# jimmyyhwu/spatial-intention-maps

Hardware: AMD Instinct MI355X
Metric: Q-map transitions/sec, 96x96: `value` = full train() step (M2: policy fwd + bwd, double-DQN next-state forwards, clip, SGD); `value_fwd_bwd_only` = policy fwd+bwd alone (M1, the literal reading of "fwd+bwd") (higher is better)
Workload: dtype f32

## Files before the change

### include/simq.h

```cpp
#ifndef SIMQ_H
#define SIMQ_H

#include <stdint.h>

#ifdef __cplusplus
extern "C" {
#endif

#define SIMQ_VERSION 500
#define SIMQ_STATE_WIDTH 96

#define SIMQ_MODE_EVAL 0
#define SIMQ_MODE_TRAIN 1
#define SIMQ_MODE_TRAIN_NOGRAD 2

#define SIMQ_KIND_CONV_W 0
#define SIMQ_KIND_CONV_B 1
#define SIMQ_KIND_BN_W 2
#define SIMQ_KIND_BN_B 3

#define SIMQ_PREC_FP32 0
#define SIMQ_PREC_BF16X3 1
#define SIMQ_PREC_BF16 2

typedef struct simq_plan simq_plan;

int simq_version(void);
#define SIMQ_BUILD_ABLATIONS 1
int simq_build_flags(void);
const char* simq_last_error(void);

int simq_plan_create(int num_input_channels, int num_output_channels, simq_plan** out);
int simq_plan_create_ex(int num_input_channels, int num_output_channels, int precision, simq_plan** out);
typedef struct simq_plan_options {
    int struct_bytes;
    int winograd;
    int winograd_min_cc;
    int winograd_f4_forward;
    int winograd_f4_min_tiles;
    int winograd_f4_grad;
    int winograd_f4_fwd_grad_min_cc;
    int winograd_wgrad;
    int winograd_wgrad_f4;
    int stem_bf16;
    int bf16_act_grads;
    int keep_fp32_activations;
    int fold_eval_bn_bf16;
    int fuse_bn_backward_sums;
    int fuse_stem_backward_sums;
    int fuse_bn1_apply;
    int deterministic;
    int bn1_mask_from_preact;
    int wgrad_ksplit;
    int fwd_overlap;
    int wgrad_overlap;
    int plane_xcd;
    int wgrad_xcd_group;
    int tail_split;
    int early_target_after_block;
    int gemm_split;
} simq_plan_options;
void simq_plan_options_default(simq_plan_options* options);
int simq_plan_create_opts(int num_input_channels, int num_output_channels, int precision, const simq_plan_options* options,
                          simq_plan** out);
int simq_plan_get_options(const simq_plan* plan, simq_plan_options* out);
int simq_plan_precision(const simq_plan* plan);
void simq_plan_destroy(simq_plan* plan);

int64_t simq_param_count(const simq_plan* plan);
int simq_param_num_tensors(const simq_plan* plan);
int simq_param_tensor_info(const simq_plan* plan, int index, char* name, int name_cap,
                           int64_t* offset, int64_t shape[4], int* kind);
int64_t simq_bnbuf_count(const simq_plan* plan);
int simq_bn_num_layers(const simq_plan* plan);
int simq_bn_layer_info(const simq_plan* plan, int index, char* name, int name_cap, int64_t* offset, int* channels);

int64_t simq_workspace_bytes(const simq_plan* plan, int batch);
int64_t simq_workspace_bytes_forward(const simq_plan* plan, int batch);

int64_t simq_wcache_bytes(const simq_plan* plan);
int simq_weights_prepare(const simq_plan* plan, const float* d_params, void* d_wcache, void* stream);

int simq_workspace_tensor(const simq_plan* plan, int batch, const char* name, int64_t* byte_offset, int64_t* elems,
                          int* channels);

int simq_workspace_tensor_ex(const simq_plan* plan, int batch, const char* name, int64_t* byte_offset, int64_t* elems, int* channels,
                             int* storage);

int simq_forward(const simq_plan* plan, int mode, int batch, const float* d_params, const void* d_wcache, float* d_bnbuf,
                 const float* d_x, float* d_q, void* d_workspace, void* stream);

int simq_backward(const simq_plan* plan, int batch, const float* d_params, const void* d_wcache, const float* d_dq,
                  float* d_grads, void* d_workspace, void* stream);

int64_t simq_backward_trace_bytes(const simq_plan* plan, int batch);
int simq_backward_trace_tensor(const simq_plan* plan, int batch, const char* name, int64_t* byte_offset, int64_t* elems, int* channels,
                               int* storage);
int simq_backward_traced(const simq_plan* plan, int batch, const float* d_params, const void* d_wcache, const float* d_dq,
                         float* d_grads, void* d_workspace, void* d_trace, void* stream);

int simq_backward_phase(const simq_plan* plan, int batch, const float* d_params, const void* d_wcache, const float* d_dq,
                        float* d_grads, void* d_workspace, int phase, void* stream);
int64_t simq_grad_bucket_split(const simq_plan* plan);
int simq_backward_onehot(const simq_plan* plan, int batch, const float* d_params, const void* d_wcache, const int64_t* d_action,
                         const float* d_q_sa, const float* d_y, float grad_scale, float* d_grads, void* d_workspace, int phase,
                         void* stream);

typedef int (*simq_reduce_fn)(void* user, double* d_buf, int64_t count, void* stream);
typedef struct simq_sync { simq_reduce_fn reduce; void* user; int global_batch; int world_size; } simq_sync;
int simq_forward_sync(const simq_plan* plan, int mode, int batch, const float* d_params, const void* d_wcache, float* d_bnbuf,
                      const float* d_x, float* d_q, void* d_workspace, void* stream, const simq_sync* sync);
int simq_backward_sync(const simq_plan* plan, int batch, const float* d_params, const void* d_wcache, const float* d_dq,
                       const int64_t* d_action, const float* d_q_sa, const float* d_y, float grad_scale, float* d_grads,
                       void* d_workspace, int phase, void* stream, const simq_sync* sync);
int simq_comm_reduce_f64(void* comm, double* d_buf, int64_t count, void* stream);
int simq_forward_sync_null(const simq_plan* plan, int layout_batch, float* d_bnbuf, void* d_workspace, void* stream, const simq_sync* sync);

int simq_q_argmax(const float* d_q, int rows, int n, int64_t* d_index, float* d_max, void* stream);
int simq_q_gather(const float* d_q, int rows, int n, const int64_t* d_index, float* d_out, void* stream);
int simq_scatter_next_values(const float* d_values, const int32_t* d_nonfinal_pos, int n_nonfinal,
                             float* d_next_state_values, int batch, void* stream);
int simq_td_huber(const float* d_q, int batch, int n, const int64_t* d_action, const float* d_reward,
                  const float* d_next_state_values, float gamma, float grad_scale,
                  float* d_q_sa, float* d_y, float* d_td_error, float* d_out4, float* d_dq, void* stream);

int simq_clip_sgd_step(float* d_params, float* d_grads, float* d_momentum, int64_t count,
                       float max_norm, float lr, float momentum, float weight_decay, int first_step,
                       void* d_scratch, float* d_total_norm, void* stream);

int simq_replay_gather(const float* d_ring, int64_t item_floats, const int64_t* d_index, int count,
                       float* d_out, void* stream);

typedef struct simq_train_args {
    const simq_plan* plan;
    int batch, num_nonfinal, global_batch, use_double_dqn, first_step;
    int sync_bn;
    float gamma, lr, momentum, weight_decay, max_norm, reserved2_;
    float* params; void* wcache; float* bnbuf; float* grads; float* momentum_buf; void* ws_train; void* ws_tmp;
    const float* t_params; const void* t_wcache; float* t_bnbuf; void* t_ws;
    const float* state; const float* next_state; const int64_t* action; const float* reward; const int32_t* nonfinal_pos;
    float* q; float* q_next; float* q_tgt; float* dq;
    float* nsv; float* vals; int64_t* best; float* q_sa; float* y; float* td; float* out4;
    void* opt_scratch; float* total_norm;
    void* stream; void* side_stream;
    int global_nonfinal;
    int struct_bytes;
    struct simq_comm* comm;
    float* loss_host;
    void* target_stream;
    void* third_stream;
} simq_train_args;
int simq_train_step(const simq_train_args* a);
int simq_train_loss_wait(const simq_plan* plan);
int simq_plan_adopt_side_stream(const simq_plan* plan, void* side_stream);

#define SIMQ_COMM_ID_BYTES 128
#define SIMQ_COMM_F32 0
#define SIMQ_COMM_F64 1
typedef struct simq_comm simq_comm;
int simq_comm_unique_id(void* id_out );
int simq_comm_init(const void* id, int world_size, int rank, simq_comm** out);
int simq_comm_adopt_stream(simq_comm* comm, void* stream);
int simq_comm_world_size(const simq_comm* comm);
int simq_comm_rank(const simq_comm* comm);
int simq_comm_allreduce(simq_comm* comm, void* d_buf, int64_t count, int dtype, void* producer_stream);
int simq_comm_broadcast(simq_comm* comm, void* d_buf, int64_t bytes, int root, void* producer_stream);
int simq_comm_wait(simq_comm* comm, void* consumer_stream);
int simq_comm_progress(simq_comm* comm, int64_t out[4]);
int simq_comm_time_waits(simq_comm* comm, int on);
int simq_comm_last_wait_ms(simq_comm* comm, float* ms);
int simq_comm_destroy(simq_comm* comm);

int simq_bce_with_logits(const float* d_logits, const float* d_target, int64_t n, float* d_dlogits, double* d_loss_sum, void* stream);
int simq_split_last_channel(const float* d_x, float* d_head, float* d_last, int64_t pixels, int channels, void* stream);
int simq_sigmoid_concat(const float* d_state, const float* d_logit, float* d_out, float* d_prob, int64_t pixels, int channels, void* stream);

int simq_nchw_to_nhwc(const float* d_in, float* d_out, int batch, int channels, int hw, void* stream);
int simq_nhwc_to_nchw(const float* d_in, float* d_out, int batch, int channels, int hw, void* stream);

typedef struct simq_launch_opts {
    int struct_bytes;
    int force_bm, force_bn;
    int tail_split;
    int plane_xcd;
    int wgrad_xcd_group;
    int wgrad_ksplit;
    int gemm_split;
} simq_launch_opts;
void simq_launch_opts_default(simq_launch_opts* opts);
int simq_conv2d_fwd(const float* d_x, const float* d_w_ohwi, const float* d_bias, float* d_y,
                    int batch, int hin, int win, int cin, int cout, int r, int s, int stride, int pad,
                    double* d_stats , void* stream, const simq_launch_opts* opts);
int simq_conv2d_fwd_winograd(const float* d_x, const float* d_w_ohwi, const float* d_bias, float* d_y,
                             int batch, int hin, int win, int cin, int cout,
                             double* d_stats , float* d_scratch, void* stream, const simq_launch_opts* opts);
int simq_conv2d_fwd_winograd4(const float* d_x, const float* d_w_ohwi, const float* d_bias, float* d_y,
                              int batch, int hin, int win, int cin, int cout,
                              double* d_stats , float* d_scratch, void* stream, const simq_launch_opts* opts);
int simq_bn_relu_apply(const void* d_y, const double* d_stats, const float* d_gamma, const float* d_beta, const void* d_res, int relu,
                       void* d_out, int64_t rows, int channels, int storage, float* d_saved, float* d_running, void* stream);
int simq_bn_relu_backward(const void* d_g, const void* d_mask, int mask_kind, const void* d_y, const float* d_saved, const float* d_gamma,
                          const double* d_red, void* d_dy, void* d_dz_out, float* d_dgamma, float* d_dbeta, int64_t rows, int channels,
                          int storage, void* stream);
int simq_conv2d_fwd_bnrelu_in(const float* d_y_pre, const float* d_in_scale, const float* d_in_shift, const float* d_w_ohwi,
                              const float* d_bias, float* d_y, int batch, int hin, int win, int cin, int cout, int r, int s, int stride,
                              int pad, int form, float* d_scratch, void* stream, const simq_launch_opts* opts);
int simq_conv2d_wgrad_bnrelu_in(const float* d_y_pre, const float* d_in_scale, const float* d_in_shift, const float* d_dy, float* d_dw,
                                int batch, int hin, int win, int cin, int cout, int r, int s, int stride, int pad, int form,
                                float* d_scratch, void* stream, const simq_launch_opts* opts);
int simq_conv2d_fwd_stem_f32(const float* d_x, const float* d_w_ohwi, float* d_y, int batch, int hin, int win, int cin, double* d_stats,
                             void* stream);
int simq_conv2d_fwd_stem_bf16(const float* d_x, const float* d_w_ohwi, uint16_t* d_y, int batch, int hin, int win, int cin,
                              double* d_stats, void* d_scratch, void* stream);
int simq_conv2d_wgrad_stem_bf16(const float* d_x, const uint16_t* d_dy, float* d_dw, int batch, int hin, int win, int cin,
                                float* d_scratch, void* stream);
int simq_conv2d_wgrad_winograd(const float* d_x, const float* d_dy, float* d_dw_ohwi,
                               int batch, int hin, int win, int cin, int cout, float* d_scratch, void* stream, const simq_launch_opts* opts);
int simq_gemm_f32_batched(const float* d_x, const float* d_w, float* d_y, int m, int n, int k, int batch, void* stream,
                          const simq_launch_opts* opts);
int simq_conv2d_dgrad(const float* d_dy, const float* d_w_ohwi, float* d_wt_scratch, float* d_dx,
                      int batch, int hin, int win, int cin, int cout, int r, int s, int pad, void* stream, const simq_launch_opts* opts);
int simq_conv2d_wgrad(const float* d_x, const float* d_dy, float* d_dw_ohwi ,
                      int batch, int hin, int win, int cin, int cout, int r, int s, int stride, int pad,
                      void* stream, const simq_launch_opts* opts);
int simq_conv2d_fwd_bf16(const float* d_x, const float* d_w_ohwi, const float* d_bias, float* d_y, int batch, int hin, int win,
                         int cin, int cout, int r, int s, int stride, int pad, int nplanes, void* d_scratch, double* d_stats,
                         void* stream, const simq_launch_opts* opts);
int simq_conv2d_wgrad_bf16(const float* d_x, const float* d_dy, float* d_dw_ohwi, int batch, int hin, int win, int cin, int cout,
                           int r, int s, int stride, int pad, int nplanes, void* d_scratch, void* stream, const simq_launch_opts* opts);
int64_t simq_conv2d_wgrad_bf16_slab_bytes(void);
int simq_conv2d_wgrad_bf16_slab(const float* d_x, const float* d_dy, float* d_dw_ohwi, int batch, int hin, int win, int cin, int cout,
                                int r, int s, int stride, int pad, int nplanes, void* d_scratch, void* d_slab, void* stream, const simq_launch_opts* opts);
int simq_upsample2x_fwd(const float* d_in, float* d_out, int batch, int h, int w, int c, void* stream);
int simq_upsample2x_bwd(const float* d_dout, float* d_din, int batch, int h, int w, int c, void* stream);

typedef struct simq_grid_problem {
    int64_t grid_offset;
    int64_t out_offset;
    int32_t rows, cols;
    int32_t src_i, src_j;
} simq_grid_problem;
#define SIMQ_GRID_MAX_CELLS (1 << 22)
int simq_grid_distance_images(const uint8_t* d_grids, int64_t grids_bytes, const simq_grid_problem* problems, int n,
                              simq_grid_problem* d_problems, float* d_out, int64_t out_floats, float pixels_per_meter,
                              int unreachable_to_max, float scale, int32_t* d_status, void* stream);

typedef struct simq_grid_path_problem {
    int64_t grid_offset;
    int64_t thin_offset;
    int64_t closest_offset;
    int64_t path_offset;
    int64_t parents_offset;
    int64_t dist_offset;
    int32_t path_capacity;
    int32_t rows, cols;
    int32_t src_i, src_j, tgt_i, tgt_j;
    int32_t box_i0, box_j0, box_rows, box_cols;
    int32_t reserved_;
} simq_grid_path_problem;
#define SIMQ_GRID_PATH_MAX_BOX_CELLS 20000
int simq_grid_paths(const uint8_t* d_grids, int64_t grids_bytes, const int32_t* d_closest, int64_t closest_ints,
                    const simq_grid_path_problem* problems, int n, simq_grid_path_problem* d_problems, int32_t* d_paths,
                    int64_t path_pairs, int32_t* d_lengths, int32_t* d_endpoints, int32_t* d_parents, int64_t parents_ints, float* d_dist,
                    int64_t dist_floats, int32_t* d_status, void* stream);

typedef struct simq_grid_query_problem {
    int64_t grid_offset;
    int64_t closest_offset;
    int64_t work_offset;
    int64_t target_offset;
    int32_t n_targets;
    int32_t rows, cols;
    int32_t src_i, src_j;
    int32_t reserved_;
} simq_grid_query_problem;
int simq_grid_distance_queries(const uint8_t* d_grids, int64_t grids_bytes, const int32_t* d_closest, int64_t closest_ints,
                               const simq_grid_query_problem* problems, int n, const int32_t* targets, int64_t n_targets_total,
                               void* d_descriptors, float* d_work, int64_t work_floats, int images, float* d_out, int64_t out_floats,
                               int32_t* d_status, void* stream);

#define SIMQ_LOCAL_MAP 0
#define SIMQ_LOCAL_DISTANCE 1
#define SIMQ_LOCAL_ROBOTS 2
#define SIMQ_LOCAL_OVERHEAD 3
#define SIMQ_LOCAL_CONSTANT 4
#define SIMQ_LOCAL_CROP 136
#define SIMQ_LOCAL_MAX_CHANNELS 64
typedef struct simq_local_rotation {
    double r[4];
    double offset[2];
    int32_t shape[2];
} simq_local_rotation;
typedef struct simq_local_map {
    const float* d_data;
    int32_t rows, cols;
} simq_local_map;
typedef struct simq_local_robot {
    simq_local_rotation rot;
    int32_t pixel_i, pixel_j;
    int32_t mask;
    float seg_value;
    float map_value;
    int32_t seg_mask;
} simq_local_robot;
typedef struct simq_local_problem {
    simq_local_rotation rot;
    int32_t pixel_i, pixel_j;
    int32_t rows, cols;
    int32_t robot_begin, robot_count;
} simq_local_problem;
typedef struct simq_local_channel {
    int32_t kind;
    int32_t map;
    float value;
    int32_t reserved_;
} simq_local_channel;
int64_t simq_local_state_desc_bytes(int n_maps, int n_robots, int n, int n_channels);
int simq_local_state_images(const simq_local_map* maps, int n_maps, const float* d_masks, int n_masks, const simq_local_robot* robots,
                            int n_robots, const simq_local_problem* problems, int n, const simq_local_channel* channels, int n_channels,
                            void* d_desc, int64_t desc_bytes, float* d_out, int64_t out_floats, void* stream);

#define SIMQ_INTENTION_STORE 0
#define SIMQ_INTENTION_RAMP 1
#define SIMQ_INTENTION_MAX_RADIUS 8
typedef struct simq_intention_segment {
    double start, stop, step;
    int32_t r0, c0, r1, c1;
    int32_t mode;
    int32_t drop_last;
    float value;
    int32_t reserved_;
} simq_intention_segment;
typedef struct simq_intention_problem {
    int32_t seg_begin, seg_count;
} simq_intention_problem;
int64_t simq_intention_desc_bytes(int n_segments, int n);
int simq_intention_maps(const simq_intention_segment* segments, int n_segments, const simq_intention_problem* problems, int n, int rows,
                        int cols, int radius, void* d_desc, int64_t desc_bytes, float* d_out, int64_t out_floats, void* stream);

#define SIMQ_OCCUPANCY_MAX_DIM 256
#define SIMQ_OCCUPANCY_MAX_RADIUS 16
typedef struct simq_occupancy_problem {
    int64_t occupancy_offset;
    int64_t mask_offset;
    int64_t out_offset;
    int32_t rows, cols;
    int32_t radius, thin_radius;
} simq_occupancy_problem;
int simq_occupancy_maps(const uint8_t* d_maps, int64_t maps_bytes, const simq_occupancy_problem* problems, int n,
                        simq_occupancy_problem* d_problems, uint8_t* d_cspace, uint8_t* d_thin, int64_t cspace_bytes, int32_t* d_closest,
                        int64_t closest_ints, int32_t* d_status, void* stream);

#define SIMQ_OBSERVATION_MAX_POINTS (1 << 22)
typedef struct simq_observation_problem {
    int64_t depth_offset;
    int64_t ids_offset;
    int64_t px_offset;
    int64_t py_offset;
    int64_t overhead_offset;
    int64_t occupancy_offset;
    float cam[3], principal[3], right[3], up[3];
    float far_near, far, far_minus_near;
    int32_t min_obstacle, max_obstacle;
    int32_t receptacle, has_receptacle;
    int32_t min_cube, max_cube;
    int32_t height, width;
    int32_t rows, cols;
    int32_t reserved_;
} simq_observation_problem;
int simq_observation_update(const void* d_frames, int64_t frame_words, const simq_observation_problem* problems, int n,
                            simq_observation_problem* d_problems, float* d_overhead, int64_t overhead_floats, uint8_t* d_occupancy,
                            int64_t occupancy_bytes, int32_t* d_status, void* stream);

#define SIMQ_VISUALIZATION_MAX_OUTPUTS 4
typedef struct simq_visualization_problem {
    const float* d_state;
    const float* d_output;
    int64_t out_offset;
    int32_t n, channels;
} simq_visualization_problem;
int simq_state_output_visualizations(const simq_visualization_problem* problems, int n_problems, simq_visualization_problem* d_problems,
                                     const float* d_jet, double alpha, int chw, float* d_out, int64_t out_floats, void* stream);

int simq_profile_start(void);
int simq_profile_stop(double* out, int max_kinds);
int simq_launch_counts_reset(void);
int64_t simq_launch_count(const char* family);
int simq_launch_counts(char* buf, int cap);

#ifdef __cplusplus
}
#endif
#endif
```

### spatial-intention-maps_amd/csrc/backward.hip

```cpp
#include "plan.h"

using namespace simq;

namespace {

int bn_bwd(const Ctx& c, const BnL& bn, const float* g, const float* mask, const float* y, const Act& dy, float* dz_out, int64_t rows,
           bool reduced = false, const uint16_t* mask16 = nullptr, int y_bf16 = -1, int g_bf16 = 0, bool mask_from_y = false) {
    if (y_bf16 < 0) y_bf16 = c.ybf();
    SIMQ_REQUIRE(!mask_from_y || (reduced && !mask && !mask16), "bn_bwd: the recomputed mask needs the fused reduction and no mask tensor");
    if (!reduced) {
        if (bn.C <= 128) {
            double* rep = reinterpret_cast<double*>(c.ws + c.L.colsum);
            SIMQ_CHECK_HIP(hipMemsetAsync(rep, 0, sizeof(double) * kStatReplicas * 2 * bn.C, c.stream));
            RC(launch_bn_bwd_reduce(g, mask, y, c.aux(bn, 2), c.aux(bn, 3), rep, rows, bn.C, c.stream, y_bf16, g_bf16, kStatReplicas));
            RC(launch_stats_fold(rep, c.red(bn), 2 * bn.C, kStatReplicas, c.stream));
        } else {
            RC(launch_bn_bwd_reduce(g, mask, y, c.aux(bn, 2), c.aux(bn, 3), c.red(bn), rows, bn.C, c.stream, y_bf16, g_bf16));
        }
    }
    RC(c.sync_reduce(c.red(bn), 2 * (int64_t)bn.C));
    return launch_bn_bwd_apply(g, mask, y, c.aux(bn, 2), c.aux(bn, 3), c.params + bn.g_off, c.red(bn), dy.fv ? dy.f : nullptr, dz_out,
                               c.grads + bn.g_off, c.grads + bn.b_off, rows, bn.C, c.stream, dy.pl, mask16, y_bf16,
                               c.sync ? c.bn_rows(rows) : 0.0, c.sync ? 1.f / (float)c.sync->world_size : 1.f, g_bf16,
                               mask_from_y ? c.aux(bn, 0) : nullptr, mask_from_y ? c.aux(bn, 1) : nullptr);
}

int conv_wgrad(const Ctx& c, const ConvL& cv, const Act& x, const Act& dy, int hin, const InBn& in = InBn()) {
    ConvGeom g = geom(c.p, cv, c.B, hin);
    if (c.mc() && cv.wp_off >= 0) {
        SIMQ_REQUIRE(!in.on(), "conv_wgrad: BatchNorm-on-load exists for fp32 plans only");
        const uint16_t* xs[2] = {x.pl.hi, x.pl.lo ? x.pl.lo : x.pl.hi};
        const uint16_t* ds[2] = {dy.pl.hi, dy.pl.lo ? dy.pl.lo : dy.pl.hi};
        return launch_conv_wgrad_bf16(xs, ds, c.p->np(), c.grads + cv.w_off, g, c.stream, c.L.wslab >= 0 ? c.f(c.L.wslab) : nullptr, c.dslab());
    }
    if (cv.wu_off >= 0 && c.L.wino >= 0 && winograd_wgrad_eligible(g) && c.p->opt.winograd_wgrad &&
        winograd_wgrad_pays(g, c.p->opt.winograd_wgrad_f4 != 0))
        return launch_conv_wgrad_winograd(x.f, dy.f, c.grads + cv.w_off, g, c.f(c.L.wino), c.stream, c.p->opt.winograd_wgrad_f4 != 0, in);
    return launch_conv_wgrad(x.f, dy.f, c.grads + cv.w_off, g, c.stream, in, c.dslab());
}

int conv_dgrad(const Ctx& c, const ConvL& cv, const Act& dy, float* dx, const float* addend, int hin,
               const ConvEpilogue& fuse = ConvEpilogue(), int g_bf16 = 0) {
    ConvGeom g;
    g.tune = c.p->tune();
    g.B = c.B; g.Hin = hin; g.Win = hin; g.Cin = cv.cout; g.Cout = cv.cin; g.Hout = hin; g.Wout = hin;
    g.R = cv.k; g.S = cv.k; g.stride = 1; g.pad = cv.k - 1 - cv.pad;
    ConvEpilogue e = fuse;
    e.addend = addend;
    e.y_bf16 = g_bf16; e.addend_bf16 = g_bf16;
    if (c.mc() && cv.wp_off >= 0) {
        const uint16_t* ds[2] = {dy.pl.hi, dy.pl.lo ? dy.pl.lo : dy.pl.hi};
        const uint16_t* wsp[2];
        c.wplanes(cv, true, wsp);
        return launch_conv_igemm_bf16(ds, wsp, c.p->np(), dx, g, e, c.stream);
    }
    if (cv.wut4_off >= 0 && c.L.wino >= 0 && winograd_f4_forward(g, c.p->opt.winograd_f4_min_tiles))
        return launch_conv_winograd4(dy.f, reinterpret_cast<const float*>(c.wc + c.W.wu) + cv.wut4_off, dx, g, e, c.f(c.L.wino), c.stream);
    if (cv.wut_off >= 0 && c.L.wino >= 0 && winograd_eligible(g))
        return launch_conv_winograd(dy.f, reinterpret_cast<const float*>(c.wc + c.W.wu) + cv.wut_off, dx, g, e, c.f(c.L.wino), c.stream);
    return launch_conv_igemm(dy.f, reinterpret_cast<const float*>(c.wc + c.W.wt) + cv.wt_off, dx, g, e, c.stream);
}

}

namespace simq {

int backward_impl(const Ctx& c, const float* d_dq, int phase, const OneHotGrad* oh) {
    const simq_plan* p = c.p;
    const Layout& L = c.L;
    const int B = c.B;
    const int wov = p->opt.wgrad_overlap;
    const bool mc_piped = c.mc() && wov == 4 && c.planes_only() && L.DP[2] >= 0 && L.S2[0] >= 0;
    const bool ov = c.wstream != nullptr && (wov == 2 || mc_piped || ((wov == 1 || wov == 3 || wov == 4) && !c.mc()));
    const bool wide_mc = ov && mc_piped;
    const bool wide = (ov && !c.mc() && wov != 3) || wide_mc;
    const bool piped = wide && wov == 4 && L.S2[0] >= 0 && c.ev_wdone[0] && c.ev_wdone[1];
    Ctx cw = c;
    if (ov) { cw.stream = c.wstream; if (L.wino2 >= 0) cw.L.wino = L.wino2; }
    const TraceLayout TL = c.trace ? make_trace_layout(p, B) : TraceLayout();
    auto trace = [&](int64_t off, const void* src, int64_t bytes) -> int {
        if (c.trace && src) SIMQ_CHECK_HIP(hipMemcpyAsync(c.trace + off, src, (size_t)bytes, hipMemcpyDeviceToDevice, c.stream));
        return 0;
    };
    auto fork = [&]() -> int {
        if (ov) { SIMQ_CHECK_HIP(hipEventRecord(c.ev_wfork, c.stream)); SIMQ_CHECK_HIP(hipStreamWaitEvent(c.wstream, c.ev_wfork, 0)); }
        return 0;
    };
    auto join = [&]() -> int {
        if (ov) { SIMQ_CHECK_HIP(hipEventRecord(c.ev_wjoin, c.wstream)); SIMQ_CHECK_HIP(hipStreamWaitEvent(c.stream, c.ev_wjoin, 0)); }
        return 0;
    };
    if (phase != 2) {
        SIMQ_CHECK_HIP(hipMemsetAsync(c.grads, 0, p->nparams * sizeof(float), c.stream));
        SIMQ_CHECK_HIP(hipMemsetAsync(c.ws + L.red, 0, p->red_total * sizeof(double), c.stream));
    }
    float* S[4] = {c.f(L.S[0]), c.f(L.S[1]), c.f(L.S[2]), c.f(L.S[3])};
    const int64_t smax = (int64_t)B * 294912;
    auto dyact = [&](float* buf, int which) { Act a; a.f = buf; a.pl = c.planes(L.DP[which], smax); return a; };
    double* cs = reinterpret_cast<double*>(c.ws + L.colsum);
    double* cs_side = cs + kStatReplicas * 2 * 128;
    const int64_t rows = (int64_t)B * 576;
    const bool no_fuse_head = !p->opt.fuse_bn_backward_sums;
    const bool head_side = piped && phase != 2;
    Act dyh = dyact(S[0], 0);
    Act t2 = dyact(S[1], 1);
    if (phase != 2) {
    if (oh) {
        RC(launch_head_onehot_bwd(c.f(L.ah2), c.params + p->h3.w_off, oh->action, oh->q_sa, oh->y, oh->grad_scale, S[1],
                                  c.grads + p->h3.w_off, c.grads + p->h3.b_off, B, p->cout, c.stream,
                                  c.f(L.yh2), 0, c.aux(p->hb2, 2), c.aux(p->hb2, 3), no_fuse_head ? nullptr : c.red(p->hb2), p->opt.deterministic));
    } else {
        RC(launch_upsample2x_fwd(c.f(L.ah2), c.f(L.up2), B, 48, 48, 32, c.stream));
        RC(launch_head_conv3_bwd(c.f(L.up2), c.params + p->h3.w_off, d_dq, S[0], c.grads + p->h3.w_off, c.grads + p->h3.b_off, B, 9216, 32, p->cout, c.stream,
                                 c.dslab()));
        RC(launch_upsample2x_bwd(S[0], S[1], B, 48, 48, 32, c.stream));
        RC(trace(TL.head.da2, S[1], (int64_t)B * 2304 * 32 * 4));
    }
    if (head_side) {
        dyh.f = c.f(L.S2[0]); dyh.pl = c.planes(L.DP2[0], smax);
        t2.f = c.f(L.S2[1]); t2.pl = c.planes(L.DP2[1], smax);
    }
    const Ctx& ch = head_side ? cw : c;
    static const int bias_side_on = SIMQ_TUNE_INT("SIMQ_HEAD_BIAS_SIDE", 1);
    const bool bias_side = head_side && c.mc() && bias_side_on;
    bool hb1_fused = false;
    {
        Act dy2; dy2.f = S[0];
        RC(bn_bwd(c, p->hb2, S[1], c.f(L.ah2), c.f(L.yh2), dy2, nullptr, (int64_t)B * 2304, oh != nullptr && !no_fuse_head, nullptr, 0));
        RC(trace(TL.head.dy2, S[0], (int64_t)B * 2304 * 32 * 4));
        RC(launch_upsample2x_bwd(S[0], t2.f, B, 24, 24, 32, c.stream, t2.pl));
        RC(trace(TL.head.dz2, t2.f, rows * 32 * 4));
        Act a1; a1.f = c.f(L.ah1); a1.pl = c.planes(L.p_up1, rows * 128);
        if (head_side) RC(fork());
        RC(launch_colsum_rep(t2.f, bias_side ? cs_side : cs, c.grads + p->h2.b_off, rows, 32, kStatReplicas, bias_side ? ch.stream : c.stream));
        if (c.lazy1()) {
            Act yh1; yh1.f = c.f(L.yh1);
            RC(conv_wgrad(ch, p->h2, yh1, t2, 24, c.inbn_saved(p->hb1)));
        } else {
            RC(conv_wgrad(ch, p->h2, a1, t2, 24));
        }
        ConvEpilogue fh;
        const bool fuse_hb1 = !no_fuse_head && !c.mc();
        if (fuse_hb1) {
            if (c.lazy1()) { fh.bnr_mscale = c.aux(p->hb1, 0); fh.bnr_mshift = c.aux(p->hb1, 1); }
            else fh.bnr_mask = c.f(L.ah1);
            fh.bnr_y1 = c.f(L.yh1); fh.bnr_y_bf16 = c.ybf();
            fh.bnr_mean1 = c.aux(p->hb1, 2); fh.bnr_invstd1 = c.aux(p->hb1, 3); fh.bnr_red1 = c.red(p->hb1);
        }
        RC(conv_dgrad(c, p->h2, t2, S[2], nullptr, 24, fh));
        RC(trace(TL.head.da1, S[2], rows * 128 * 4));
        hb1_fused = fuse_hb1;
    }
    RC(bn_bwd(c, p->hb1, S[2], c.lazy1() ? nullptr : c.f(L.ah1), c.f(L.yh1), dyh, nullptr, rows, hb1_fused, nullptr, -1, 0, c.lazy1()));
    RC(trace(TL.head.dy1, dyh.f, rows * 128 * 4));
    if (head_side) RC(fork());
    RC(launch_colsum_rep(dyh.f, bias_side ? cs_side : cs, c.grads + p->h1.b_off, rows, 128, kStatReplicas, bias_side ? ch.stream : c.stream));
    RC(conv_wgrad(ch, p->h1, c.act(L.blk[7].out, L.blk[7].p_out, rows * 512), dyh, 24));
    if (head_side) SIMQ_CHECK_HIP(hipEventRecord(c.ev_wdone[1], c.wstream));
    }
    const bool no_fuse = !p->opt.fuse_bn_backward_sums;
    auto fuse_block_out = [&](int bi) {
        ConvEpilogue e;
        if (no_fuse) return e;
        const BlockL& bb = p->blocks[bi];
        if (c.planes_only()) e.bnr_mask16 = c.planes(L.blk[bi].p_out, rows * bb.planes).hi;
        else e.bnr_mask = c.f(L.blk[bi].out);
        e.bnr_y_bf16 = c.ybf();
        e.bnr_y1 = c.f(L.blk[bi].y2); e.bnr_mean1 = c.aux(bb.b2, 2); e.bnr_invstd1 = c.aux(bb.b2, 3); e.bnr_red1 = c.red(bb.b2);
        if (bb.has_ds) {
            e.bnr_y2 = c.f(L.blk[bi].yd); e.bnr_mean2 = c.aux(bb.bds, 2); e.bnr_invstd2 = c.aux(bb.bds, 3); e.bnr_red2 = c.red(bb.bds);
        }
        return e;
    };
    const int gb = c.gbf();
    if (phase != 2) RC(conv_dgrad(c, p->h1, dyh, S[1], nullptr, 24, fuse_block_out(7), gb));
    const int gi = 1;
    const int i_hi = phase == 2 ? kPhaseSplitBlock - 1 : 7, i_lo = phase == 1 ? kPhaseSplitBlock : 0;
    for (int i = i_hi; i >= i_lo; --i) {
        if (c.ev_late && i == c.late_block) SIMQ_CHECK_HIP(hipEventRecord(c.ev_late, c.stream));
        const BlockL& b = p->blocks[i];
        const Layout::Blk& o = L.blk[i];
        const Act xin = i == 0 ? c.act(L.pooled, L.p_pooled, rows * 64)
                               : c.act(L.blk[i - 1].out, L.blk[i - 1].p_out, rows * p->blocks[i - 1].planes);
        const Act a1 = c.act(o.a1, o.p_a1, rows * b.planes);
        float* G = S[gi];
        Act T0 = dyact(S[(gi + 1) & 3], 0);
        Act T1 = dyact(S[(gi + 2) & 3], 1);
        float* T2 = S[(gi + 3) & 3];
        const int set = (i_hi - i) & 1;
        if (piped) {
            if (set) {
                T0 = Act(); T0.f = c.f(L.S2[0]); T0.pl = c.planes(L.DP2[0], smax);
                T1 = Act(); T1.f = c.f(L.S2[1]); T1.pl = c.planes(L.DP2[1], smax);
                T2 = c.f(L.S2[2]);
            }
            if (i_hi - i >= 2 || (head_side && i_hi - i == 1))
                SIMQ_CHECK_HIP(hipStreamWaitEvent(c.stream, c.ev_wdone[set], 0));
        }
        const bool po = c.planes_only();
        T0.fv = T1.fv = !po;
        const float* m_out = po ? nullptr : c.f(o.out);
        const bool mfy = c.mask1_from_y() && !no_fuse;
        const float* m_a1 = (po || mfy) ? nullptr : c.f(o.a1);
        const uint16_t* m16_out = po ? c.planes(o.p_out, rows * b.planes).hi : nullptr;
        const uint16_t* m16_a1 = (po && !mfy) ? c.planes(o.p_a1, rows * b.planes).hi : nullptr;
        const int64_t nel = rows * b.planes, gsz = gb ? 2 : 4, dsz = po ? 2 : 4;
        auto dptr = [&](const Act& a) -> const void* { return po ? (const void*)a.pl.hi : (const void*)a.f; };
        RC(trace(TL.blk[i].g_out, G, nel * gsz));
        RC(bn_bwd(c, b.b2, G, m_out, c.f(o.y2), T0, b.has_ds ? nullptr : T1.f, rows, !no_fuse, m16_out, -1, gb));
        if (b.has_ds) RC(bn_bwd(c, b.bds, G, m_out, c.f(o.yd), T1, nullptr, rows, !no_fuse, m16_out, -1, gb));
        RC(trace(TL.blk[i].dy2, dptr(T0), nel * dsz));
        if (b.has_ds) RC(trace(TL.blk[i].t1, dptr(T1), nel * dsz));
        else RC(trace(TL.blk[i].t1, T1.f, nel * gsz));
        RC(fork());
        if (c.lazy1()) {
            Act y1; y1.f = c.f(o.y1);
            RC(conv_wgrad(cw, b.c2, y1, T0, 24, c.inbn_saved(b.b1)));
        } else {
            RC(conv_wgrad(cw, b.c2, a1, T0, 24));
        }
        ConvEpilogue f1;
        if (!no_fuse) {
        f1.bnr_y_bf16 = c.ybf();
        if (mfy) { f1.bnr_mscale = c.aux(b.b1, 0); f1.bnr_mshift = c.aux(b.b1, 1); }
        f1.bnr_mask = m_a1; f1.bnr_mask16 = m16_a1; f1.bnr_y1 = c.f(o.y1); f1.bnr_mean1 = c.aux(b.b1, 2); f1.bnr_invstd1 = c.aux(b.b1, 3); f1.bnr_red1 = c.red(b.b1);
        }
        RC(conv_dgrad(c, b.c2, T0, T2, nullptr, 24, f1, gb));
        RC(trace(TL.blk[i].da1, T2, nel * gsz));
        Act D1 = T0;
        if (wide) { D1 = Act(); D1.f = T2; D1.fv = !po; if (wide_mc) D1.pl = c.planes((piped && set) ? L.DP2[2] : L.DP[2], smax); }
        else RC(join());
        RC(bn_bwd(c, b.b1, T2, m_a1, c.f(o.y1), D1, nullptr, rows, !no_fuse, m16_a1, -1, gb, mfy));
        RC(trace(TL.blk[i].dy1, dptr(D1), nel * dsz));
        RC(fork());
        RC(conv_wgrad(cw, b.c1, xin, D1, 24));
        const ConvEpilogue fin = i > 0 ? fuse_block_out(i - 1) : ConvEpilogue();
        if (b.has_ds) {
            RC(conv_wgrad(cw, b.ds, xin, T1, 24));
            RC(conv_dgrad(c, b.ds, T1, G, nullptr, 24, ConvEpilogue(), gb));
            RC(trace(TL.blk[i].g_ds, G, rows * b.cin * gsz));
            RC(conv_dgrad(c, b.c1, D1, G, G, 24, fin, gb));
        } else {
            RC(conv_dgrad(c, b.c1, D1, G, T1.f, 24, fin, gb));
        }
        RC(trace(TL.blk[i].g_in, G, rows * b.cin * gsz));
        if (piped) SIMQ_CHECK_HIP(hipEventRecord(c.ev_wdone[set], c.wstream));
        else RC(join());
    }
    const bool late_join = piped && phase != 1 && i_hi > i_lo && ((i_hi - i_lo) & 1) == 1 && !p->opt.deterministic;
    if (piped) {
        if (late_join) SIMQ_CHECK_HIP(hipStreamWaitEvent(c.stream, c.ev_wdone[0], 0));
        else RC(join());
    }
    if (phase == 1) return 0;
    float* G = S[gi];
    float* T0 = S[(gi + 1) & 3];
    Act T1; T1.f = S[(gi + 2) & 3];
    const bool stem16 = c.W.stem16 >= 0;
    if (stem16) { T1 = dyact(S[(gi + 2) & 3], 1); T1.fv = false; }
    Act x0; x0.f = c.x_ext ? const_cast<float*>(c.x_ext) : c.f(L.x);
    const int y0_bf16 = c.W.stem16 >= 0 ? 1 : 0;
    const bool no_stem_fuse = !p->opt.fuse_stem_backward_sums || !p->opt.fuse_bn_backward_sums;
    double* srep = reinterpret_cast<double*>(c.ws + L.red) + p->stem_rep_off;
    RC(launch_stem_pool_bwd(G, c.f(L.pooled), reinterpret_cast<const uint8_t*>(c.ws + L.idx), T0, B, 48, 48, 64, c.stream, c.gbf(),
                            c.f(L.y0), c.aux(p->stem_bn, 2), c.aux(p->stem_bn, 3), no_stem_fuse ? nullptr : srep, y0_bf16, kStatReplicas));
    if (!no_stem_fuse) RC(launch_stats_fold(srep, c.red(p->stem_bn), 2 * p->stem_bn.C, kStatReplicas, c.stream));
    RC(trace(TL.stem.dz, T0, (int64_t)B * 2304 * 64 * 4));
    RC(bn_bwd(c, p->stem_bn, T0, nullptr, c.f(L.y0), T1, nullptr, (int64_t)B * 2304, !no_stem_fuse, nullptr, y0_bf16));
    RC(trace(TL.stem.dy0, stem16 ? (const void*)T1.pl.hi : (const void*)T1.f, (int64_t)B * 2304 * 64 * (stem16 ? 2 : 4)));
    if (stem16)
        RC(launch_stem_wgrad_bf16(x0.f, T1.pl.hi, c.grads + p->stem.w_off, T0, B, 96, 96, p->cin, c.stream));
    else
        RC(conv_wgrad(c, p->stem, x0, T1, 96));
    if (late_join) RC(join());
    return 0;
}

}

static int attach_backward_side(Ctx& c) {
    const int wov = c.p->opt.wgrad_overlap;
    if (c.wstream || wov == 0 || (c.mc() && wov != 2 && wov != 4)) return 0;
    PlanStreams* ps = nullptr;
    int dev = 0;
    RC(plan_streams(c.p, &ps, &dev));
    if (!ps) return 0;
    if (c.stream) {
        hipDevice_t sdev = 0;
        SIMQ_CHECK_HIP(hipStreamGetDevice(c.stream, &sdev));
        if ((int)sdev != dev) return 0;
    }
    if (!ps->bwd_ev[0]) {
        std::lock_guard<std::mutex> lk(c.p->mu);
        for (int i = 0; i < 4; ++i) SIMQ_CHECK_HIP(hipEventCreateWithFlags(&ps->bwd_ev[i], hipEventDisableTiming));
    }
    if (!ps->bwd_side_ext && !ps->bwd_side) {
        std::lock_guard<std::mutex> lk(c.p->mu);
        SIMQ_CHECK_HIP(hipStreamCreateWithFlags(&ps->bwd_side, hipStreamNonBlocking));
    }
    c.wstream = ps->bwd_side_ext ? ps->bwd_side_ext : ps->bwd_side; c.ev_wfork = ps->bwd_ev[0]; c.ev_wjoin = ps->bwd_ev[1]; c.ev_wdone[0] = ps->bwd_ev[2]; c.ev_wdone[1] = ps->bwd_ev[3];
    return 0;
}

namespace simq {
TraceLayout make_trace_layout(const simq_plan* p, int B) {
    TraceLayout T;
    int64_t off = 0;
    auto take = [&](int64_t bytes) { int64_t o = off; off = align_up(off + bytes, 256); return o; };
    const bool mc = p->precision != SIMQ_PREC_FP32;
    const bool po = mc && !p->opt.keep_fp32_activations && p->opt.fuse_bn_backward_sums;
    const int64_t gsz = (p->precision == SIMQ_PREC_BF16 && p->opt.bf16_act_grads) ? 2 : 4, dsz = po ? 2 : 4;
    for (int i = 7; i >= 0; --i) {
        const int64_t n = (int64_t)B * 576 * p->blocks[i].planes;
        T.blk[i].g_out = take(n * gsz); T.blk[i].dy2 = take(n * dsz);
        T.blk[i].t1 = take(n * (p->blocks[i].has_ds ? dsz : gsz));
        T.blk[i].da1 = take(n * gsz); T.blk[i].dy1 = take(n * dsz);
        T.blk[i].g_ds = p->blocks[i].has_ds ? take((int64_t)B * 576 * p->blocks[i].cin * gsz) : -1;
        T.blk[i].g_in = take((int64_t)B * 576 * p->blocks[i].cin * gsz);
    }
    T.head.da2 = take((int64_t)B * 2304 * 32 * 4); T.head.dy2 = take((int64_t)B * 2304 * 32 * 4); T.head.dz2 = take((int64_t)B * 576 * 32 * 4);
    T.head.da1 = take((int64_t)B * 576 * 128 * 4); T.head.dy1 = take((int64_t)B * 576 * 128 * 4);
    T.stem.dz = take((int64_t)B * 2304 * 64 * 4); T.stem.dy0 = take((int64_t)B * 2304 * 64 * 4);
    T.total = off;
    return T;
}

int backward_sync_side(const simq_plan* plan, int batch, const float* d_params, const void* d_wcache, const float* d_dq,
                              const int64_t* d_action, const float* d_q_sa, const float* d_y, float grad_scale, float* d_grads,
                              void* d_workspace, int phase, void* stream, const simq_sync* sync, hipStream_t wstream, hipEvent_t ev_wfork,
                              hipEvent_t ev_wjoin, hipEvent_t ev_wdone0, hipEvent_t ev_wdone1, const float* x_ext, hipEvent_t ev_late, int late_block) {
    Ctx c{plan, batch, d_params, d_grads, nullptr, static_cast<char*>(d_workspace), make_layout(plan, batch), static_cast<hipStream_t>(stream)};
    c.wc = static_cast<char*>(const_cast<void*>(d_wcache)); c.W = make_wlayout(plan);
    c.sync = sync;
    c.x_ext = x_ext;
    c.ev_late = ev_late; c.late_block = late_block;
    if (wstream && ev_wfork && ev_wjoin) { c.wstream = wstream; c.ev_wfork = ev_wfork; c.ev_wjoin = ev_wjoin; c.ev_wdone[0] = ev_wdone0; c.ev_wdone[1] = ev_wdone1; }
    else RC(attach_backward_side(c));
    if (d_dq) return backward_impl(c, d_dq, phase);
    const OneHotGrad oh{d_action, d_q_sa, d_y, grad_scale};
    return backward_impl(c, nullptr, phase, &oh);
}
}

extern "C" {

int simq_backward_sync(const simq_plan* plan, int batch, const float* d_params, const void* d_wcache, const float* d_dq,
                       const int64_t* d_action, const float* d_q_sa, const float* d_y, float grad_scale, float* d_grads,
                       void* d_workspace, int phase, void* stream, const simq_sync* sync) {
    SIMQ_REQUIRE(plan && d_params && d_wcache && d_grads && d_workspace && (d_dq || (d_action && d_q_sa && d_y)), "backward_sync: NULL argument");
    SIMQ_REQUIRE(phase >= 0 && phase <= 2, "backward: bad phase %d", phase);
    SIMQ_REQUIRE(batch >= 1 && batch <= 4096, "backward: batch=%d out of range", batch);
    RC(check_sync(sync, batch));
    return backward_sync_side(plan, batch, d_params, d_wcache, d_dq, d_action, d_q_sa, d_y, grad_scale, d_grads, d_workspace, phase, stream, sync,
                              nullptr, nullptr, nullptr);
}

int simq_backward_phase(const simq_plan* plan, int batch, const float* d_params, const void* d_wcache, const float* d_dq,
                        float* d_grads, void* d_workspace, int phase, void* stream) {
    SIMQ_REQUIRE(plan && d_params && d_wcache && d_dq && d_grads && d_workspace, "backward: NULL argument");
    SIMQ_REQUIRE(phase >= 0 && phase <= 2, "backward: bad phase %d", phase);
    SIMQ_REQUIRE(batch >= 1 && batch <= 4096, "backward: batch=%d out of range", batch);
    Ctx c{plan, batch, d_params, d_grads, nullptr, static_cast<char*>(d_workspace), make_layout(plan, batch), static_cast<hipStream_t>(stream)};
    c.wc = static_cast<char*>(const_cast<void*>(d_wcache)); c.W = make_wlayout(plan);
    RC(attach_backward_side(c));
    return backward_impl(c, d_dq, phase);
}

int simq_backward_onehot(const simq_plan* plan, int batch, const float* d_params, const void* d_wcache, const int64_t* d_action,
                         const float* d_q_sa, const float* d_y, float grad_scale, float* d_grads, void* d_workspace, int phase,
                         void* stream) {
    SIMQ_REQUIRE(plan && d_params && d_wcache && d_action && d_q_sa && d_y && d_grads && d_workspace, "backward_onehot: NULL argument");
    SIMQ_REQUIRE(phase >= 0 && phase <= 2, "backward: bad phase %d", phase);
    SIMQ_REQUIRE(batch >= 1 && batch <= 4096, "backward: batch=%d out of range", batch);
    Ctx c{plan, batch, d_params, d_grads, nullptr, static_cast<char*>(d_workspace), make_layout(plan, batch), static_cast<hipStream_t>(stream)};
    c.wc = static_cast<char*>(const_cast<void*>(d_wcache)); c.W = make_wlayout(plan);
    const OneHotGrad oh{d_action, d_q_sa, d_y, grad_scale};
    RC(attach_backward_side(c));
    return backward_impl(c, nullptr, phase, &oh);
}

int simq_plan_adopt_side_stream(const simq_plan* plan, void* side_stream) {
    SIMQ_REQUIRE(plan, "plan_adopt_side_stream: NULL plan");
    PlanStreams* ps = nullptr;
    int dev = 0;
    RC(plan_streams(plan, &ps, &dev));
    SIMQ_REQUIRE(ps, "plan_adopt_side_stream: device index %d out of range", dev);
    if (side_stream) {
        hipDevice_t sdev = 0;
        SIMQ_CHECK_HIP(hipStreamGetDevice(static_cast<hipStream_t>(side_stream), &sdev));
        SIMQ_REQUIRE((int)sdev == dev, "plan_adopt_side_stream: the stream belongs to device %d, the calling thread's current device is %d", (int)sdev, dev);
    }
    ps->bwd_side_ext = static_cast<hipStream_t>(side_stream);
    return 0;
}

int64_t simq_backward_trace_bytes(const simq_plan* plan, int batch) {
    if (!plan || batch < 1) return -1;
    return make_trace_layout(plan, batch).total;
}

int simq_backward_trace_tensor(const simq_plan* plan, int batch, const char* name, int64_t* byte_offset, int64_t* elems, int* channels, int* storage) {
    SIMQ_REQUIRE(plan && name && batch >= 1, "backward_trace_tensor: bad argument");
    const TraceLayout T = make_trace_layout(plan, batch);
    const bool mc = plan->precision != SIMQ_PREC_FP32;
    const bool po = mc && !plan->opt.keep_fp32_activations && plan->opt.fuse_bn_backward_sums;
    const int gst = (plan->precision == SIMQ_PREC_BF16 && plan->opt.bf16_act_grads) ? 1 : 0, dst = po ? 1 : 0;
    int li = 0, bi = 0;
    char what[32] = "";
    int64_t off = -1;
    int ch = 0, st = 0;
    if (sscanf(name, "layer%d.%d.%31s", &li, &bi, what) == 3 && li >= 1 && li <= 4 && bi >= 0 && bi <= 1) {
        const int i = (li - 1) * 2 + bi;
        const BlockL& b = plan->blocks[i];
        const std::string w(what);
        ch = b.planes;
        if (w == "g_out") { off = T.blk[i].g_out; st = gst; }
        else if (w == "dy2") { off = T.blk[i].dy2; st = dst; }
        else if (w == "dz" && !b.has_ds) { off = T.blk[i].t1; st = gst; }
        else if (w == "dyd" && b.has_ds) { off = T.blk[i].t1; st = dst; }
        else if (w == "da1") { off = T.blk[i].da1; st = gst; }
        else if (w == "dy1") { off = T.blk[i].dy1; st = dst; }
        else if (w == "g_in") { off = T.blk[i].g_in; st = gst; ch = b.cin; }
        else if (w == "g_ds" && b.has_ds) { off = T.blk[i].g_ds; st = gst; ch = b.cin; }
    }
    int64_t pixels = 576;
    if (off < 0) {
        const std::string n(name);
        const bool stem16 = make_wlayout(plan).stem16 >= 0;
        if (n == "head.da2") { off = T.head.da2; ch = 32; pixels = 2304; }
        else if (n == "head.dy2") { off = T.head.dy2; ch = 32; pixels = 2304; }
        else if (n == "head.dz2") { off = T.head.dz2; ch = 32; }
        else if (n == "head.da1") { off = T.head.da1; ch = 128; }
        else if (n == "head.dy1") { off = T.head.dy1; ch = 128; }
        else if (n == "stem.dz") { off = T.stem.dz; ch = 64; pixels = 2304; }
        else if (n == "stem.dy0") { off = T.stem.dy0; ch = 64; pixels = 2304; st = stem16 ? 1 : 0; }
    }
    SIMQ_REQUIRE(off >= 0, "backward_trace_tensor: '%s' is not a tensor of the traced walk (layer<1-4>.<0-1>.<g_out|dy2|dz|dyd|da1|dy1|g_ds|g_in>, "
                 "head.<da2|dy2|dz2|da1|dy1>, stem.<dz|dy0>)", name);
    if (byte_offset) *byte_offset = off;
    if (elems) *elems = (int64_t)batch * pixels * ch;
    if (channels) *channels = ch;
    if (storage) *storage = st;
    return 0;
}

int simq_backward_traced(const simq_plan* plan, int batch, const float* d_params, const void* d_wcache, const float* d_dq,
                         float* d_grads, void* d_workspace, void* d_trace, void* stream) {
    SIMQ_REQUIRE(plan && d_params && d_wcache && d_dq && d_grads && d_workspace && d_trace, "backward_traced: NULL argument");
    SIMQ_REQUIRE(batch >= 1 && batch <= 4096, "backward: batch=%d out of range", batch);
    Ctx c{plan, batch, d_params, d_grads, nullptr, static_cast<char*>(d_workspace), make_layout(plan, batch), static_cast<hipStream_t>(stream)};
    c.wc = static_cast<char*>(const_cast<void*>(d_wcache)); c.W = make_wlayout(plan);
    c.trace = static_cast<char*>(d_trace);
    RC(attach_backward_side(c));
    return backward_impl(c, d_dq, 0);
}

int simq_backward(const simq_plan* plan, int batch, const float* d_params, const void* d_wcache, const float* d_dq,
                  float* d_grads, void* d_workspace, void* stream) {
    return simq_backward_phase(plan, batch, d_params, d_wcache, d_dq, d_grads, d_workspace, 0, stream);
}

}
```

### spatial-intention-maps_amd/csrc/common.h

```cpp
#pragma once
#include <hip/hip_runtime.h>
#include <stdint.h>

struct simq_comm;

namespace simq {

typedef float floatx16 __attribute__((ext_vector_type(16)));
typedef float floatx4 __attribute__((ext_vector_type(4)));

void set_error(const char* fmt, ...);

#ifdef SIMQ_ABLATIONS
int tune_env_int(const char* name, int dflt);
#define SIMQ_TUNE_INT(name, dflt) (simq::tune_env_int(name, dflt))
#else
#define SIMQ_TUNE_INT(name, dflt) (dflt)
#endif

#define SIMQ_CHECK_HIP(expr)                                                        \
    do {                                                                            \
        hipError_t _e = (expr);                                                     \
        if (_e != hipSuccess) {                                                     \
            simq::set_error("%s:%d: %s -> %s", __FILE__, __LINE__, #expr, hipGetErrorString(_e)); \
            return -2;                                                              \
        }                                                                           \
    } while (0)

#define SIMQ_CHECK_LAUNCH() SIMQ_CHECK_HIP(hipGetLastError())

#define SIMQ_REQUIRE(cond, ...)             \
    do {                                    \
        if (!(cond)) {                      \
            simq::set_error(__VA_ARGS__);   \
            return -1;                      \
        }                                   \
    } while (0)

struct LaunchTune {
    int force_bm = 0, force_bn = 0;
    int tail_split = 0;
    int plane_xcd = 1;
    int wgrad_xcd_group = 1;
    int wgrad_ksplit = 0;
    int gemm_split = 0;
};

struct ConvGeom {
    int B, Hin, Win, Cin, Hout, Wout, Cout, R, S, stride, pad;
    LaunchTune tune;
    int M() const { return B * Hout * Wout; }
    int K() const { return R * S * Cin; }
};

struct ConvEpilogue {
    const float* bias = nullptr;
    double* stats = nullptr;
    const float* scale = nullptr;
    const float* shift = nullptr;
    const float* addend = nullptr;
    int relu = 0;
    int y_bf16 = 0, bnr_y_bf16 = 0;
    int addend_bf16 = 0;
    const float* bnr_mask = nullptr;
    const uint16_t* bnr_mask16 = nullptr;
    const float* bnr_mscale = nullptr; const float* bnr_mshift = nullptr;
    const float* bnr_y1 = nullptr; const float* bnr_mean1 = nullptr; const float* bnr_invstd1 = nullptr; double* bnr_red1 = nullptr;
    const float* bnr_y2 = nullptr; const float* bnr_mean2 = nullptr; const float* bnr_invstd2 = nullptr; double* bnr_red2 = nullptr;
};

struct BnRef {
    const double* stats = nullptr;
    const float* gamma = nullptr;
    const float* beta = nullptr;
    float* rmean = nullptr;
    float* rvar = nullptr;
    float* save_mean = nullptr;
    float* save_invstd = nullptr;
    float* save_scale = nullptr;
    float* save_shift = nullptr;
    double rows = 0.0, inv_rows = 0.0;
    int C = 0;
    double* defer = nullptr;
};
struct InBn {
    const float* scale = nullptr; const float* shift = nullptr;
    BnRef bn;
    int live = 0;
    bool on() const { return live != 0 || scale != nullptr; }
};

void prof_launch_begin(int kind, double flops, double bytes, hipStream_t stream);
void prof_launch_end(hipStream_t stream);
void note_launch(const char* family);

int launch_conv_igemm(const float* x, const float* w, float* y, const ConvGeom& g, const ConvEpilogue& e,
                      hipStream_t stream, const InBn& in = InBn());
int try_gemm_batched_pp(const float* x, const float* w, float* y, int M, int N, int K, int batch, hipStream_t stream);
int launch_gemm_batched(const float* x, const float* w, float* y, int M, int N, int K, int batch, hipStream_t stream, const LaunchTune& tune = LaunchTune());
bool gemm_split3_eligible(int M, int N, int K, int batch);
int launch_gemm_batched_split3(const float* x, const float* w, float* y, int M, int N, int K, int batch, hipStream_t stream, const LaunchTune& tune);
bool winograd_eligible(const ConvGeom& g);
bool winograd_pays(int cin, int cout, long min_cc);
int64_t winograd_scratch_floats(const ConvGeom& g);
int launch_wino_weight(const float* w_ohwi, float* U, int cout, int cin, hipStream_t stream);
struct WinoWeightDesc { int64_t src_off, u_off; int cout, cin, from_wt, pad_; };
constexpr int kWinoWeightTableCap = 72;
struct WinoWeightTable { WinoWeightDesc d[kWinoWeightTableCap]; int n; };
int launch_wino_weight_all(const float* params, const float* wt, float* ubase, const WinoWeightTable& t, hipStream_t stream);
int launch_conv_winograd(const float* x, const float* U, float* y, const ConvGeom& g, const ConvEpilogue& e, float* scratch,
                         hipStream_t stream, const InBn& in = InBn());
bool winograd_f4_forward(const ConvGeom& g, int min_tiles);
int launch_conv_winograd4(const float* x, const float* U4, float* y, const ConvGeom& g, const ConvEpilogue& e, float* scratch,
                          hipStream_t stream, const InBn& in = InBn());
constexpr int64_t kWgradDetSlabFloats = 16 << 20;
int launch_conv_wgrad(const float* x, const float* dy, float* dw, const ConvGeom& g, hipStream_t stream, const InBn& in = InBn(), float* det_slab = nullptr);
int launch_wgrad_slab_sum(const float* slab, float* dw, int64_t n, int splits, hipStream_t stream);
int launch_wgrad_batched(const float* x, const float* dy, float* dw, int M, int N, int K, int batch, hipStream_t stream, const LaunchTune& tune = LaunchTune());
bool winograd_wgrad_eligible(const ConvGeom& g);
bool winograd_wgrad_pays(const ConvGeom& g, bool allow_f4);
int launch_conv_wgrad_winograd(const float* x, const float* dy, float* dw, const ConvGeom& g, float* scratch, hipStream_t stream, bool allow_f4 = true,
                               const InBn& in = InBn());
int tune_forced_tile(const LaunchTune& t, int* bm, int* bn);
int launch_conv_igemm_bf16(const uint16_t* const x[2], const uint16_t* const w[2], int nplanes, float* y, const ConvGeom& g,
                           const ConvEpilogue& e, hipStream_t stream);
int launch_conv_wgrad_bf16(const uint16_t* const x[2], const uint16_t* const dy[2], int nplanes, float* dw, const ConvGeom& g,
                           hipStream_t stream, float* slab = nullptr, float* det_slab = nullptr);
int try_conv_wgrad_bf16_pp(const uint16_t* x, const uint16_t* dy, float* dw, const ConvGeom& g, unsigned x_bytes, unsigned dy_bytes,
                           hipStream_t stream);
int try_conv_wgrad_bf16_img(const uint16_t* x, const uint16_t* dy, float* dw, const ConvGeom& g, unsigned x_bytes, unsigned dy_bytes,
                           hipStream_t stream, float* slab = nullptr);
int64_t conv_wgrad_bf16_slab_bytes();
struct WeightPrepDesc { int64_t w_off, wt_off, wp_off; int cout, taps, cin, pad_; };
struct WeightPrepTable { WeightPrepDesc d[24]; int n; };
int launch_weight_prep_all(const float* params, const WeightPrepTable& t, float* wt_f32, uint16_t* wpl, uint16_t* wtpl, int np,
                           int64_t wp_total, hipStream_t stream);
int launch_split_planes(const float* src, uint16_t* hi, uint16_t* lo, int64_t n, hipStream_t stream);
int launch_weight_planes(const float* w, uint16_t* w_hi, uint16_t* w_lo, uint16_t* wt_hi, uint16_t* wt_lo, int cout, int taps,
                         int cin, hipStream_t stream);
int launch_weight_transpose(const float* w, float* wt, int cout, int taps, int cin, hipStream_t stream);

struct Planes { uint16_t* hi = nullptr; uint16_t* lo = nullptr; };

struct BnEvalDesc { int64_t g_off, b_off, buf_off, aux_off; int C, pad_; };
struct BnEvalTable { BnEvalDesc d[24]; int n; };
int launch_bn_eval_coeff(const BnEvalTable& t, const float* params, const float* bnbuf, float* aux, hipStream_t stream);
int launch_bn_running_update(const double* stats, float* rmean, float* rvar, double rows, int C, hipStream_t stream);
int launch_bn_apply(const float* y, const BnRef& bn, const float* res, const BnRef* rbn, int relu, float* out, int64_t rows,
                    int C, hipStream_t stream, Planes pl = Planes(), Planes res_pl = Planes(), int y_bf16 = 0);
int launch_head_bn_relu_conv3(const float* y, const BnRef& bn, const float* w3, float* a, float* z, int B, int HW, int Cout, hipStream_t stream);
int launch_stem_pool_fwd(const float* y, const BnRef& bn, float* pooled, uint8_t* idx, int B, int H, int W, int C,
                         hipStream_t stream, Planes pl = Planes(), int y_bf16 = 0);
int stem_conv_bf16_wbytes();
int try_conv_img_f32(const float* x, const float* w, float* y, const ConvGeom& g, const ConvEpilogue& e, hipStream_t stream, const InBn& in = InBn());
bool stem_conv_f32_eligible(int H, int W, int C, int cout, int k, int stride, int pad);
int launch_stem_conv_f32(const float* x, const float* w_ohwi, float* y, double* stats, int B, int H, int W, int C, hipStream_t stream);
bool stem_conv_bf16_eligible(int H, int W, int C, int cout, int k, int stride, int pad);
int launch_stem_weight_prep(const float* w, uint16_t* w16, int C, hipStream_t stream);
int launch_stem_conv_bf16(const float* x, const uint16_t* w16, uint16_t* y, double* stats, int B, int H, int W, int C, hipStream_t stream);
int stem_wgrad_bf16_slabs(int B, int H, int W);
int launch_stem_wgrad_bf16(const float* x, const uint16_t* dy, float* dw, float* partial, int B, int H, int W, int C, hipStream_t stream);
int launch_stem_pool_bwd(const float* g, const float* pooled, const uint8_t* idx, float* dz, int B, int H, int W,
                         int C, hipStream_t stream, int g_bf16 = 0, const float* y = nullptr, const float* mean = nullptr,
                         const float* invstd = nullptr, double* red = nullptr, int y_bf16 = 0, int replicas = 1);
int launch_bn_bwd_reduce(const float* g, const float* mask, const float* y, const float* mean,
                         const float* invstd, double* red, int64_t rows, int C, hipStream_t stream, int y_bf16 = 0, int g_bf16 = 0, int replicas = 1);
int launch_bn_bwd_apply(const float* g, const float* mask, const float* y, const float* mean,
                        const float* invstd, const float* gamma, const double* red, float* dy, float* dz_out,
                        float* dgamma, float* dbeta, int64_t rows, int C, hipStream_t stream, Planes pl = Planes(),
                        const uint16_t* mask16 = nullptr, int y_bf16 = 0, double global_rows = 0.0, float dparam_scale = 1.f,
                        int g_bf16 = 0,
                        const float* mscale = nullptr, const float* mshift = nullptr);
int launch_colsum(const float* x, double* red_scratch, float* out, int64_t rows, int C, hipStream_t stream);
int launch_colsum_rep(const float* x, double* red_scratch, float* out, int64_t rows, int C, int replicas, hipStream_t stream);
int launch_colsum_finish(const double* red, float* out, int C, hipStream_t stream);
int launch_upsample2x_fwd(const float* in, float* out, int B, int H, int W, int C, hipStream_t stream, Planes pl = Planes(),
                          double* stats = nullptr, int relu = 0, int replicas = 1);
int launch_bn_running_deferred(float* bnbuf, const double* defer, int64_t n, hipStream_t stream);
int launch_stats_fold(const double* rep, double* out, int n, int replicas, hipStream_t stream);
int launch_upsample2x_bwd(const float* dout, float* din, int B, int H, int W, int C, hipStream_t stream, Planes pl = Planes());
int launch_add_inplace(float* dst, const float* src, int64_t n, hipStream_t stream);
int launch_nchw_to_nhwc(const float* in, float* out, int B, int C, int HW, hipStream_t stream);
int launch_nhwc_to_nchw(const float* in, float* out, int B, int C, int HW, hipStream_t stream);

int launch_head_conv3_fwd(const float* x, const float* w, const float* bias, float* q, int B, int HW, int Cin,
                          int Cout, hipStream_t stream);
int launch_head_up_relu_conv3(const float* z2, const float* w, float* z, int B, int Cout, hipStream_t stream);
int launch_head_upsample_q(const float* z, const float* bias, float* q, int B, int Cout, hipStream_t stream);
int launch_head_onehot_bwd(const float* ah2, const float* w3, const int64_t* action, const float* q_sa, const float* y,
                           float grad_scale, float* ds1, float* dw3, float* db3, int B, int Cout, hipStream_t stream,
                           const float* ypre = nullptr, int ypre_bf16 = 0, const float* mean = nullptr, const float* invstd = nullptr,
                           double* red = nullptr,
                           int serial = 0);
int launch_head_conv3_bwd(const float* x, const float* w, const float* dq, float* dx, float* dw, float* dbias,
                          int B, int HW, int Cin, int Cout, hipStream_t stream, float* det_slab = nullptr);

int launch_q_argmax(const float* q, int rows, int n, int64_t* index, float* maxv, hipStream_t stream);
int launch_q_gather(const float* q, int rows, int n, const int64_t* index, float* out, hipStream_t stream);
int launch_scatter_next_values(const float* values, const int32_t* pos, int n, float* nsv, int batch,
                               hipStream_t stream);
int launch_td_huber(const float* q, int batch, int n, const int64_t* action, const float* reward,
                    const float* nsv, float gamma, float grad_scale, float* q_sa, float* y, float* td,
                    float* out4, float* dq, hipStream_t stream);
int launch_clip_sgd(float* p, float* g, float* m, int64_t count, float max_norm, float lr, float momentum,
                    float wd, int first_step, void* scratch, float* total_norm, hipStream_t stream);
int launch_bce_logits(const float* x, const float* t, int64_t n, float* dx, double* loss_sum, hipStream_t stream);
int launch_split_last_channel(const float* x, float* head, float* last, int64_t pixels, int C, hipStream_t stream);
int launch_sigmoid_concat(const float* state, const float* logit, float* out, float* prob, int64_t pixels, int Cs, hipStream_t stream);
int launch_replay_gather(const float* ring, int64_t item_floats, const int64_t* index, int count, float* out,
                         hipStream_t stream);

int comm_allreduce(simq_comm* c, void* buf, int64_t count, int dtype, hipStream_t producer);
int comm_reduce_f64(void* comm, double* buf, int64_t count, void* stream);
int comm_wait(simq_comm* c, hipStream_t consumer);
hipStream_t comm_stream(simq_comm* c);

}
```

### spatial-intention-maps_amd/csrc/conv_wgrad.hip

```cpp
#include <cstdlib>
#include <type_traits>

#include "common.h"

namespace simq {

namespace {

constexpr int BR = 16;

struct WgradArgs {
    const float* x;
    const float* dy;
    float* dw;
    int Hin, Win, Cin, Hout, Wout, Cout, R, S, stride, pad;
    int M, K;
    int tilesI, tilesJ, rows_per_split;
    int splits, xcd_group;
    unsigned x_bytes, dy_bytes;
    long gx, gdy, gdw;
    float* slab;
    const float* xscale; const float* xshift;
};

template <int TI, int TJ, int WI, int WJ, bool VEC, bool XBN = false>
__global__ void __launch_bounds__(256) wgrad_kernel(const WgradArgs p) {
    static_assert(WI * WJ == 4, "4 waves per block");
    static_assert(VEC || !XBN, "the BatchNorm-on-load form exists for the vector loader only");
    constexpr int NI = TI / WI / 32, NJ = TJ / WJ / 32;
    static_assert(NI >= 1 && NJ >= 1, "wave tile must be a multiple of 32x32");
    constexpr int STAGE = BR * (TI + TJ);
    __shared__ __attribute__((aligned(16))) float smem[2 * STAGE];

    const int tid = threadIdx.x, lane = tid & 63, wave = tid >> 6;
    const int wi = wave / WJ, wj = wave % WJ;
    int id = blockIdx.x, split;
    {
        const int tiles = p.tilesI * p.tilesJ;
        if (p.xcd_group) {
            const int k = id & 7, j = id >> 3;
            split = (j / tiles) * 8 + k;
            id = (j + k) % tiles;
            if (split >= p.splits) return;
        } else {
            split = id / tiles;
            id -= split * tiles;
        }
    }
    const int tj = id % p.tilesJ;
    const int ti = id / p.tilesJ;
    const int i0 = ti * TI;
    const int rbeg = split * p.rows_per_split;
    const int rend = min(p.M, rbeg + p.rows_per_split);
    const int hw = p.Hout * p.Wout;

    int tap = 0, cj0 = 0, ky = 0, kx = 0;
    int sk = 0, sci = 0, sky = 0, skx = 0;
    bool skok = false;
    if constexpr (VEC) {
        const int cj_tiles = p.Cin / TJ;
        tap = tj / cj_tiles;
        cj0 = (tj - tap * cj_tiles) * TJ;
        ky = tap / p.S;
        kx = tap - ky * p.S;
    } else {
        sk = tj * TJ + (tid % TJ);
        skok = sk < p.K;
        int t = sk / p.Cin;
        sci = sk - t * p.Cin;
        sky = t / p.S;
        skx = t - sky * p.S;
    }

    floatx16 acc[NI][NJ];
#pragma unroll
    for (int a = 0; a < NI; ++a)
#pragma unroll
        for (int b = 0; b < NJ; ++b)
#pragma unroll
            for (int r = 0; r < 16; ++r) acc[a][b][r] = 0.f;

    constexpr int Y_F4 = BR * TI / 4, X_F4 = BR * TJ / 4;
    constexpr int Y_PASSES = (Y_F4 + 255) / 256, X_PASSES_V = (X_F4 + 255) / 256;
    constexpr int X_PASSES_S = BR * TJ / 256;
    float4 vy[2][Y_PASSES], vx[2][VEC ? X_PASSES_V : 1];
    float sx[2][VEC ? 1 : X_PASSES_S];
    unsigned xok[2] = {0u, 0u};
    float4 xsc = make_float4(1.f, 1.f, 1.f, 1.f), xsh = make_float4(0.f, 0.f, 0.f, 0.f);
    if constexpr (XBN) {
        const int ch = cj0 + (tid % (TJ / 4)) * 4;
        xsc = make_float4(p.xscale[ch], p.xscale[ch + 1], p.xscale[ch + 2], p.xscale[ch + 3]);
        xsh = make_float4(p.xshift[ch], p.xshift[ch + 1], p.xshift[ch + 2], p.xshift[ch + 3]);
    }
    __amdgpu_buffer_rsrc_t xr = __builtin_amdgcn_make_buffer_rsrc(const_cast<float*>(p.x + blockIdx.y * p.gx), 0, p.x_bytes, 0x00020000);
    __amdgpu_buffer_rsrc_t yr = __builtin_amdgcn_make_buffer_rsrc(const_cast<float*>(p.dy + blockIdx.y * p.gdy), 0, p.dy_bytes, 0x00020000);

    int xb[VEC ? X_PASSES_V : 1], xoy[VEC ? X_PASSES_V : 1], xox[VEC ? X_PASSES_V : 1];
    if constexpr (VEC) {
#pragma unroll
        for (int ps = 0; ps < X_PASSES_V; ++ps) {
            const int r = rbeg + (tid + 256 * ps) / (TJ / 4);
            xb[ps] = r / hw;
            const int rem = r - xb[ps] * hw;
            xoy[ps] = rem / p.Wout;
            xox[ps] = rem - xoy[ps] * p.Wout;
        }
    }
    auto load_tile = [&](auto set_c, int r0) {
        constexpr int SET = decltype(set_c)::value;
#pragma unroll
        for (int ps = 0; ps < Y_PASSES; ++ps) {
            const int idx = tid + 256 * ps;
            const int row = idx / (TI / 4), c4 = idx - row * (TI / 4);
            const int r = r0 + row;
            const bool ok = (Y_F4 % 256 == 0 || idx < Y_F4) && r < rend;
            const unsigned voff = ok ? (unsigned)(r * p.Cout + i0 + c4 * 4) * 4u : 0xFFFFFFFFu;
            vy[SET][ps] = __builtin_bit_cast(float4, __builtin_amdgcn_raw_buffer_load_b128(yr, voff, 0, 0));
        }
        if constexpr (VEC) {
            if constexpr (XBN) xok[SET] = 0u;
#pragma unroll
            for (int ps = 0; ps < X_PASSES_V; ++ps) {
                const int idx = tid + 256 * ps;
                const int row = idx / (TJ / 4), c4 = idx - row * (TJ / 4);
                const int r = r0 + row;
                const int iy = xoy[ps] * p.stride - p.pad + ky, ix = xox[ps] * p.stride - p.pad + kx;
                const bool ok = (X_F4 % 256 == 0 || idx < X_F4) && r < rend && (unsigned)iy < (unsigned)p.Hin &&
                                (unsigned)ix < (unsigned)p.Win;
                const unsigned voff = ok ? (unsigned)(((xb[ps] * p.Hin + iy) * p.Win + ix) * p.Cin + cj0 + c4 * 4) * 4u : 0xFFFFFFFFu;
                vx[SET][ps] = __builtin_bit_cast(float4, __builtin_amdgcn_raw_buffer_load_b128(xr, voff, 0, 0));
                if constexpr (XBN) xok[SET] |= ok ? (1u << ps) : 0u;
                xox[ps] += BR;
                while (xox[ps] >= p.Wout) { xox[ps] -= p.Wout; ++xoy[ps]; }
                if (xoy[ps] >= p.Hout) { xoy[ps] -= p.Hout; ++xb[ps]; }
            }
        } else {
#pragma unroll
            for (int ps = 0; ps < X_PASSES_S; ++ps) {
                const int row = tid / TJ + (256 / TJ) * ps;
                const int r = r0 + row;
                const int b = r / hw, rem = r - b * hw;
                const int oy = rem / p.Wout, ox = rem - oy * p.Wout;
                const int iy = oy * p.stride - p.pad + sky, ix = ox * p.stride - p.pad + skx;
                const bool ok = skok && r < rend && (unsigned)iy < (unsigned)p.Hin && (unsigned)ix < (unsigned)p.Win;
                const unsigned voff = ok ? (unsigned)(((b * p.Hin + iy) * p.Win + ix) * p.Cin + sci) * 4u : 0xFFFFFFFFu;
                sx[SET][ps] = __builtin_bit_cast(float, __builtin_amdgcn_raw_buffer_load_b32(xr, voff, 0, 0));
            }
        }
    };
    auto store_tile = [&](auto set_c, int buf) {
        constexpr int SET = decltype(set_c)::value;
        float* Ys = smem + buf * STAGE;
        float* Xs = Ys + BR * TI;
#pragma unroll
        for (int ps = 0; ps < Y_PASSES; ++ps) {
            int idx = tid + 256 * ps;
            if (Y_F4 % 256 == 0 || idx < Y_F4) *reinterpret_cast<float4*>(Ys + idx * 4) = vy[SET][ps];
        }
        if constexpr (VEC) {
#pragma unroll
            for (int ps = 0; ps < X_PASSES_V; ++ps) {
                int idx = tid + 256 * ps;
                float4 v = vx[SET][ps];
                if constexpr (XBN) {
                    const bool ok = (xok[SET] >> ps) & 1u;
                    v.x = ok ? fmaxf(__builtin_fmaf(v.x, xsc.x, xsh.x), 0.f) : 0.f; v.y = ok ? fmaxf(__builtin_fmaf(v.y, xsc.y, xsh.y), 0.f) : 0.f;
                    v.z = ok ? fmaxf(__builtin_fmaf(v.z, xsc.z, xsh.z), 0.f) : 0.f; v.w = ok ? fmaxf(__builtin_fmaf(v.w, xsc.w, xsh.w), 0.f) : 0.f;
                }
                if (X_F4 % 256 == 0 || idx < X_F4) *reinterpret_cast<float4*>(Xs + idx * 4) = v;
            }
        } else {
#pragma unroll
            for (int ps = 0; ps < X_PASSES_S; ++ps) Xs[(tid / TJ + (256 / TJ) * ps) * TJ + (tid % TJ)] = sx[SET][ps];
        }
    };

    const int fi = lane & 31, fh = lane >> 5;
    auto compute = [&](int buf) {
        const float* Ys = smem + buf * STAGE;
        const float* Xs = Ys + BR * TI;
#pragma unroll
        for (int kk = 0; kk < BR / 2; ++kk) {
            float af[NI], bf[NJ];
#pragma unroll
            for (int a = 0; a < NI; ++a) af[a] = Ys[(kk * 2 + fh) * TI + wi * (TI / WI) + a * 32 + fi];
#pragma unroll
            for (int b = 0; b < NJ; ++b) bf[b] = Xs[(kk * 2 + fh) * TJ + wj * (TJ / WJ) + b * 32 + fi];
#pragma unroll
            for (int a = 0; a < NI; ++a)
#pragma unroll
                for (int b = 0; b < NJ; ++b)
                    acc[a][b] = __builtin_amdgcn_mfma_f32_32x32x2f32(af[a], bf[b], acc[a][b], 0, 0, 0);
        }
    };
    using S0 = std::integral_constant<int, 0>;
    using S1 = std::integral_constant<int, 1>;

    if (rbeg >= rend) return;
    const int nk = (rend - rbeg + BR - 1) / BR;
    load_tile(S0{}, rbeg);
    store_tile(S0{}, 0);
    load_tile(S1{}, rbeg + BR);
    __syncthreads();
    int kt = 0;
    for (; kt + 1 < nk; kt += 2) {
        load_tile(S0{}, rbeg + (kt + 2) * BR);
        compute(0);
        store_tile(S1{}, 1);
        __syncthreads();
        load_tile(S1{}, rbeg + (kt + 3) * BR);
        compute(1);
        store_tile(S0{}, 0);
        __syncthreads();
    }
    if (kt < nk) compute(0);

#pragma unroll
    for (int b = 0; b < NJ; ++b) {
        const int j = wj * (TJ / WJ) + b * 32 + fi;
        size_t col;
        bool cok = true;
        if constexpr (VEC) {
            col = (size_t)tap * p.Cin + cj0 + j;
        } else {
            col = (size_t)tj * TJ + j;
            cok = col < (size_t)p.K;
        }
        if (!cok) continue;
#pragma unroll
        for (int a = 0; a < NI; ++a) {
#pragma unroll
            for (int r = 0; r < 16; ++r) {
                const int i = i0 + wi * (TI / WI) + a * 32 + (r & 3) + 8 * (r >> 2) + 4 * fh;
                if (p.slab) p.slab[((size_t)split * p.Cout + i) * p.K + col] = acc[a][b][r];
                else unsafeAtomicAdd(p.dw + blockIdx.y * p.gdw + (size_t)i * p.K + col, acc[a][b][r]);
            }
        }
    }
}

template <int TI, int TJ, int WI, int WJ, bool VEC>
int run(const WgradArgs& a, hipStream_t stream, const LaunchTune& tune, int batch = 1) {
    static_assert(256 % (TJ / 4) == 0, "a lane keeps its channel quad across the passes of the x loader");
    WgradArgs p = a;
    p.tilesI = p.Cout / TI;
    p.tilesJ = VEC ? p.R * p.S * (p.Cin / TJ) : (p.K + TJ - 1) / TJ;
    const int tiles = p.tilesI * p.tilesJ;
    const int ltiles = tiles * batch;
    const int rsteps = (p.M + BR - 1) / BR;
    int max_splits = rsteps / 8;
    if (max_splits > 96) max_splits = 96;
    if (max_splits < 1) max_splits = 1;
    int splits = 1;
    double best = 1e300;
    for (int s = 1; s <= max_splits; ++s) {
        const long rounds = ((long)ltiles * s + 255) / 256;
        const double util = rounds == 1 ? 0.6 : rounds == 2 ? 0.85 : 1.0;
        const double cost = (double)rounds * ((rsteps + s - 1) / s + 6) / util;
        if (cost < best * 0.999) { best = cost; splits = s; }
    }
    if (p.slab) {
        const int64_t fit = kWgradDetSlabFloats / ((int64_t)p.Cout * p.K);
        SIMQ_REQUIRE(batch == 1 && fit >= 1, "wgrad: the deterministic slab holds %ld floats, one tile set needs %ld", (long)kWgradDetSlabFloats, (long)p.Cout * p.K);
        if (splits > fit) splits = (int)fit;
    }
    if (const int forced_s = batch > 1 ? SIMQ_TUNE_INT("SIMQ_WGRAD_BATCHED_SPLITS", 0) : SIMQ_TUNE_INT("SIMQ_WGRAD_SPLITS", 0)) splits = forced_s;
    int rps = (p.M + splits - 1) / splits;
    rps = ((rps + BR - 1) / BR) * BR;
    splits = (p.M + rps - 1) / rps;
    p.rows_per_split = rps;
    p.splits = splits;
    p.xcd_group = (tune.wgrad_xcd_group == 2 && batch == 1 && splits >= 8 && tiles > 1) ? 1 : 0;
    const int launch_splits = p.xcd_group ? ((splits + 7) / 8) * 8 : splits;
    note_launch(batch > 1 ? "wgrad_f32_batched" : "wgrad_f32");
    prof_launch_begin(1, 2.0 * p.M * p.Cout * p.K * batch,
                      4.0 * batch * ((double)p.M / (p.Hout * p.Wout) * p.Hin * p.Win * p.Cin + (double)p.Cout * p.K + (double)p.M * p.Cout),
                      stream);
    if constexpr (VEC) {
        if (p.xscale) hipLaunchKernelGGL((wgrad_kernel<TI, TJ, WI, WJ, VEC, true>), dim3((unsigned)(tiles * launch_splits), (unsigned)batch), dim3(256), 0, stream, p);
        else hipLaunchKernelGGL((wgrad_kernel<TI, TJ, WI, WJ, VEC>), dim3((unsigned)(tiles * launch_splits), (unsigned)batch), dim3(256), 0, stream, p);
    } else {
        hipLaunchKernelGGL((wgrad_kernel<TI, TJ, WI, WJ, VEC>), dim3((unsigned)(tiles * launch_splits), (unsigned)batch), dim3(256), 0, stream, p);
    }
    prof_launch_end(stream);
    SIMQ_CHECK_LAUNCH();
    if (p.slab) return launch_wgrad_slab_sum(p.slab, p.dw, (int64_t)p.Cout * p.K, splits, stream);
    return 0;
}

__global__ void __launch_bounds__(256) wgrad_slab_sum_kernel(const float* __restrict__ slab, float* __restrict__ dw, size_t n, int splits) {
    for (size_t e = blockIdx.x * (size_t)256 + threadIdx.x; e < n; e += (size_t)gridDim.x * 256) {
        float a = slab[e];
        for (int s2 = 1; s2 < splits; ++s2) a += slab[(size_t)s2 * n + e];
        dw[e] = a;
    }
}

}

int launch_wgrad_slab_sum(const float* slab, float* dw, int64_t n, int splits, hipStream_t stream) {
    int blocks = (int)((n + 255) / 256);
    if (blocks > 2048) blocks = 2048;
    hipLaunchKernelGGL(wgrad_slab_sum_kernel, dim3(blocks), dim3(256), 0, stream, slab, dw, (size_t)n, splits);
    SIMQ_CHECK_LAUNCH();
    return 0;
}

int launch_conv_wgrad(const float* x, const float* dy, float* dw, const ConvGeom& g, hipStream_t stream, const InBn& in, float* det_slab) {
    WgradArgs a;
    a.x = x; a.dy = dy; a.dw = dw; a.slab = det_slab;
    a.xscale = in.scale; a.xshift = in.shift;
    SIMQ_REQUIRE(!in.live, "conv_wgrad: BatchNorm-on-load takes the scale / shift the forward pass saved (not a live layer)");
    SIMQ_REQUIRE(!in.scale || g.Cin % 64 == 0, "conv_wgrad: BatchNorm-on-load needs Cin %% 64 == 0 (Cin=%d)", g.Cin);
    a.Hin = g.Hin; a.Win = g.Win; a.Cin = g.Cin; a.Hout = g.Hout; a.Wout = g.Wout; a.Cout = g.Cout;
    a.R = g.R; a.S = g.S; a.stride = g.stride; a.pad = g.pad;
    a.M = g.M(); a.K = g.K();
    a.tilesI = a.tilesJ = a.rows_per_split = 0;
    a.gx = a.gdy = a.gdw = 0;
    SIMQ_REQUIRE(a.M > 0, "wgrad: empty problem");
    SIMQ_REQUIRE(g.Cout % 32 == 0, "conv_wgrad: Cout=%d must be a multiple of 32", g.Cout);
    const double xb = 4.0 * g.B * g.Hin * g.Win * g.Cin, yb = 4.0 * a.M * g.Cout;
    SIMQ_REQUIRE(xb < 4294967000.0 && yb < 4294967000.0, "conv_wgrad: tensor exceeds the 4 GiB buffer-addressing limit");
    a.x_bytes = (unsigned)xb; a.dy_bytes = (unsigned)yb;
    const bool vec = (g.Cin % 64) == 0;
    if (vec) {
        if (g.Cout % 128 == 0) {
            if (g.Cin % 128 == 0) return (g.Cout / 128) * (g.R * g.S * g.Cin / 128) >= 16 ? run<128, 128, 2, 2, true>(a, stream, g.tune)
                                                                                            : run<64, 64, 2, 2, true>(a, stream, g.tune);
            return run<128, 64, 2, 2, true>(a, stream, g.tune);
        }
        if (g.Cout % 64 == 0) return run<64, 64, 2, 2, true>(a, stream, g.tune);
        if (g.Cin % 128 == 0) return run<32, 128, 1, 4, true>(a, stream, g.tune);
        SIMQ_REQUIRE(false, "conv_wgrad: unsupported Cout=%d Cin=%d", g.Cout, g.Cin);
    }
    SIMQ_REQUIRE(g.Cout % 64 == 0, "conv_wgrad (generic gather): Cout=%d must be a multiple of 64", g.Cout);
    return run<64, 64, 2, 2, false>(a, stream, g.tune);
}

int launch_wgrad_batched(const float* x, const float* dy, float* dw, int M, int N, int K, int batch, hipStream_t stream, const LaunchTune& tune) {
    SIMQ_REQUIRE(M > 0 && N % 128 == 0 && K % 128 == 0 && batch >= 1, "wgrad_batched: M=%d N=%d K=%d batch=%d not supported", M, N, K, batch);
    WgradArgs a;
    a.x = x; a.dy = dy; a.dw = dw;
    a.Hin = M; a.Win = 1; a.Cin = K; a.Hout = M; a.Wout = 1; a.Cout = N; a.R = 1; a.S = 1; a.stride = 1; a.pad = 0;
    a.M = M; a.K = K;
    a.tilesI = a.tilesJ = a.rows_per_split = 0;
    a.gx = (long)M * K; a.gdy = (long)M * N; a.gdw = (long)N * K;
    a.xscale = a.xshift = nullptr; a.slab = nullptr;
    const double xb = 4.0 * M * K, yb = 4.0 * M * N;
    SIMQ_REQUIRE(xb < 4294967000.0 && yb < 4294967000.0, "wgrad_batched: operand exceeds the 4 GiB buffer-addressing limit");
    a.x_bytes = (unsigned)xb; a.dy_bytes = (unsigned)yb;
    return run<128, 128, 2, 2, true>(a, stream, tune, batch);
}

}
```

### spatial-intention-maps_amd/csrc/head.hip

```cpp
#include "common.h"

namespace simq {

namespace {

constexpr int MAX_COUT = 4;

template <int CIN>
__global__ void __launch_bounds__(256) head_conv3_fwd_kernel(const float* __restrict__ x, const float* __restrict__ w,
                                                             const float* __restrict__ bias, float* __restrict__ q,
                                                             int B, int HW, int Cout) {
    constexpr int L = CIN / 4;
    const int sub = threadIdx.x % L;
    float4 wv[MAX_COUT];
    for (int co = 0; co < MAX_COUT; ++co)
        wv[co] = co < Cout ? *reinterpret_cast<const float4*>(w + co * CIN + sub * 4) : make_float4(0, 0, 0, 0);
    const size_t total = (size_t)B * HW;
    const size_t ppb = blockDim.x / L;
    for (size_t pix = blockIdx.x * ppb + threadIdx.x / L; pix < total; pix += (size_t)gridDim.x * ppb) {
        float4 v = *reinterpret_cast<const float4*>(x + pix * CIN + sub * 4);
        const unsigned b = (unsigned)pix / (unsigned)HW, p = (unsigned)pix - b * (unsigned)HW;
        for (int co = 0; co < Cout; ++co) {
            float s = v.x * wv[co].x + v.y * wv[co].y + v.z * wv[co].z + v.w * wv[co].w;
#pragma unroll
            for (int o = L / 2; o >= 1; o >>= 1) s += __shfl_xor(s, o);
            if (sub == 0) q[((size_t)b * Cout + co) * HW + p] = s + (bias ? bias[co] : 0.f);
        }
    }
}

template <int CIN>
__global__ void __launch_bounds__(256) head_conv3_bwd_kernel(const float* __restrict__ x, const float* __restrict__ w,
                                                             const float* __restrict__ dq, float* __restrict__ dx,
                                                             float* dw, float* dbias, int B, int HW, int Cout, float* slab_w, float* slab_b) {
    constexpr int L = CIN / 4;
    __shared__ float red[256 * 4];
    const int sub = threadIdx.x % L;
    float4 wv[MAX_COUT], gw[MAX_COUT];
    float gb[MAX_COUT];
    for (int co = 0; co < MAX_COUT; ++co) {
        wv[co] = co < Cout ? *reinterpret_cast<const float4*>(w + co * CIN + sub * 4) : make_float4(0, 0, 0, 0);
        gw[co] = make_float4(0, 0, 0, 0);
        gb[co] = 0.f;
    }
    const size_t total = (size_t)B * HW;
    const size_t ppb = blockDim.x / L;
    for (size_t pix = blockIdx.x * ppb + threadIdx.x / L; pix < total; pix += (size_t)gridDim.x * ppb) {
        const unsigned b = (unsigned)pix / (unsigned)HW, p = (unsigned)pix - b * (unsigned)HW;
        float4 v = *reinterpret_cast<const float4*>(x + pix * CIN + sub * 4);
        float4 o = make_float4(0, 0, 0, 0);
#pragma unroll
        for (int co = 0; co < MAX_COUT; ++co) {
            if (co < Cout) {
                float g = dq[((size_t)b * Cout + co) * HW + p];
                o.x += g * wv[co].x; o.y += g * wv[co].y; o.z += g * wv[co].z; o.w += g * wv[co].w;
                gw[co].x += g * v.x; gw[co].y += g * v.y; gw[co].z += g * v.z; gw[co].w += g * v.w;
                gb[co] += g;
            }
        }
        *reinterpret_cast<float4*>(dx + pix * CIN + sub * 4) = o;
    }
    for (int co = 0; co < Cout; ++co) {
        __syncthreads();
        red[threadIdx.x * 4 + 0] = gw[co].x; red[threadIdx.x * 4 + 1] = gw[co].y;
        red[threadIdx.x * 4 + 2] = gw[co].z; red[threadIdx.x * 4 + 3] = gw[co].w;
        __syncthreads();
        if (threadIdx.x < CIN) {
            int s = threadIdx.x / 4, e = threadIdx.x % 4;
            float a = 0.f;
            for (int t = s; t < 256; t += L) a += red[t * 4 + e];
            if (slab_w) slab_w[(size_t)blockIdx.x * Cout * CIN + co * CIN + threadIdx.x] = a;
            else unsafeAtomicAdd(dw + co * CIN + threadIdx.x, a);
        }
        __syncthreads();
        red[threadIdx.x] = (sub == 0) ? gb[co] : 0.f;
        __syncthreads();
        if (threadIdx.x == 0) {
            float a = 0.f;
            for (int t = 0; t < 256; ++t) a += red[t];
            if (slab_b) slab_b[(size_t)blockIdx.x * Cout + co] = a;
            else unsafeAtomicAdd(dbias + co, a);
        }
    }
}

__device__ __forceinline__ void lerp2x(int o, int in_size, float scale, int& i0, int& i1, float& l0, float& l1) {
    const float real = scale * (float)o;
    i0 = (int)real;
    if (i0 > in_size - 1) i0 = in_size - 1;
    i1 = i0 + ((i0 < in_size - 1) ? 1 : 0);
    l1 = fminf(fmaxf(real - (float)i0, 0.f), 1.f);
    l0 = 1.f - l1;
}

__global__ void __launch_bounds__(256) head_up_relu_conv3_kernel(const float* __restrict__ z2, const float* __restrict__ w, float* __restrict__ z,
                                                                  int B, int Cout) {
    constexpr int CIN = 32, L = CIN / 4, W1 = 24, W2 = 48;
    const int sub = threadIdx.x % L;
    float4 wv[MAX_COUT];
    for (int co = 0; co < MAX_COUT; ++co)
        wv[co] = co < Cout ? *reinterpret_cast<const float4*>(w + co * CIN + sub * 4) : make_float4(0, 0, 0, 0);
    const float sc = (float)(W1 - 1) / (float)(W2 - 1);
    const unsigned total = (unsigned)B * W2 * W2, ppb = 256 / L;
    for (unsigned pix = blockIdx.x * ppb + threadIdx.x / L; pix < total; pix += gridDim.x * ppb) {
        const unsigned b = pix / (W2 * W2), p = pix - b * (W2 * W2);
        const int oy = (int)(p / W2), ox = (int)(p - (unsigned)oy * W2);
        int y0, y1, x0, x1;
        float ly0, ly1, lx0, lx1;
        lerp2x(oy, W1, sc, y0, y1, ly0, ly1);
        lerp2x(ox, W1, sc, x0, x1, lx0, lx1);
        const float* base = z2 + (size_t)b * W1 * W1 * CIN + sub * 4;
        const float4 v00 = *reinterpret_cast<const float4*>(base + (y0 * W1 + x0) * CIN), v01 = *reinterpret_cast<const float4*>(base + (y0 * W1 + x1) * CIN);
        const float4 v10 = *reinterpret_cast<const float4*>(base + (y1 * W1 + x0) * CIN), v11 = *reinterpret_cast<const float4*>(base + (y1 * W1 + x1) * CIN);
        float4 v;
        v.x = fmaxf(ly0 * (lx0 * v00.x + lx1 * v01.x) + ly1 * (lx0 * v10.x + lx1 * v11.x), 0.f);
        v.y = fmaxf(ly0 * (lx0 * v00.y + lx1 * v01.y) + ly1 * (lx0 * v10.y + lx1 * v11.y), 0.f);
        v.z = fmaxf(ly0 * (lx0 * v00.z + lx1 * v01.z) + ly1 * (lx0 * v10.z + lx1 * v11.z), 0.f);
        v.w = fmaxf(ly0 * (lx0 * v00.w + lx1 * v01.w) + ly1 * (lx0 * v10.w + lx1 * v11.w), 0.f);
        for (int co = 0; co < Cout; ++co) {
            float s = v.x * wv[co].x + v.y * wv[co].y + v.z * wv[co].z + v.w * wv[co].w;
#pragma unroll
            for (int o = L / 2; o >= 1; o >>= 1) s += __shfl_xor(s, o);
            if (sub == 0) z[((size_t)b * Cout + co) * (W2 * W2) + p] = s;
        }
    }
}

__global__ void __launch_bounds__(32) head_onehot_bwd_kernel(const float* __restrict__ ah2, const float* __restrict__ w3,
                                                             const int64_t* __restrict__ action, const float* __restrict__ q_sa,
                                                             const float* __restrict__ y, float grad_scale, float* ds1, float* dw3,
                                                             float* db3, int Cout, const float* __restrict__ ypre, int ypre_bf16,
                                                             const float* __restrict__ mean, const float* __restrict__ invstd, double* red, int B) {
    constexpr int W2 = 96, W1 = 48, CIN = 32;
    for (int b = blockIdx.x; b < B; b += gridDim.x) {
    const int ci = threadIdx.x;
    const int64_t a = action[b];
    const int co = (int)(a / (W2 * W2)), p = (int)(a - (int64_t)co * W2 * W2);
    if (co >= Cout) continue;
    const int oy = p / W2, ox = p - oy * W2;
    const float d = q_sa[b] - y[b];
    const float g = fminf(fmaxf(d, -1.f), 1.f) * grad_scale;
    const float s = (float)(W1 - 1) / (float)(W2 - 1);
    int y0, y1, x0, x1;
    float ly0, ly1, lx0, lx1;
    lerp2x(oy, W1, s, y0, y1, ly0, ly1);
    lerp2x(ox, W1, s, x0, x1, lx0, lx1);
    const float* src = ah2 + (size_t)b * W1 * W1 * CIN + ci;
    const float up = ly0 * (lx0 * src[(y0 * W1 + x0) * CIN] + lx1 * src[(y0 * W1 + x1) * CIN]) +
                     ly1 * (lx0 * src[(y1 * W1 + x0) * CIN] + lx1 * src[(y1 * W1 + x1) * CIN]);
    unsafeAtomicAdd(dw3 + co * CIN + ci, g * up);
    if (ci == 0) unsafeAtomicAdd(db3 + co, g);
    const float dx = g * w3[co * CIN + ci];
    float* base = ds1 + (size_t)b * W1 * W1 * CIN + ci;
    base[(y0 * W1 + x0) * CIN] += ly0 * lx0 * dx;
    base[(y0 * W1 + x1) * CIN] += ly0 * lx1 * dx;
    base[(y1 * W1 + x0) * CIN] += ly1 * lx0 * dx;
    base[(y1 * W1 + x1) * CIN] += ly1 * lx1 * dx;
    if (!red) continue;
    const float mu = mean[ci], is = invstd[ci];
    float s0 = 0.f, s1 = 0.f;
#pragma unroll
    for (int a = 0; a < 2; ++a) {
        if (a == 1 && y1 == y0) continue;
#pragma unroll
        for (int e = 0; e < 2; ++e) {
            if (e == 1 && x1 == x0) continue;
            const size_t o = ((size_t)b * W1 * W1 + (a ? y1 : y0) * W1 + (e ? x1 : x0)) * CIN + ci;
            const float dz = ah2[o] > 0.f ? ds1[o] : 0.f;
            const float yv = ypre_bf16 ? __uint_as_float((uint32_t)reinterpret_cast<const uint16_t*>(ypre)[o] << 16) : ypre[o];
            s0 += dz;
            s1 += dz * ((yv - mu) * is);
        }
    }
    unsafeAtomicAdd(red + ci, (double)s0);
    unsafeAtomicAdd(red + CIN + ci, (double)s1);
    }
}

__global__ void __launch_bounds__(256) head_upsample_q_kernel(const float* __restrict__ z, const float* __restrict__ bias,
                                                              float* __restrict__ q, int planes, int Cout, int vec) {
    constexpr int W2 = 96, W1 = 48;
    const float s = (float)(W1 - 1) / (float)(W2 - 1);
    const unsigned total = (unsigned)planes * W2 * (W2 / 4);
    for (unsigned i = blockIdx.x * blockDim.x + threadIdx.x; i < total; i += gridDim.x * blockDim.x) {
        const unsigned x4 = i % (W2 / 4), r = i / (W2 / 4);
        const unsigned oy = r % W2, pl = r / W2;
        const float bv = bias[pl % (unsigned)Cout];
        int y0, y1; float ly0, ly1;
        lerp2x((int)oy, W1, s, y0, y1, ly0, ly1);
        const float* r0 = z + (size_t)pl * W1 * W1 + y0 * W1;
        const float* r1 = z + (size_t)pl * W1 * W1 + y1 * W1;
        float o[4];
#pragma unroll
        for (int e = 0; e < 4; ++e) {
            int x0, x1; float lx0, lx1;
            lerp2x((int)x4 * 4 + e, W1, s, x0, x1, lx0, lx1);
            o[e] = ly0 * (lx0 * r0[x0] + lx1 * r0[x1]) + ly1 * (lx0 * r1[x0] + lx1 * r1[x1]) + bv;
        }
        float* dst = q + ((size_t)pl * W2 + oy) * W2 + x4 * 4;
        if (vec) *reinterpret_cast<float4*>(dst) = make_float4(o[0], o[1], o[2], o[3]);
        else { dst[0] = o[0]; dst[1] = o[1]; dst[2] = o[2]; dst[3] = o[3]; }
    }
}

}

int launch_head_upsample_q(const float* z, const float* bias, float* q, int B, int Cout, hipStream_t stream) {
    SIMQ_REQUIRE(Cout >= 1 && Cout <= MAX_COUT, "head_upsample_q: Cout=%d unsupported", Cout);
    SIMQ_REQUIRE((size_t)B * Cout * 9216 < 2147483648ull, "head_upsample_q: too many pixels for 32-bit indexing");
    const unsigned total = (unsigned)B * Cout * 96 * 24;
    unsigned blocks = (total + 255) / 256;
    if (blocks > 4096) blocks = 4096;
    hipLaunchKernelGGL(head_upsample_q_kernel, dim3(blocks), dim3(256), 0, stream, z, bias, q, B * Cout, Cout,
                       (reinterpret_cast<uintptr_t>(q) & 15) == 0 ? 1 : 0);
    SIMQ_CHECK_LAUNCH();
    return 0;
}

int launch_head_onehot_bwd(const float* ah2, const float* w3, const int64_t* action, const float* q_sa, const float* y,
                           float grad_scale, float* ds1, float* dw3, float* db3, int B, int Cout, hipStream_t stream,
                           const float* ypre, int ypre_bf16, const float* mean, const float* invstd, double* red, int serial) {
    SIMQ_REQUIRE(Cout >= 1 && Cout <= MAX_COUT, "head_onehot_bwd: Cout=%d unsupported", Cout);
    SIMQ_CHECK_HIP(hipMemsetAsync(ds1, 0, sizeof(float) * (size_t)B * 48 * 48 * 32, stream));
    hipLaunchKernelGGL(head_onehot_bwd_kernel, dim3(serial ? 1 : B), dim3(32), 0, stream, ah2, w3, action, q_sa, y, grad_scale, ds1, dw3, db3, Cout,
                       ypre, ypre_bf16, mean, invstd, red, B);
    SIMQ_CHECK_LAUNCH();
    return 0;
}

int launch_head_up_relu_conv3(const float* z2, const float* w, float* z, int B, int Cout, hipStream_t stream) {
    SIMQ_REQUIRE(Cout >= 1 && Cout <= MAX_COUT, "head_up_relu_conv3: Cout=%d unsupported", Cout);
    SIMQ_REQUIRE((size_t)B * 2304 < 2147483648ull / 32, "head_up_relu_conv3: too many pixels for 32-bit indexing");
    size_t blocks = ((size_t)B * 2304 + 31) / 32;
    if (blocks > 4096) blocks = 4096;
    hipLaunchKernelGGL(head_up_relu_conv3_kernel, dim3((unsigned)blocks), dim3(256), 0, stream, z2, w, z, B, Cout);
    SIMQ_CHECK_LAUNCH();
    return 0;
}

int launch_head_conv3_fwd(const float* x, const float* w, const float* bias, float* q, int B, int HW, int Cin, int Cout,
                          hipStream_t stream) {
    SIMQ_REQUIRE(Cin == 32 && Cout >= 1 && Cout <= MAX_COUT, "head_conv3: Cin=%d Cout=%d unsupported", Cin, Cout);
    SIMQ_REQUIRE((size_t)B * HW < 2147483648ull, "head_conv3: too many pixels for 32-bit indexing");
    size_t blocks = ((size_t)B * HW + 31) / 32;
    if (blocks > 4096) blocks = 4096;
    hipLaunchKernelGGL(head_conv3_fwd_kernel<32>, dim3((unsigned)blocks), dim3(256), 0, stream, x, w, bias, q, B, HW, Cout);
    SIMQ_CHECK_LAUNCH();
    return 0;
}

int launch_head_conv3_bwd(const float* x, const float* w, const float* dq, float* dx, float* dw, float* dbias, int B,
                          int HW, int Cin, int Cout, hipStream_t stream, float* det_slab) {
    SIMQ_REQUIRE(Cin == 32 && Cout >= 1 && Cout <= MAX_COUT, "head_conv3: Cin=%d Cout=%d unsupported", Cin, Cout);
    SIMQ_REQUIRE((size_t)B * HW < 2147483648ull, "head_conv3: too many pixels for 32-bit indexing");
    size_t blocks = ((size_t)B * HW + 31) / 32;
    if (blocks > 1024) blocks = 1024;
    float* slab_w = det_slab;
    float* slab_b = det_slab ? det_slab + 1024 * MAX_COUT * 32 : nullptr;
    hipLaunchKernelGGL(head_conv3_bwd_kernel<32>, dim3((unsigned)blocks), dim3(256), 0, stream, x, w, dq, dx, dw, dbias, B,
                       HW, Cout, slab_w, slab_b);
    SIMQ_CHECK_LAUNCH();
    if (det_slab) {
        if (int rc = launch_wgrad_slab_sum(slab_w, dw, (int64_t)Cout * 32, (int)blocks, stream)) return rc;
        return launch_wgrad_slab_sum(slab_b, dbias, Cout, (int)blocks, stream);
    }
    return 0;
}

}
```

### spatial-intention-maps_amd/csrc/layout.hip

```cpp
#include <algorithm>
#include <cstdarg>
#include <cstdio>
#include <cstdlib>
#include <cstring>

#include "plan.h"

namespace simq {

static thread_local char g_error[512] = "";

#ifdef SIMQ_ABLATIONS
int tune_env_int(const char* name, int dflt) {
    const char* e = getenv(name);
    return e ? atoi(e) : dflt;
}
#endif

void set_error(const char* fmt, ...) {
    va_list ap;
    va_start(ap, fmt);
    vsnprintf(g_error, sizeof(g_error), fmt, ap);
    va_end(ap);
}

Layout make_layout(const simq_plan* p, int B) {
    Layout L;
    int64_t off = 0;
    auto take = [&](int64_t bytes) { int64_t o = off; off = align_up(off + bytes, 256); return o; };
    const int64_t f = sizeof(float);
    L.x = take((int64_t)B * 96 * 96 * p->cin * f);
    L.y0 = take((int64_t)B * 48 * 48 * 64 * f);
    L.pooled = take((int64_t)B * 576 * 64 * f);
    L.idx = take((int64_t)B * 576 * 64);
    for (int i = 0; i < 8; ++i) {
        const int64_t n = (int64_t)B * 576 * p->blocks[i].planes * f;
        L.blk[i].y1 = take(n); L.blk[i].a1 = take(n); L.blk[i].y2 = take(n);
        L.blk[i].yd = p->blocks[i].has_ds ? take(n) : -1;
        L.blk[i].out = take(n);
    }
    L.yh1 = take((int64_t)B * 576 * 128 * f); L.ah1 = take((int64_t)B * 576 * 128 * f);
    L.up1 = take((int64_t)B * 576 * 32 * f);
    L.yh2 = take((int64_t)B * 2304 * 32 * f); L.ah2 = take((int64_t)B * 2304 * 32 * f);
    L.up2 = take((int64_t)B * 9216 * 32 * f);
    L.aux = take(p->aux_total * f);
    L.red = take(p->red_total * (int64_t)sizeof(double));
    L.colsum = take(2 * kStatReplicas * 2 * 128 * sizeof(double));
    L.defer = take(p->nbnbuf * (int64_t)sizeof(double));
    const int64_t smax = (int64_t)B * 294912 * f;
    for (int i = 0; i < 4; ++i) L.S[i] = take(smax);
    L.p_pooled = L.p_up1 = L.DP[0] = L.DP[1] = L.DP[2] = L.DP2[0] = L.DP2[1] = L.DP2[2] = -1;
    for (int i = 0; i < 8; ++i) L.blk[i].p_a1 = L.blk[i].p_out = -1;
    if (p->precision != SIMQ_PREC_FP32) {
        const int64_t h = (int64_t)sizeof(uint16_t) * p->np();
        L.p_pooled = take((int64_t)B * 576 * 64 * h);
        for (int i = 0; i < 8; ++i) {
            const int64_t n = (int64_t)B * 576 * p->blocks[i].planes * h;
            L.blk[i].p_a1 = take(n);
            L.blk[i].p_out = take(n);
        }
        L.p_up1 = take((int64_t)B * 576 * 128 * h);
        L.DP[0] = take((int64_t)B * 294912 * h);
        L.DP[1] = take((int64_t)B * 294912 * h);
    }
    L.wino = p->wino_scratch_per_sample > 0 ? take(((int64_t)B * p->wino_scratch_per_sample + p->wino_du_floats) * f) : -1;
    L.fwd_total = off;
    L.wino2 = L.wino >= 0 ? take(((int64_t)B * p->wino_scratch_per_sample + p->wino_du_floats) * f) : -1;
    const bool piped_mc = p->precision != SIMQ_PREC_FP32;
    for (int i = 0; i < 3; ++i) L.S2[i] = take(smax);
    if (piped_mc) {
        const int64_t h = (int64_t)sizeof(uint16_t) * p->np();
        L.DP[2] = take((int64_t)B * 294912 * h);
        for (int i = 0; i < 3; ++i) L.DP2[i] = take((int64_t)B * 294912 * h);
    }
    L.wslab = p->precision == SIMQ_PREC_BF16 ? take(conv_wgrad_bf16_slab_bytes()) : -1;
    L.dslab = p->opt.deterministic ? take(kWgradDetSlabFloats * f) : -1;
    L.total = off;
    return L;
}

WLayout make_wlayout(const simq_plan* p) {
    WLayout W;
    W.wt = W.wpl = W.wtpl = W.wu = W.stem16 = -1;
    int64_t off = 0;
    auto take = [&](int64_t bytes) { int64_t o = off; off = align_up(off + bytes, 256); return o; };
    if (p->precision == SIMQ_PREC_FP32) {
        W.wt = take(p->wt_total * (int64_t)sizeof(float));
        if (p->wu_total > 0) W.wu = take(p->wu_total * (int64_t)sizeof(float));
    } else {
        const int64_t h = (int64_t)sizeof(uint16_t) * p->np();
        W.wpl = take(p->wp_total * h);
        W.wtpl = take(p->wp_total * h);
        if (p->precision == SIMQ_PREC_BF16 && p->opt.stem_bf16 &&
            stem_conv_bf16_eligible(96, 96, p->stem.cin, p->stem.cout, p->stem.k, p->stem.stride, p->stem.pad))
            W.stem16 = take(stem_conv_bf16_wbytes());
    }
    W.total = off;
    return W;
}

WeightPrepTable weight_table(const simq_plan* p) {
    WeightPrepTable t;
    t.n = 0;
    (void)for_each_mc_conv(p, [&](const ConvL& cv) {
        WeightPrepDesc& d = t.d[t.n++];
        d.w_off = cv.w_off; d.wt_off = cv.wt_off; d.wp_off = cv.wp_off; d.cout = cv.cout; d.taps = cv.k * cv.k; d.cin = cv.cin; d.pad_ = 0;
        return 0;
    });
    return t;
}

int plan_streams(const simq_plan* plan, PlanStreams** out, int* device) {
    int dev = 0;
    SIMQ_CHECK_HIP(hipGetDevice(&dev));
    if (device) *device = dev;
    *out = (dev >= 0 && dev < kMaxDevices) ? &plan->streams[dev] : nullptr;
    return 0;
}

}

using namespace simq;

namespace {

struct Builder {
    simq_plan* p;
    void conv(ConvL& c, const std::string& name, int cin, int cout, int k, int stride, int pad, bool bias, bool dgrad) {
        c.name = name; c.cin = cin; c.cout = cout; c.k = k; c.stride = stride; c.pad = pad;
        c.w_off = p->nparams;
        p->tensors.push_back({name + ".weight", c.w_off, {cout, k, k, cin}, SIMQ_KIND_CONV_W});
        p->nparams += c.wcount();
        if (bias) {
            c.b_off = p->nparams;
            p->tensors.push_back({name + ".bias", c.b_off, {cout, 1, 1, 1}, SIMQ_KIND_CONV_B});
            p->nparams += cout;
        }
        if (dgrad) { c.wt_off = p->wt_total; p->wt_total += c.wcount(); c.wp_off = p->wp_total; p->wp_total += c.wcount(); }
        if (p->precision == SIMQ_PREC_FP32 && dgrad && k == 3 && stride == 1 && pad == 1 && p->opt.winograd && winograd_pays(cin, cout, p->opt.winograd_min_cc)) {
            ConvGeom g;
            g.B = 1; g.Hin = g.Win = g.Hout = g.Wout = 24; g.Cin = cin; g.Cout = cout; g.R = g.S = 3; g.stride = 1; g.pad = 1;
            ConvGeom gt = g;
            gt.Cin = cout; gt.Cout = cin;
            if (winograd_eligible(g)) {
                p->wino_du_floats = std::max(p->wino_du_floats, 36 * c.wcount() / 9);
                c.wu_off = p->wu_total; p->wu_total += 16 * c.wcount() / 9;
                c.wu4_off = p->wu_total; p->wu_total += 36 * c.wcount() / 9;
                p->wino_scratch_per_sample = std::max(p->wino_scratch_per_sample, winograd_scratch_floats(g));
            }
            if (winograd_eligible(gt)) {
                c.wut_off = p->wu_total; p->wu_total += 16 * c.wcount() / 9;
                if (p->opt.winograd_f4_grad) { c.wut4_off = p->wu_total; p->wu_total += 36 * c.wcount() / 9; }
                p->wino_scratch_per_sample = std::max(p->wino_scratch_per_sample, winograd_scratch_floats(gt));
            }
        }
    }
    void bn(BnL& b, const std::string& name, int C) {
        b.name = name; b.C = C;
        b.g_off = p->nparams; p->tensors.push_back({name + ".weight", b.g_off, {C, 1, 1, 1}, SIMQ_KIND_BN_W}); p->nparams += C;
        b.b_off = p->nparams; p->tensors.push_back({name + ".bias", b.b_off, {C, 1, 1, 1}, SIMQ_KIND_BN_B}); p->nparams += C;
        b.buf_off = p->nbnbuf; p->nbnbuf += 2 * C;
        b.aux_off = p->aux_total; p->aux_total += 4 * C;
        b.red_off = p->red_total; p->red_total += 2 * C;
        p->bns.push_back(&b);
    }
};

int copy_name(const std::string& s, char* dst, int cap) {
    if (!dst || cap <= 0) return 0;
    snprintf(dst, (size_t)cap, "%s", s.c_str());
    return 0;
}

}

extern "C" {

int simq_version(void) { return SIMQ_VERSION; }

int simq_build_flags(void) {
#ifdef SIMQ_ABLATIONS
    return SIMQ_BUILD_ABLATIONS;
#else
    return 0;
#endif
}
const char* simq_last_error(void) { return simq::g_error; }

void simq_plan_options_default(simq_plan_options* o) {
    if (!o) return;
    o->struct_bytes = (int)sizeof(simq_plan_options);
    o->winograd = 1; o->winograd_min_cc = 128 * 128; o->winograd_f4_forward = 1; o->winograd_f4_min_tiles = 256;
    o->winograd_f4_grad = 2; o->winograd_f4_fwd_grad_min_cc = 512 * 512; o->winograd_wgrad = 1; o->winograd_wgrad_f4 = 1;
    o->stem_bf16 = 1; o->bf16_act_grads = 1; o->keep_fp32_activations = 0; o->fold_eval_bn_bf16 = 1;
    o->fuse_bn_backward_sums = 1; o->fuse_stem_backward_sums = 1;
    o->fuse_bn1_apply = 1; o->bn1_mask_from_preact = 1; o->deterministic = 0;
    o->wgrad_ksplit = 0; o->fwd_overlap = 2; o->wgrad_overlap = 4; o->plane_xcd = 1; o->wgrad_xcd_group = 1; o->tail_split = 0;
    o->early_target_after_block = 4;
    o->gemm_split = 1;
}

void simq_launch_opts_default(simq_launch_opts* o) {
    if (!o) return;
    const LaunchTune t;
    o->struct_bytes = (int)sizeof(simq_launch_opts);
    o->force_bm = t.force_bm; o->force_bn = t.force_bn; o->tail_split = t.tail_split; o->plane_xcd = t.plane_xcd;
    o->wgrad_xcd_group = t.wgrad_xcd_group; o->wgrad_ksplit = t.wgrad_ksplit; o->gemm_split = t.gemm_split;
}

int simq_plan_get_options(const simq_plan* plan, simq_plan_options* out) {
    SIMQ_REQUIRE(plan && out, "plan_get_options: NULL argument");
    *out = plan->opt;
    return 0;
}

int simq_plan_create_ex(int cin, int cout, int precision, simq_plan** out) { return simq_plan_create_opts(cin, cout, precision, nullptr, out); }

int simq_plan_create_opts(int cin, int cout, int precision, const simq_plan_options* opts, simq_plan** out) {
    SIMQ_REQUIRE(out != nullptr, "plan_create: out is NULL");
    simq_plan_options opt;
    simq_plan_options_default(&opt);
    if (opts) {
        SIMQ_REQUIRE(opts->struct_bytes == (int)sizeof(simq_plan_options), "plan_create: simq_plan_options.struct_bytes = %d, this library's struct has %d "
                     "(fill it with simq_plan_options_default first)", opts->struct_bytes, (int)sizeof(simq_plan_options));
        opt = *opts;
        SIMQ_REQUIRE(opt.winograd_f4_grad >= 0 && opt.winograd_f4_grad <= 2, "plan_create: winograd_f4_grad = %d (0, 1 or 2)", opt.winograd_f4_grad);
        SIMQ_REQUIRE(opt.winograd_min_cc >= 64 * 64, "plan_create: winograd_min_cc = %d below 64*64 (layer1 does not fit the transform table)", opt.winograd_min_cc);
        SIMQ_REQUIRE(opt.winograd_f4_min_tiles >= 1, "plan_create: winograd_f4_min_tiles = %d", opt.winograd_f4_min_tiles);
        SIMQ_REQUIRE(opt.wgrad_ksplit == 0 || opt.wgrad_ksplit == 1 || opt.wgrad_ksplit == 2 || opt.wgrad_ksplit == 4, "plan_create: wgrad_ksplit = %d (0, 1, 2 or 4)", opt.wgrad_ksplit);
        SIMQ_REQUIRE(opt.fwd_overlap >= 0 && opt.fwd_overlap <= 2, "plan_create: fwd_overlap = %d (0, 1 or 2)", opt.fwd_overlap);
        SIMQ_REQUIRE(opt.wgrad_overlap >= 0 && opt.wgrad_overlap <= 4, "plan_create: wgrad_overlap = %d (0 .. 4)", opt.wgrad_overlap);
        SIMQ_REQUIRE(opt.wgrad_xcd_group >= 0 && opt.wgrad_xcd_group <= 2, "plan_create: wgrad_xcd_group = %d (0, 1 or 2)", opt.wgrad_xcd_group);
        SIMQ_REQUIRE(opt.early_target_after_block >= -1 && opt.early_target_after_block <= 7, "plan_create: early_target_after_block = %d (-1 .. 7)",
                     opt.early_target_after_block);
        SIMQ_REQUIRE(opt.gemm_split == 0 || opt.gemm_split == 1, "plan_create: gemm_split = %d (0 or 1)", opt.gemm_split);
    }
    SIMQ_REQUIRE(cin >= 1 && cin <= 64, "plan_create: num_input_channels=%d out of range", cin);
    SIMQ_REQUIRE(cout >= 1 && cout <= 4, "plan_create: num_output_channels=%d out of range [1,4]", cout);
    SIMQ_REQUIRE(precision >= SIMQ_PREC_FP32 && precision <= SIMQ_PREC_BF16, "plan_create: bad precision %d", precision);
    simq_plan* p = new simq_plan();
    p->cin = cin; p->cout = cout; p->precision = precision; p->opt = opt;
    Builder bd{p};
    bd.conv(p->stem, "resnet18.conv1", cin, 64, 7, 2, 3, false, false);
    bd.bn(p->stem_bn, "resnet18.bn1", 64);
    int inplanes = 64, bi = 0;
    const int planes_of[4] = {64, 128, 256, 512};
    for (int li = 0; li < 4; ++li) {
        for (int k = 0; k < 2; ++k, ++bi) {
            BlockL& b = p->blocks[bi];
            const int planes = planes_of[li];
            const int bcin = k == 0 ? inplanes : planes;
            char nm[64];
            snprintf(nm, sizeof(nm), "resnet18.layer%d.%d.", li + 1, k);
            b.cin = bcin; b.planes = planes; b.has_ds = (k == 0 && bcin != planes);
            bd.conv(b.c1, std::string(nm) + "conv1", bcin, planes, 3, 1, 1, false, true);
            bd.bn(b.b1, std::string(nm) + "bn1", planes);
            bd.conv(b.c2, std::string(nm) + "conv2", planes, planes, 3, 1, 1, false, true);
            bd.bn(b.b2, std::string(nm) + "bn2", planes);
            if (b.has_ds) {
                bd.conv(b.ds, std::string(nm) + "downsample.0", bcin, planes, 1, 1, 0, false, true);
                bd.bn(b.bds, std::string(nm) + "downsample.1", planes);
            }
        }
        inplanes = planes_of[li];
    }
    bd.conv(p->h1, "conv1", 512, 128, 1, 1, 0, true, true);
    bd.bn(p->hb1, "bn1", 128);
    bd.conv(p->h2, "conv2", 128, 32, 1, 1, 0, true, true);
    bd.bn(p->hb2, "bn2", 32);
    p->hb2_rep_off = p->red_total; p->red_total += kStatReplicas * 2 * 32;
    p->stem_rep_off = p->red_total; p->red_total += kStatReplicas * 2 * 64;
    bd.conv(p->h3, "conv3", 32, cout, 1, 1, 0, true, false);
    for (const TensorInfo& t : p->tensors)
        if (t.kind == SIMQ_KIND_CONV_W && (t.off % 4) != 0) {
            set_error("plan_create: tensor %s not 16-byte aligned in the flat buffer", t.name.c_str());
            delete p;
            return -1;
        }
    *out = p;
    return 0;
}

int simq_plan_create(int cin, int cout, simq_plan** out) { return simq_plan_create_ex(cin, cout, SIMQ_PREC_FP32, out); }

void simq_plan_destroy(simq_plan* plan) {
    if (!plan) return;
    for (int d = 0; d < kMaxDevices; ++d) {
        PlanStreams& s = plan->streams[d];
        hipStream_t* streams[3] = {&s.bwd_side, &s.third, &s.copy};
        for (hipStream_t* st : streams)
            if (*st) { (void)hipStreamDestroy(*st); *st = nullptr; }
        hipEvent_t* events[] = {&s.bwd_ev[0], &s.bwd_ev[1], &s.bwd_ev[2], &s.bwd_ev[3], &s.third_ev, &s.step_ev[0], &s.step_ev[1], &s.step_ev[2],
                                &s.step_ev[3], &s.step_ev[4], &s.step_ev[5], &s.step_ev[6], &s.copy_ready, &s.copy_done};
        for (hipEvent_t* ev : events)
            if (*ev) { (void)hipEventDestroy(*ev); *ev = nullptr; }
    }
    (void)hipGetLastError();
    delete plan;
}

int simq_plan_precision(const simq_plan* plan) { return plan ? plan->precision : -1; }

int64_t simq_param_count(const simq_plan* plan) { return plan ? plan->nparams : -1; }
int simq_param_num_tensors(const simq_plan* plan) { return plan ? (int)plan->tensors.size() : -1; }

int simq_param_tensor_info(const simq_plan* plan, int index, char* name, int name_cap, int64_t* offset, int64_t shape[4], int* kind) {
    SIMQ_REQUIRE(plan && index >= 0 && index < (int)plan->tensors.size(), "param_tensor_info: bad index %d", index);
    const TensorInfo& t = plan->tensors[index];
    copy_name(t.name, name, name_cap);
    if (offset) *offset = t.off;
    if (shape) for (int i = 0; i < 4; ++i) shape[i] = t.shape[i];
    if (kind) *kind = t.kind;
    return 0;
}

int64_t simq_bnbuf_count(const simq_plan* plan) { return plan ? plan->nbnbuf : -1; }
int simq_bn_num_layers(const simq_plan* plan) { return plan ? (int)plan->bns.size() : -1; }

int simq_bn_layer_info(const simq_plan* plan, int index, char* name, int name_cap, int64_t* offset, int* channels) {
    SIMQ_REQUIRE(plan && index >= 0 && index < (int)plan->bns.size(), "bn_layer_info: bad index %d", index);
    const BnL* b = plan->bns[index];
    copy_name(b->name, name, name_cap);
    if (offset) *offset = b->buf_off;
    if (channels) *channels = b->C;
    return 0;
}

int64_t simq_workspace_bytes(const simq_plan* plan, int batch) {
    if (!plan || batch < 1) return -1;
    return make_layout(plan, batch).total;
}

int64_t simq_workspace_bytes_forward(const simq_plan* plan, int batch) {
    if (!plan || batch < 1) return -1;
    return make_layout(plan, batch).fwd_total;
}

int simq_workspace_tensor(const simq_plan* plan, int batch, const char* name, int64_t* byte_offset, int64_t* elems, int* channels) {
    SIMQ_REQUIRE(plan && name && batch >= 1, "workspace_tensor: bad argument");
    const Layout L = make_layout(plan, batch);
    const std::string n(name);
    int64_t off = -1, cnt = 0;
    int ch = 0;
    if (n == "stem.conv") { off = L.y0; ch = 64; cnt = (int64_t)batch * 2304 * 64; }
    else if (n == "stem.pool") { off = L.pooled; ch = 64; cnt = (int64_t)batch * 576 * 64; }
    else if (n == "head.a1") {
        SIMQ_REQUIRE(plan->precision != SIMQ_PREC_FP32 || !plan->opt.fuse_bn1_apply || !plan->opt.fuse_bn_backward_sums,
                     "workspace_tensor: head.a1 is not stored by this plan (simq_plan_options.fuse_bn1_apply: the head's BatchNorm 1 + ReLU is "
                     "applied inside conv2's operand staging); create the plan with fuse_bn1_apply = 0 to inspect it");
        off = L.ah1; ch = 128; cnt = (int64_t)batch * 576 * 128;
    }
    else if (n == "head.a2") { off = L.ah2; ch = 32; cnt = (int64_t)batch * 2304 * 32; }
    else {
        int li = 0, bi = 0;
        if (sscanf(name, "layer%d.%d", &li, &bi) == 2 && li >= 1 && li <= 4 && bi >= 0 && bi <= 1) {
            const int i = (li - 1) * 2 + bi;
            off = L.blk[i].out; ch = plan->blocks[i].planes; cnt = (int64_t)batch * 576 * ch;
        }
    }
    SIMQ_REQUIRE(off >= 0, "workspace_tensor: unknown tensor '%s'", name);
    if (byte_offset) *byte_offset = off;
    if (elems) *elems = cnt;
    if (channels) *channels = ch;
    return 0;
}

int simq_workspace_tensor_ex(const simq_plan* plan, int batch, const char* name, int64_t* byte_offset, int64_t* elems, int* channels, int* storage) {
    SIMQ_REQUIRE(plan && name && batch >= 1, "workspace_tensor_ex: bad argument");
    const Layout L = make_layout(plan, batch);
    const bool mc = plan->precision != SIMQ_PREC_FP32, ybf = plan->precision == SIMQ_PREC_BF16;
    const bool planes_only = mc && !plan->opt.keep_fp32_activations && plan->opt.fuse_bn_backward_sums;
    int li = 0, bi = 0;
    char what[32] = "";
    int64_t off = -1, cnt = 0;
    int ch = 0, st = 0;
    if (sscanf(name, "layer%d.%d.%31s", &li, &bi, what) == 3 && li >= 1 && li <= 4 && bi >= 0 && bi <= 1) {
        const int i = (li - 1) * 2 + bi;
        const BlockL& b = plan->blocks[i];
        const Layout::Blk& o = L.blk[i];
        const std::string w(what);
        ch = b.planes; cnt = (int64_t)batch * 576 * ch;
        auto bnaux = [&](const BnL& bn) { off = L.aux + bn.aux_off * (int64_t)sizeof(float); cnt = 4 * (int64_t)bn.C; ch = bn.C; st = 0; };
        if (w == "y1") { off = o.y1; st = ybf; }
        else if (w == "y2") { off = o.y2; st = ybf; }
        else if (w == "yd" && b.has_ds) { off = o.yd; st = ybf; }
        else if (w == "a1") { off = planes_only ? o.p_a1 : o.a1; st = planes_only ? 1 : 0; }
        else if (w == "out") { off = planes_only ? o.p_out : o.out; st = planes_only ? 1 : 0; }
        else if (w == "bn1") bnaux(b.b1);
        else if (w == "bn2") bnaux(b.b2);
        else if (w == "bnd" && b.has_ds) bnaux(b.bds);
        auto bnred = [&](const BnL& bn) { off = L.red + bn.red_off * (int64_t)sizeof(double); cnt = 2 * (int64_t)bn.C; ch = bn.C; st = 2; };
        if (w == "red1") bnred(b.b1);
        else if (w == "red2") bnred(b.b2);
        else if (w == "redd" && b.has_ds) bnred(b.bds);
        if ((w == "a1") && plan->precision == SIMQ_PREC_FP32 && plan->opt.fuse_bn1_apply && plan->opt.fuse_bn_backward_sums) off = -1;
    } else if (std::string(name) == "stem.pool.plane" && mc) {
        off = L.p_pooled; ch = 64; cnt = (int64_t)batch * 576 * 64; st = 1;
    } else {
        const std::string n(name);
        const bool stem16 = make_wlayout(plan).stem16 >= 0;
        auto bnaux = [&](const BnL& bn) { off = L.aux + bn.aux_off * (int64_t)sizeof(float); cnt = 4 * (int64_t)bn.C; ch = bn.C; st = 0; };
        if (n == "stem.y0") { off = L.y0; ch = 64; cnt = (int64_t)batch * 2304 * 64; st = stem16 ? 1 : 0; }
        else if (n == "stem.bn") bnaux(plan->stem_bn);
        else if (n == "stem.idx") { off = L.idx; ch = 64; cnt = (int64_t)batch * 576 * 64; st = 3; }
        else if (n == "head.y1") { off = L.yh1; ch = 128; cnt = (int64_t)batch * 576 * 128; st = (ybf && plan->h1.wp_off >= 0) ? 1 : 0; }
        else if (n == "head.bn1") bnaux(plan->hb1);
        else if (n == "head.a1.plane" && mc) { off = L.p_up1; ch = 128; cnt = (int64_t)batch * 576 * 128; st = 1; }
        else if (n == "head.z2") { off = L.up1; ch = 32; cnt = (int64_t)batch * 576 * 32; }
        else if (n == "head.y2") { off = L.yh2; ch = 32; cnt = (int64_t)batch * 2304 * 32; }
        else if (n == "head.bn2") bnaux(plan->hb2);
        else if (n == "head.z3") { off = L.up2; ch = plan->cout; cnt = (int64_t)batch * 2304 * plan->cout; }
        auto bnred = [&](const BnL& bn) { off = L.red + bn.red_off * (int64_t)sizeof(double); cnt = 2 * (int64_t)bn.C; ch = bn.C; st = 2; };
        if (n == "stem.red") bnred(plan->stem_bn);
        else if (n == "head.red1") bnred(plan->hb1);
        else if (n == "head.red2") bnred(plan->hb2);
    }
    SIMQ_REQUIRE(off >= 0, "workspace_tensor_ex: '%s' is not a tensor this plan stores", name);
    if (byte_offset) *byte_offset = off;
    if (elems) *elems = cnt;
    if (channels) *channels = ch;
    if (storage) *storage = st;
    return 0;
}

int64_t simq_wcache_bytes(const simq_plan* plan) { return plan ? make_wlayout(plan).total : -1; }

int simq_weights_prepare(const simq_plan* plan, const float* d_params, void* d_wcache, void* stream) {
    SIMQ_REQUIRE(plan && d_params && d_wcache, "weights_prepare: NULL argument");
    const WLayout W = make_wlayout(plan);
    char* wc = static_cast<char*>(d_wcache);
    if (plan->precision == SIMQ_PREC_FP32) {
        RC(launch_weight_prep_all(d_params, weight_table(plan), reinterpret_cast<float*>(wc + W.wt), nullptr, nullptr, 1, 0,
                                  static_cast<hipStream_t>(stream)));
        if (W.wu < 0) return 0;
        WinoWeightTable t;
        t.n = 0;
        RC(for_each_mc_conv(plan, [&](const ConvL& cv) {
            SIMQ_REQUIRE(t.n + 4 <= kWinoWeightTableCap, "weights_prepare: more Winograd layers than the transform table holds");
            if (cv.wu_off >= 0) t.d[t.n++] = WinoWeightDesc{cv.w_off, cv.wu_off, cv.cout, cv.cin, 0, 0};
            if (cv.wu4_off >= 0) t.d[t.n++] = WinoWeightDesc{cv.w_off, cv.wu4_off, cv.cout, cv.cin, 0, 1};
            if (cv.wut_off >= 0) t.d[t.n++] = WinoWeightDesc{cv.wt_off, cv.wut_off, cv.cin, cv.cout, 1, 0};
            if (cv.wut4_off >= 0) t.d[t.n++] = WinoWeightDesc{cv.wt_off, cv.wut4_off, cv.cin, cv.cout, 1, 1};
            return 0;
        }));
        return launch_wino_weight_all(d_params, reinterpret_cast<const float*>(wc + W.wt), reinterpret_cast<float*>(wc + W.wu), t,
                                      static_cast<hipStream_t>(stream));
    }
    RC(launch_weight_prep_all(d_params, weight_table(plan), nullptr, reinterpret_cast<uint16_t*>(wc + W.wpl),
                              reinterpret_cast<uint16_t*>(wc + W.wtpl), plan->np(), plan->wp_total, static_cast<hipStream_t>(stream)));
    if (W.stem16 >= 0)
        RC(launch_stem_weight_prep(d_params + plan->stem.w_off, reinterpret_cast<uint16_t*>(wc + W.stem16), plan->stem.cin,
                                   static_cast<hipStream_t>(stream)));
    return 0;
}

}
```

### spatial-intention-maps_amd/csrc/ops_abi.hip

```cpp
#include "plan.h"

using namespace simq;

namespace {
int tune_of(const simq_launch_opts* o, LaunchTune* t) {
    *t = LaunchTune();
    if (!o) return 0;
    SIMQ_REQUIRE(o->struct_bytes == (int)sizeof(simq_launch_opts), "simq_launch_opts.struct_bytes = %d, this library's struct has %d (fill it with "
                 "simq_launch_opts_default first)", o->struct_bytes, (int)sizeof(simq_launch_opts));
    t->force_bm = o->force_bm > 0 ? o->force_bm : 0; t->force_bn = o->force_bm > 0 ? o->force_bn : 0;
    t->tail_split = o->tail_split; t->plane_xcd = o->plane_xcd; t->wgrad_xcd_group = o->wgrad_xcd_group; t->wgrad_ksplit = o->wgrad_ksplit;
    t->gemm_split = o->gemm_split;
    return 0;
}
}

extern "C" {

int simq_q_argmax(const float* d_q, int rows, int n, int64_t* d_index, float* d_max, void* stream) {
    SIMQ_REQUIRE(rows >= 0 && n >= 1, "q_argmax: bad shape");
    return launch_q_argmax(d_q, rows, n, d_index, d_max, static_cast<hipStream_t>(stream));
}

int simq_q_gather(const float* d_q, int rows, int n, const int64_t* d_index, float* d_out, void* stream) {
    SIMQ_REQUIRE(rows >= 0 && n >= 1, "q_gather: bad shape");
    return launch_q_gather(d_q, rows, n, d_index, d_out, static_cast<hipStream_t>(stream));
}

int simq_scatter_next_values(const float* d_values, const int32_t* d_nonfinal_pos, int n_nonfinal, float* d_nsv, int batch, void* stream) {
    return launch_scatter_next_values(d_values, d_nonfinal_pos, n_nonfinal, d_nsv, batch, static_cast<hipStream_t>(stream));
}

int simq_td_huber(const float* d_q, int batch, int n, const int64_t* d_action, const float* d_reward, const float* d_nsv,
                  float gamma, float grad_scale, float* d_q_sa, float* d_y, float* d_td_error, float* d_out4, float* d_dq, void* stream) {
    SIMQ_REQUIRE(batch >= 1 && n >= 1, "td_huber: bad shape");
    return launch_td_huber(d_q, batch, n, d_action, d_reward, d_nsv, gamma, grad_scale, d_q_sa, d_y, d_td_error, d_out4, d_dq,
                           static_cast<hipStream_t>(stream));
}

int simq_clip_sgd_step(float* d_params, float* d_grads, float* d_momentum, int64_t count, float max_norm, float lr,
                       float momentum, float weight_decay, int first_step, void* d_scratch, float* d_total_norm, void* stream) {
    SIMQ_REQUIRE(d_params && d_grads && d_momentum && d_scratch && count > 0, "clip_sgd_step: bad argument");
    return launch_clip_sgd(d_params, d_grads, d_momentum, count, max_norm, lr, momentum, weight_decay, first_step, d_scratch,
                           d_total_norm, static_cast<hipStream_t>(stream));
}

int simq_bce_with_logits(const float* d_logits, const float* d_target, int64_t n, float* d_dlogits, double* d_loss_sum, void* stream) {
    SIMQ_REQUIRE(d_logits && d_target && d_loss_sum && n > 0, "bce_with_logits: bad argument");
    return launch_bce_logits(d_logits, d_target, n, d_dlogits, d_loss_sum, static_cast<hipStream_t>(stream));
}

int simq_split_last_channel(const float* d_x, float* d_head, float* d_last, int64_t pixels, int channels, void* stream) {
    SIMQ_REQUIRE(d_x && d_head && d_last && pixels > 0 && channels >= 2, "split_last_channel: bad argument");
    return launch_split_last_channel(d_x, d_head, d_last, pixels, channels, static_cast<hipStream_t>(stream));
}

int simq_sigmoid_concat(const float* d_state, const float* d_logit, float* d_out, float* d_prob, int64_t pixels, int channels, void* stream) {
    SIMQ_REQUIRE(d_state && d_logit && d_out && pixels > 0 && channels >= 1, "sigmoid_concat: bad argument");
    return launch_sigmoid_concat(d_state, d_logit, d_out, d_prob, pixels, channels, static_cast<hipStream_t>(stream));
}

int simq_replay_gather(const float* d_ring, int64_t item_floats, const int64_t* d_index, int count, float* d_out, void* stream) {
    return launch_replay_gather(d_ring, item_floats, d_index, count, d_out, static_cast<hipStream_t>(stream));
}

int simq_nchw_to_nhwc(const float* d_in, float* d_out, int batch, int channels, int hw, void* stream) {
    return launch_nchw_to_nhwc(d_in, d_out, batch, channels, hw, static_cast<hipStream_t>(stream));
}

int simq_nhwc_to_nchw(const float* d_in, float* d_out, int batch, int channels, int hw, void* stream) {
    return launch_nhwc_to_nchw(d_in, d_out, batch, channels, hw, static_cast<hipStream_t>(stream));
}

int simq_conv2d_fwd(const float* d_x, const float* d_w, const float* d_bias, float* d_y, int batch, int hin, int win,
                    int cin, int cout, int r, int s, int stride, int pad, double* d_stats, void* stream, const simq_launch_opts* opts) {
    ConvGeom g;
    RC(tune_of(opts, &g.tune));
    g.B = batch; g.Hin = hin; g.Win = win; g.Cin = cin; g.Cout = cout; g.R = r; g.S = s; g.stride = stride; g.pad = pad;
    g.Hout = (hin + 2 * pad - r) / stride + 1; g.Wout = (win + 2 * pad - s) / stride + 1;
    ConvEpilogue e;
    e.bias = d_bias; e.stats = d_stats;
    return launch_conv_igemm(d_x, d_w, d_y, g, e, static_cast<hipStream_t>(stream));
}

int simq_conv2d_fwd_winograd(const float* d_x, const float* d_w, const float* d_bias, float* d_y, int batch, int hin, int win,
                             int cin, int cout, double* d_stats, float* d_scratch, void* stream, const simq_launch_opts* opts) {
    SIMQ_REQUIRE(d_x && d_w && d_y && d_scratch && batch >= 1, "conv2d_fwd_winograd: bad argument");
    ConvGeom g;
    RC(tune_of(opts, &g.tune));
    g.B = batch; g.Hin = hin; g.Win = win; g.Cin = cin; g.Cout = cout; g.R = 3; g.S = 3; g.stride = 1; g.pad = 1; g.Hout = hin; g.Wout = win;
    SIMQ_REQUIRE(winograd_eligible(g), "conv2d_fwd_winograd: geometry not supported (even map, cin %% 16, cout %% 64)");
    ConvEpilogue e;
    e.bias = d_bias; e.stats = d_stats;
    hipStream_t st = static_cast<hipStream_t>(stream);
    RC(launch_wino_weight(d_w, d_scratch, cout, cin, st));
    return launch_conv_winograd(d_x, d_scratch, d_y, g, e, d_scratch + (size_t)16 * cout * cin, st);
}

int simq_bn_relu_apply(const void* d_y, const double* d_stats, const float* d_gamma, const float* d_beta, const void* d_res, int relu, void* d_out,
                       int64_t rows, int channels, int storage, float* d_saved, float* d_running, void* stream) {
    SIMQ_REQUIRE(d_y && d_stats && d_gamma && d_beta && d_out && d_saved && d_running && rows >= 1 && channels >= 4, "bn_relu_apply: bad argument");
    SIMQ_REQUIRE(storage == 0 || storage == 1, "bn_relu_apply: storage %d (0 fp32, 1 bf16)", storage);
    BnRef r;
    r.stats = d_stats; r.gamma = d_gamma; r.beta = d_beta;
    r.rmean = d_running; r.rvar = d_running + channels;
    r.save_scale = d_saved; r.save_shift = d_saved + channels; r.save_mean = d_saved + 2 * channels; r.save_invstd = d_saved + 3 * channels;
    r.rows = (double)rows; r.inv_rows = 1.0 / r.rows; r.C = channels;
    hipStream_t st = static_cast<hipStream_t>(stream);
    if (storage == 0)
        return launch_bn_apply(static_cast<const float*>(d_y), r, static_cast<const float*>(d_res), nullptr, relu, static_cast<float*>(d_out), rows, channels, st);
    Planes out, res;
    out.hi = static_cast<uint16_t*>(d_out);
    res.hi = static_cast<uint16_t*>(const_cast<void*>(d_res));
    return launch_bn_apply(static_cast<const float*>(d_y), r, nullptr, nullptr, relu, nullptr, rows, channels, st, out, res, 1);
}

int simq_bn_relu_backward(const void* d_g, const void* d_mask, int mask_kind, const void* d_y, const float* d_saved, const float* d_gamma,
                          const double* d_red, void* d_dy, void* d_dz_out, float* d_dgamma, float* d_dbeta, int64_t rows, int channels,
                          int storage, void* stream) {
    SIMQ_REQUIRE(d_g && d_y && d_saved && d_gamma && d_red && d_dy && d_dgamma && d_dbeta && rows >= 1 && channels >= 4, "bn_relu_backward: bad argument");
    SIMQ_REQUIRE((storage == 0 || storage == 1) && mask_kind >= 0 && mask_kind <= 2 && (mask_kind != 1 || d_mask), "bn_relu_backward: storage %d / mask_kind %d", storage, mask_kind);
    const float* mean = d_saved + 2 * channels;
    const float* invstd = d_saved + 3 * channels;
    const float* msc = mask_kind == 2 ? d_saved : nullptr;
    const float* msh = mask_kind == 2 ? d_saved + channels : nullptr;
    hipStream_t st = static_cast<hipStream_t>(stream);
    if (storage == 0)
        return launch_bn_bwd_apply(static_cast<const float*>(d_g), mask_kind == 1 ? static_cast<const float*>(d_mask) : nullptr, static_cast<const float*>(d_y),
                                   mean, invstd, d_gamma, d_red, static_cast<float*>(d_dy), static_cast<float*>(d_dz_out), d_dgamma, d_dbeta, rows, channels,
                                   st, Planes(), nullptr, 0, 0.0, 1.f, 0, msc, msh);
    Planes dy;
    dy.hi = static_cast<uint16_t*>(d_dy);
    return launch_bn_bwd_apply(static_cast<const float*>(d_g), nullptr, static_cast<const float*>(d_y), mean, invstd, d_gamma, d_red, nullptr,
                               static_cast<float*>(d_dz_out), d_dgamma, d_dbeta, rows, channels, st, dy,
                               mask_kind == 1 ? static_cast<const uint16_t*>(d_mask) : nullptr, 1, 0.0, 1.f, 1, msc, msh);
}

int simq_conv2d_fwd_bnrelu_in(const float* d_y_pre, const float* d_in_scale, const float* d_in_shift, const float* d_w, const float* d_bias,
                              float* d_y, int batch, int hin, int win, int cin, int cout, int r, int s, int stride, int pad, int form,
                              float* d_scratch, void* stream, const simq_launch_opts* opts) {
    SIMQ_REQUIRE(d_y_pre && d_in_scale && d_in_shift && d_w && d_y && batch >= 1, "conv2d_fwd_bnrelu_in: bad argument");
    SIMQ_REQUIRE(form >= 0 && form <= 2 && (form == 0 || d_scratch), "conv2d_fwd_bnrelu_in: form %d (0 direct, 1 F(2x2,3x3), 2 F(4x4,3x3) with scratch)", form);
    ConvGeom g;
    RC(tune_of(opts, &g.tune));
    g.B = batch; g.Hin = hin; g.Win = win; g.Cin = cin; g.Cout = cout; g.R = r; g.S = s; g.stride = stride; g.pad = pad;
    g.Hout = (hin + 2 * pad - r) / stride + 1; g.Wout = (win + 2 * pad - s) / stride + 1;
    ConvEpilogue e;
    e.bias = d_bias;
    InBn in; in.scale = d_in_scale; in.shift = d_in_shift;
    hipStream_t st = static_cast<hipStream_t>(stream);
    if (form == 0) {
        SIMQ_REQUIRE(cin % 16 == 0, "conv2d_fwd_bnrelu_in: cin %% 16 == 0 (cin=%d)", cin);
        return launch_conv_igemm(d_y_pre, d_w, d_y, g, e, st, in);
    }
    SIMQ_REQUIRE(winograd_eligible(g) && (form == 1 || (hin % 4 == 0 && win % 4 == 0)), "conv2d_fwd_bnrelu_in: geometry not supported by the Winograd forms");
    WinoWeightTable t;
    t.n = 1;
    t.d[0] = WinoWeightDesc{0, 0, cout, cin, 0, form == 2 ? 1 : 0};
    RC(launch_wino_weight_all(d_w, nullptr, d_scratch, t, st));
    const size_t planes = form == 2 ? 36 : 16;
    if (form == 2) return launch_conv_winograd4(d_y_pre, d_scratch, d_y, g, e, d_scratch + planes * cout * cin, st, in);
    return launch_conv_winograd(d_y_pre, d_scratch, d_y, g, e, d_scratch + planes * cout * cin, st, in);
}

int simq_conv2d_wgrad_bnrelu_in(const float* d_y_pre, const float* d_in_scale, const float* d_in_shift, const float* d_dy, float* d_dw,
                                int batch, int hin, int win, int cin, int cout, int r, int s, int stride, int pad, int form,
                                float* d_scratch, void* stream, const simq_launch_opts* opts) {
    SIMQ_REQUIRE(d_y_pre && d_in_scale && d_in_shift && d_dy && d_dw && batch >= 1, "conv2d_wgrad_bnrelu_in: bad argument");
    SIMQ_REQUIRE(form == 0 || (form == 1 && d_scratch), "conv2d_wgrad_bnrelu_in: form %d (0 direct, 1 transform domain with scratch)", form);
    ConvGeom g;
    RC(tune_of(opts, &g.tune));
    g.B = batch; g.Hin = hin; g.Win = win; g.Cin = cin; g.Cout = cout; g.R = r; g.S = s; g.stride = stride; g.pad = pad;
    g.Hout = (hin + 2 * pad - r) / stride + 1; g.Wout = (win + 2 * pad - s) / stride + 1;
    InBn in; in.scale = d_in_scale; in.shift = d_in_shift;
    hipStream_t st = static_cast<hipStream_t>(stream);
    if (form == 1) {
        SIMQ_REQUIRE(winograd_wgrad_eligible(g), "conv2d_wgrad_bnrelu_in: geometry not supported (even map, cin %% 128, cout %% 128)");
        return launch_conv_wgrad_winograd(d_y_pre, d_dy, d_dw, g, d_scratch, st, true, in);
    }
    SIMQ_CHECK_HIP(hipMemsetAsync(d_dw, 0, sizeof(float) * (size_t)cout * r * s * cin, st));
    return launch_conv_wgrad(d_y_pre, d_dy, d_dw, g, st, in);
}

int simq_conv2d_fwd_stem_f32(const float* d_x, const float* d_w, float* d_y, int batch, int hin, int win, int cin, double* d_stats, void* stream) {
    SIMQ_REQUIRE(d_x && d_w && d_y && batch >= 1, "conv2d_fwd_stem_f32: bad argument");
    SIMQ_REQUIRE(stem_conv_f32_eligible(hin, win, cin, 64, 7, 2, 3), "conv2d_fwd_stem_f32: geometry not supported (7 * cin <= 64, win %% 32 == 0)");
    return launch_stem_conv_f32(d_x, d_w, d_y, d_stats, batch, hin, win, cin, static_cast<hipStream_t>(stream));
}

int simq_conv2d_fwd_stem_bf16(const float* d_x, const float* d_w, uint16_t* d_y, int batch, int hin, int win, int cin, double* d_stats,
                              void* d_scratch, void* stream) {
    SIMQ_REQUIRE(d_x && d_w && d_y && d_scratch && batch >= 1, "conv2d_fwd_stem_bf16: bad argument");
    SIMQ_REQUIRE(stem_conv_bf16_eligible(hin, win, cin, 64, 7, 2, 3), "conv2d_fwd_stem_bf16: geometry not supported (7 * cin <= 63, win %% 32 == 0)");
    hipStream_t st = static_cast<hipStream_t>(stream);
    RC(launch_stem_weight_prep(d_w, static_cast<uint16_t*>(d_scratch), cin, st));
    return launch_stem_conv_bf16(d_x, static_cast<const uint16_t*>(d_scratch), d_y, d_stats, batch, hin, win, cin, st);
}

int simq_conv2d_wgrad_stem_bf16(const float* d_x, const uint16_t* d_dy, float* d_dw, int batch, int hin, int win, int cin, float* d_scratch,
                                void* stream) {
    SIMQ_REQUIRE(d_x && d_dy && d_dw && d_scratch && batch >= 1, "conv2d_wgrad_stem_bf16: bad argument");
    SIMQ_REQUIRE(stem_conv_bf16_eligible(hin, win, cin, 64, 7, 2, 3), "conv2d_wgrad_stem_bf16: geometry not supported (7 * cin <= 63, win %% 32 == 0)");
    return launch_stem_wgrad_bf16(d_x, d_dy, d_dw, d_scratch, batch, hin, win, cin, static_cast<hipStream_t>(stream));
}

int simq_conv2d_fwd_winograd4(const float* d_x, const float* d_w, const float* d_bias, float* d_y, int batch, int hin, int win,
                              int cin, int cout, double* d_stats, float* d_scratch, void* stream, const simq_launch_opts* opts) {
    SIMQ_REQUIRE(d_x && d_w && d_y && d_scratch && batch >= 1, "conv2d_fwd_winograd4: bad argument");
    ConvGeom g;
    RC(tune_of(opts, &g.tune));
    g.B = batch; g.Hin = hin; g.Win = win; g.Cin = cin; g.Cout = cout; g.R = 3; g.S = 3; g.stride = 1; g.pad = 1; g.Hout = hin; g.Wout = win;
    SIMQ_REQUIRE(winograd_eligible(g) && hin % 4 == 0 && win % 4 == 0, "conv2d_fwd_winograd4: geometry not supported (map %% 4, cin %% 16, cout %% 64)");
    ConvEpilogue e;
    e.bias = d_bias; e.stats = d_stats;
    hipStream_t st = static_cast<hipStream_t>(stream);
    WinoWeightTable t;
    t.n = 1;
    t.d[0] = WinoWeightDesc{0, 0, cout, cin, 0, 1};
    RC(launch_wino_weight_all(d_w, nullptr, d_scratch, t, st));
    return launch_conv_winograd4(d_x, d_scratch, d_y, g, e, d_scratch + (size_t)36 * cout * cin, st);
}

int simq_conv2d_wgrad_winograd(const float* d_x, const float* d_dy, float* d_dw, int batch, int hin, int win, int cin, int cout,
                               float* d_scratch, void* stream, const simq_launch_opts* opts) {
    SIMQ_REQUIRE(d_x && d_dy && d_dw && d_scratch && batch >= 1, "conv2d_wgrad_winograd: bad argument");
    ConvGeom g;
    RC(tune_of(opts, &g.tune));
    g.B = batch; g.Hin = hin; g.Win = win; g.Cin = cin; g.Cout = cout; g.R = 3; g.S = 3; g.stride = 1; g.pad = 1; g.Hout = hin; g.Wout = win;
    SIMQ_REQUIRE(winograd_wgrad_eligible(g), "conv2d_wgrad_winograd: geometry not supported (even map, cin %% 128, cout %% 128)");
    return launch_conv_wgrad_winograd(d_x, d_dy, d_dw, g, d_scratch, static_cast<hipStream_t>(stream));
}

int simq_gemm_f32_batched(const float* d_x, const float* d_w, float* d_y, int m, int n, int k, int batch, void* stream, const simq_launch_opts* opts) {
    SIMQ_REQUIRE(d_x && d_w && d_y, "gemm_f32_batched: NULL argument");
    LaunchTune t;
    RC(tune_of(opts, &t));
    return launch_gemm_batched(d_x, d_w, d_y, m, n, k, batch, static_cast<hipStream_t>(stream), t);
}

int simq_conv2d_dgrad(const float* d_dy, const float* d_w, float* d_wt_scratch, float* d_dx, int batch, int hin, int win,
                      int cin, int cout, int r, int s, int pad, void* stream, const simq_launch_opts* opts) {
    hipStream_t st = static_cast<hipStream_t>(stream);
    SIMQ_REQUIRE(r == s, "conv2d_dgrad: square filters only");
    RC(launch_weight_transpose(d_w, d_wt_scratch, cout, r * s, cin, st));
    ConvGeom g;
    RC(tune_of(opts, &g.tune));
    g.B = batch; g.Hin = hin; g.Win = win; g.Cin = cout; g.Cout = cin; g.Hout = hin; g.Wout = win;
    g.R = r; g.S = s; g.stride = 1; g.pad = r - 1 - pad;
    ConvEpilogue e;
    return launch_conv_igemm(d_dy, d_wt_scratch, d_dx, g, e, st);
}

int simq_conv2d_wgrad(const float* d_x, const float* d_dy, float* d_dw, int batch, int hin, int win, int cin, int cout,
                      int r, int s, int stride, int pad, void* stream, const simq_launch_opts* opts) {
    hipStream_t st = static_cast<hipStream_t>(stream);
    ConvGeom g;
    RC(tune_of(opts, &g.tune));
    g.B = batch; g.Hin = hin; g.Win = win; g.Cin = cin; g.Cout = cout; g.R = r; g.S = s; g.stride = stride; g.pad = pad;
    g.Hout = (hin + 2 * pad - r) / stride + 1; g.Wout = (win + 2 * pad - s) / stride + 1;
    SIMQ_CHECK_HIP(hipMemsetAsync(d_dw, 0, sizeof(float) * (size_t)cout * r * s * cin, st));
    return launch_conv_wgrad(d_x, d_dy, d_dw, g, st);
}

int simq_conv2d_fwd_bf16(const float* d_x, const float* d_w, const float* d_bias, float* d_y, int batch, int hin, int win,
                         int cin, int cout, int r, int s, int stride, int pad, int nplanes, void* d_scratch, double* d_stats,
                         void* stream, const simq_launch_opts* opts) {
    hipStream_t st = static_cast<hipStream_t>(stream);
    ConvGeom g;
    RC(tune_of(opts, &g.tune));
    g.B = batch; g.Hin = hin; g.Win = win; g.Cin = cin; g.Cout = cout; g.R = r; g.S = s; g.stride = stride; g.pad = pad;
    g.Hout = (hin + 2 * pad - r) / stride + 1; g.Wout = (win + 2 * pad - s) / stride + 1;
    const int64_t nx = (int64_t)batch * hin * win * cin, nw = (int64_t)cout * r * s * cin;
    uint16_t* base = static_cast<uint16_t*>(d_scratch);
    uint16_t* xp[2] = {base, base + nx};
    uint16_t* wp[2] = {base + 2 * nx, base + 2 * nx + nw};
    RC(launch_split_planes(d_x, xp[0], nplanes == 2 ? xp[1] : nullptr, nx, st));
    RC(launch_split_planes(d_w, wp[0], nplanes == 2 ? wp[1] : nullptr, nw, st));
    ConvEpilogue e;
    e.bias = d_bias; e.stats = d_stats;
    return launch_conv_igemm_bf16(xp, wp, nplanes, d_y, g, e, st);
}

int64_t simq_conv2d_wgrad_bf16_slab_bytes(void) { return conv_wgrad_bf16_slab_bytes(); }

int simq_conv2d_wgrad_bf16(const float* d_x, const float* d_dy, float* d_dw, int batch, int hin, int win, int cin, int cout,
                           int r, int s, int stride, int pad, int nplanes, void* d_scratch, void* stream, const simq_launch_opts* opts) {
    return simq_conv2d_wgrad_bf16_slab(d_x, d_dy, d_dw, batch, hin, win, cin, cout, r, s, stride, pad, nplanes, d_scratch, nullptr, stream, opts);
}

int simq_conv2d_wgrad_bf16_slab(const float* d_x, const float* d_dy, float* d_dw, int batch, int hin, int win, int cin, int cout,
                                int r, int s, int stride, int pad, int nplanes, void* d_scratch, void* d_slab, void* stream, const simq_launch_opts* opts) {
    hipStream_t st = static_cast<hipStream_t>(stream);
    ConvGeom g;
    RC(tune_of(opts, &g.tune));
    g.B = batch; g.Hin = hin; g.Win = win; g.Cin = cin; g.Cout = cout; g.R = r; g.S = s; g.stride = stride; g.pad = pad;
    g.Hout = (hin + 2 * pad - r) / stride + 1; g.Wout = (win + 2 * pad - s) / stride + 1;
    const int64_t nx = (int64_t)batch * hin * win * cin, ny = (int64_t)batch * g.Hout * g.Wout * cout;
    uint16_t* base = static_cast<uint16_t*>(d_scratch);
    uint16_t* xp[2] = {base, base + nx};
    uint16_t* yp[2] = {base + 2 * nx, base + 2 * nx + ny};
    RC(launch_split_planes(d_x, xp[0], nplanes == 2 ? xp[1] : nullptr, nx, st));
    RC(launch_split_planes(d_dy, yp[0], nplanes == 2 ? yp[1] : nullptr, ny, st));
    SIMQ_CHECK_HIP(hipMemsetAsync(d_dw, 0, sizeof(float) * (size_t)cout * r * s * cin, st));
    return launch_conv_wgrad_bf16(xp, yp, nplanes, d_dw, g, st, static_cast<float*>(d_slab));
}

int simq_upsample2x_fwd(const float* d_in, float* d_out, int batch, int h, int w, int c, void* stream) {
    return launch_upsample2x_fwd(d_in, d_out, batch, h, w, c, static_cast<hipStream_t>(stream));
}

int simq_upsample2x_bwd(const float* d_dout, float* d_din, int batch, int h, int w, int c, void* stream) {
    return launch_upsample2x_bwd(d_dout, d_din, batch, h, w, c, static_cast<hipStream_t>(stream));
}

}
```

### spatial-intention-maps_amd/csrc/plan.h

```cpp
#pragma once
#include <mutex>
#include <string>
#include <vector>

#include "../../include/simq.h"
#include "common.h"

namespace simq {

constexpr int kStatReplicas = 16;

struct ConvL {
    std::string name;
    int64_t w_off = -1, b_off = -1;
    int64_t wt_off = -1;
    int64_t wp_off = -1;
    int64_t wu_off = -1, wut_off = -1;
    int64_t wu4_off = -1, wut4_off = -1;
    int cin = 0, cout = 0, k = 1, stride = 1, pad = 0;
    int64_t wcount() const { return (int64_t)cout * k * k * cin; }
};

struct BnL {
    std::string name;
    int64_t g_off = -1, b_off = -1;
    int64_t buf_off = -1;
    int64_t aux_off = -1;
    int64_t red_off = -1;
    int C = 0;
};

struct BlockL {
    ConvL c1, c2, ds;
    BnL b1, b2, bds;
    bool has_ds = false;
    int cin = 0, planes = 0;
};

struct TensorInfo { std::string name; int64_t off; int64_t shape[4]; int kind; };

struct PlanStreams {
    hipStream_t bwd_side = nullptr;
    hipStream_t bwd_side_ext = nullptr;
    hipEvent_t bwd_ev[4] = {nullptr, nullptr, nullptr, nullptr};
    hipStream_t third = nullptr;
    hipEvent_t third_ev = nullptr;
    hipEvent_t step_ev[7] = {nullptr, nullptr, nullptr, nullptr, nullptr, nullptr, nullptr};
    bool late_recorded = false;
    hipStream_t copy = nullptr;
    hipEvent_t copy_ready = nullptr, copy_done = nullptr;
    bool copy_pending = false;
};
constexpr int kMaxDevices = 64;

}

struct simq_plan {
    int cin, cout;
    int precision = SIMQ_PREC_FP32;
    simq_plan_options opt;
    int np() const { return precision == SIMQ_PREC_BF16X3 ? 2 : 1; }
    simq::ConvL stem, h1, h2, h3;
    simq::BnL stem_bn, hb1, hb2;
    simq::BlockL blocks[8];
    std::vector<simq::TensorInfo> tensors;
    std::vector<simq::BnL*> bns;
    int64_t nparams = 0, nbnbuf = 0, wt_total = 0, wp_total = 0, aux_total = 0, red_total = 0, wu_total = 0;
    int64_t stem_rep_off = -1;
    int64_t hb2_rep_off = -1;
    int64_t wino_scratch_per_sample = 0;
    int64_t wino_du_floats = 0;
    mutable std::mutex mu;
    mutable simq::PlanStreams streams[simq::kMaxDevices];
    simq::LaunchTune tune() const {
        simq::LaunchTune t;
        t.tail_split = opt.tail_split; t.plane_xcd = opt.plane_xcd; t.wgrad_xcd_group = opt.wgrad_xcd_group; t.wgrad_ksplit = opt.wgrad_ksplit;
        t.gemm_split = opt.gemm_split;
        return t;
    }
};

namespace simq {

inline int64_t align_up(int64_t v, int64_t a) { return (v + a - 1) / a * a; }

struct Layout {
    int64_t x, y0, pooled, idx;
    struct Blk { int64_t y1, a1, y2, yd, out, p_a1, p_out; } blk[8];
    int64_t yh1, ah1, up1, yh2, ah2, up2;
    int64_t aux, red, colsum;
    int64_t defer;
    int64_t S[4];
    int64_t p_pooled, p_up1, DP[3];
    int64_t DP2[3];
    int64_t wino;
    int64_t wino2;
    int64_t S2[3];
    int64_t wslab;
    int64_t dslab;
    int64_t fwd_total;
    int64_t total;
};

Layout make_layout(const simq_plan* p, int B);

struct WLayout { int64_t wt = -1, wpl = -1, wtpl = -1, wu = -1, stem16 = -1, total = 0; };
WLayout make_wlayout(const simq_plan* p);

struct Act {
    float* f = nullptr;
    Planes pl;
    bool fv = true;
};

struct Ctx {
    const simq_plan* p;
    int B;
    const float* params;
    float* grads;
    float* bnbuf;
    char* ws;
    Layout L;
    hipStream_t stream;
    char* wc = nullptr;
    WLayout W = WLayout();
    const simq_sync* sync = nullptr;
    bool defer_running = false;
    hipStream_t wstream = nullptr;
    hipEvent_t ev_wfork = nullptr, ev_wjoin = nullptr;
    hipEvent_t ev_wdone[2] = {nullptr, nullptr};
    const float* x_ext = nullptr;
    hipEvent_t ev_late = nullptr; int late_block = -1;
    char* trace = nullptr;
    double bn_rows(int64_t rows) const { return sync ? (double)rows / (double)B * (double)sync->global_batch : (double)rows; }
    int sync_reduce(double* buf, int64_t count) const { return sync ? sync->reduce(sync->user, buf, count, stream) : 0; }
    float* f(int64_t off) const { return reinterpret_cast<float*>(ws + off); }
    float* aux(const BnL& b, int which) const { return f(L.aux) + b.aux_off + (int64_t)which * b.C; }
    double* red(const BnL& b) const { return reinterpret_cast<double*>(ws + L.red) + b.red_off; }
    bool mc() const { return p->precision != SIMQ_PREC_FP32; }
    int ybf() const { return p->precision == SIMQ_PREC_BF16 ? 1 : 0; }
    int ybf(const ConvL& cv) const { return (p->precision == SIMQ_PREC_BF16 && cv.wp_off >= 0) ? 1 : 0; }
    int gbf() const { return (p->precision == SIMQ_PREC_BF16 && p->opt.bf16_act_grads) ? 1 : 0; }
    Planes planes(int64_t off, int64_t elems) const {
        Planes pl;
        if (mc() && off >= 0) {
            pl.hi = reinterpret_cast<uint16_t*>(ws + off);
            pl.lo = p->np() == 2 ? pl.hi + elems : nullptr;
        }
        return pl;
    }
    Act act(int64_t off, int64_t poff, int64_t elems) const { Act a; a.f = f(off); a.pl = planes(poff, elems); return a; }
    bool planes_only() const { return mc() && !p->opt.keep_fp32_activations && p->opt.fuse_bn_backward_sums; }
    Act block_act(int64_t off, int64_t poff, int64_t elems) const { Act a = act(off, poff, elems); a.fv = !planes_only(); return a; }
    bool lazy1() const { return !mc() && p->opt.fuse_bn1_apply && p->opt.fuse_bn_backward_sums; }
    bool mask1_from_y() const {
        return lazy1() || (p->precision == SIMQ_PREC_BF16 && p->opt.bn1_mask_from_preact && planes_only());
    }
    float* dslab() const { return L.dslab >= 0 ? f(L.dslab) : nullptr; }
    InBn inbn_saved(const BnL& b) const { InBn in; in.scale = aux(b, 0); in.shift = aux(b, 1); return in; }
    void wplanes(const ConvL& cv, bool transposed, const uint16_t* out[2]) const {
        uint16_t* base = reinterpret_cast<uint16_t*>(wc + (transposed ? W.wtpl : W.wpl));
        out[0] = base + cv.wp_off;
        out[1] = p->np() == 2 ? base + p->wp_total + cv.wp_off : out[0];
    }
};

inline ConvGeom geom(const simq_plan* p, const ConvL& c, int B, int hin) {
    ConvGeom g;
    g.tune = p->tune();
    g.B = B; g.Hin = hin; g.Win = hin; g.Cin = c.cin; g.Cout = c.cout; g.R = c.k; g.S = c.k; g.stride = c.stride; g.pad = c.pad;
    g.Hout = (hin + 2 * c.pad - c.k) / c.stride + 1; g.Wout = g.Hout;
    return g;
}

#define RC(expr) do { int _rc = (expr); if (_rc) return _rc; } while (0)

template <typename F>
int for_each_mc_conv(const simq_plan* p, F fn) {
    for (int i = 0; i < 8; ++i) {
        RC(fn(p->blocks[i].c1)); RC(fn(p->blocks[i].c2));
        if (p->blocks[i].has_ds) RC(fn(p->blocks[i].ds));
    }
    RC(fn(p->h1)); RC(fn(p->h2));
    return 0;
}

WeightPrepTable weight_table(const simq_plan* p);

int forward_impl(const Ctx& c, int mode, const float* d_x, float* d_q);

constexpr int kPhaseSplitBlock = 6;

struct OneHotGrad { const int64_t* action; const float* q_sa; const float* y; float grad_scale; };

struct TraceLayout {
    struct Blk { int64_t g_out, dy2, t1, da1, dy1, g_ds, g_in; } blk[8];
    struct Head { int64_t da2, dy2, dz2, da1, dy1; } head;
    struct Stem { int64_t dz, dy0; } stem;
    int64_t total;
};
TraceLayout make_trace_layout(const simq_plan* p, int B);

int backward_impl(const Ctx& c, const float* d_dq, int phase, const OneHotGrad* oh = nullptr);
int backward_sync_side(const simq_plan* plan, int batch, const float* d_params, const void* d_wcache, const float* d_dq,
                       const int64_t* d_action, const float* d_q_sa, const float* d_y, float grad_scale, float* d_grads,
                       void* d_workspace, int phase, void* stream, const simq_sync* sync, hipStream_t wstream, hipEvent_t ev_wfork,
                       hipEvent_t ev_wjoin, hipEvent_t ev_wdone0 = nullptr, hipEvent_t ev_wdone1 = nullptr, const float* x_ext = nullptr,
                       hipEvent_t ev_late = nullptr, int late_block = -1);
int forward_sync_inplace(const simq_plan* plan, int batch, const float* d_params, const void* d_wcache, float* d_bnbuf, const float* d_x,
                         float* d_q, void* d_workspace, hipStream_t stream, const simq_sync* sync);
int check_sync(const simq_sync* sync, int batch);

int plan_streams(const simq_plan* plan, PlanStreams** out, int* device = nullptr);

}
```

### spatial-intention-maps_amd/simq/_lib.py

```python
import ctypes
import os
from ctypes import POINTER, c_char_p, c_double, c_float, c_int, c_int64, c_void_p

import torch

_HERE = os.path.dirname(os.path.abspath(__file__))
LIB_PATH = os.environ.get('SIMQ_LIBRARY') or os.path.join(_HERE, 'libsimq.so')

MODE_EVAL, MODE_TRAIN, MODE_TRAIN_NOGRAD = 0, 1, 2
KIND_CONV_W, KIND_CONV_B, KIND_BN_W, KIND_BN_B = 0, 1, 2, 3
PRECISIONS = {'fp32': 0, 'bf16x3': 1, 'bf16': 2}
COMM_ID_BYTES, COMM_F32, COMM_F64 = 128, 0, 1


class SimqError(RuntimeError):
    pass


if not os.path.exists(LIB_PATH):
    raise SimqError('libsimq.so not found at %s -- build it with `python -c "import __graft_entry__ as g; g.build()"` '
                    '(or `make -C spatial-intention-maps_amd/csrc`); there is no CPU fallback' % LIB_PATH)

_c = ctypes.CDLL(LIB_PATH)

REDUCE_FN = ctypes.CFUNCTYPE(c_int, c_void_p, c_void_p, c_int64, c_void_p)


class SyncArgs(ctypes.Structure):
    _fields_ = [('reduce', REDUCE_FN), ('user', c_void_p), ('global_batch', c_int), ('world_size', c_int)]


class PlanOptions(ctypes.Structure):
    _fields_ = [(n, c_int) for n in (
        'struct_bytes', 'winograd', 'winograd_min_cc', 'winograd_f4_forward', 'winograd_f4_min_tiles', 'winograd_f4_grad',
        'winograd_f4_fwd_grad_min_cc', 'winograd_wgrad', 'winograd_wgrad_f4', 'stem_bf16', 'bf16_act_grads', 'keep_fp32_activations', 'fold_eval_bn_bf16',
        'fuse_bn_backward_sums', 'fuse_stem_backward_sums', 'fuse_bn1_apply', 'deterministic', 'bn1_mask_from_preact',
        'wgrad_ksplit', 'fwd_overlap', 'wgrad_overlap', 'plane_xcd', 'wgrad_xcd_group', 'tail_split', 'early_target_after_block', 'gemm_split')]


class LaunchOpts(ctypes.Structure):
    _fields_ = [(n, c_int) for n in ('struct_bytes', 'force_bm', 'force_bn', 'tail_split', 'plane_xcd', 'wgrad_xcd_group', 'wgrad_ksplit', 'gemm_split')]


class TrainArgs(ctypes.Structure):
    _fields_ = [('plan', c_void_p),
                ('batch', c_int), ('num_nonfinal', c_int), ('global_batch', c_int), ('use_double_dqn', c_int), ('first_step', c_int),
                ('sync_bn', c_int),
                ('gamma', c_float), ('lr', c_float), ('momentum', c_float), ('weight_decay', c_float), ('max_norm', c_float),
                ('reserved2_', c_float)] + [(n, c_void_p) for n in (
                    'params', 'wcache', 'bnbuf', 'grads', 'momentum_buf', 'ws_train', 'ws_tmp',
                    't_params', 't_wcache', 't_bnbuf', 't_ws',
                    'state', 'next_state', 'action', 'reward', 'nonfinal_pos',
                    'q', 'q_next', 'q_tgt', 'dq', 'nsv', 'vals', 'best', 'q_sa', 'y', 'td', 'out4',
                    'opt_scratch', 'total_norm', 'stream', 'side_stream')] + [('global_nonfinal', c_int), ('struct_bytes', c_int), ('comm', c_void_p), ('loss_host', c_void_p), ('target_stream', c_void_p), ('third_stream', c_void_p)]


_SIGS = {
    'simq_version': (c_int, []),
    'simq_build_flags': (c_int, []),
    'simq_last_error': (c_char_p, []),
    'simq_plan_create': (c_int, [c_int, c_int, POINTER(c_void_p)]),
    'simq_plan_create_ex': (c_int, [c_int, c_int, c_int, POINTER(c_void_p)]),
    'simq_plan_options_default': (None, [c_void_p]),
    'simq_launch_opts_default': (None, [c_void_p]),
    'simq_plan_create_opts': (c_int, [c_int, c_int, c_int, c_void_p, POINTER(c_void_p)]),
    'simq_plan_get_options': (c_int, [c_void_p, c_void_p]),
    'simq_plan_precision': (c_int, [c_void_p]),
    'simq_plan_destroy': (None, [c_void_p]),
    'simq_param_count': (c_int64, [c_void_p]),
    'simq_param_num_tensors': (c_int, [c_void_p]),
    'simq_param_tensor_info': (c_int, [c_void_p, c_int, c_char_p, c_int, POINTER(c_int64), POINTER(c_int64 * 4), POINTER(c_int)]),
    'simq_bnbuf_count': (c_int64, [c_void_p]),
    'simq_bn_num_layers': (c_int, [c_void_p]),
    'simq_bn_layer_info': (c_int, [c_void_p, c_int, c_char_p, c_int, POINTER(c_int64), POINTER(c_int)]),
    'simq_workspace_bytes': (c_int64, [c_void_p, c_int]),
    'simq_workspace_bytes_forward': (c_int64, [c_void_p, c_int]),
    'simq_workspace_tensor': (c_int, [c_void_p, c_int, c_char_p, POINTER(c_int64), POINTER(c_int64), POINTER(c_int)]),
    'simq_workspace_tensor_ex': (c_int, [c_void_p, c_int, c_char_p, POINTER(c_int64), POINTER(c_int64), POINTER(c_int), POINTER(c_int)]),
    'simq_wcache_bytes': (c_int64, [c_void_p]),
    'simq_weights_prepare': (c_int, [c_void_p, c_void_p, c_void_p, c_void_p]),
    'simq_forward': (c_int, [c_void_p, c_int, c_int, c_void_p, c_void_p, c_void_p, c_void_p, c_void_p, c_void_p, c_void_p]),
    'simq_backward': (c_int, [c_void_p, c_int, c_void_p, c_void_p, c_void_p, c_void_p, c_void_p, c_void_p]),
    'simq_backward_phase': (c_int, [c_void_p, c_int, c_void_p, c_void_p, c_void_p, c_void_p, c_void_p, c_int, c_void_p]),
    'simq_grad_bucket_split': (c_int64, [c_void_p]),
    'simq_backward_trace_bytes': (c_int64, [c_void_p, c_int]),
    'simq_backward_trace_tensor': (c_int, [c_void_p, c_int, c_char_p, POINTER(c_int64), POINTER(c_int64), POINTER(c_int), POINTER(c_int)]),
    'simq_backward_traced': (c_int, [c_void_p, c_int, c_void_p, c_void_p, c_void_p, c_void_p, c_void_p, c_void_p, c_void_p]),
    'simq_train_step': (c_int, [c_void_p]),
    'simq_train_loss_wait': (c_int, [c_void_p]),
    'simq_plan_adopt_side_stream': (c_int, [c_void_p, c_void_p]),
    'simq_backward_onehot': (c_int, [c_void_p, c_int, c_void_p, c_void_p, c_void_p, c_void_p, c_void_p, c_float, c_void_p, c_void_p, c_int, c_void_p]),
    'simq_q_argmax': (c_int, [c_void_p, c_int, c_int, c_void_p, c_void_p, c_void_p]),
    'simq_q_gather': (c_int, [c_void_p, c_int, c_int, c_void_p, c_void_p, c_void_p]),
    'simq_scatter_next_values': (c_int, [c_void_p, c_void_p, c_int, c_void_p, c_int, c_void_p]),
    'simq_td_huber': (c_int, [c_void_p, c_int, c_int, c_void_p, c_void_p, c_void_p, c_float, c_float,
                              c_void_p, c_void_p, c_void_p, c_void_p, c_void_p, c_void_p]),
    'simq_clip_sgd_step': (c_int, [c_void_p, c_void_p, c_void_p, c_int64, c_float, c_float, c_float, c_float, c_int,
                                   c_void_p, c_void_p, c_void_p]),
    'simq_bce_with_logits': (c_int, [c_void_p, c_void_p, c_int64, c_void_p, c_void_p, c_void_p]),
    'simq_split_last_channel': (c_int, [c_void_p, c_void_p, c_void_p, c_int64, c_int, c_void_p]),
    'simq_sigmoid_concat': (c_int, [c_void_p, c_void_p, c_void_p, c_void_p, c_int64, c_int, c_void_p]),
    'simq_replay_gather': (c_int, [c_void_p, c_int64, c_void_p, c_int, c_void_p, c_void_p]),
    'simq_nchw_to_nhwc': (c_int, [c_void_p, c_void_p, c_int, c_int, c_int, c_void_p]),
    'simq_nhwc_to_nchw': (c_int, [c_void_p, c_void_p, c_int, c_int, c_int, c_void_p]),
    'simq_conv2d_fwd': (c_int, [c_void_p, c_void_p, c_void_p, c_void_p] + [c_int] * 9 + [c_void_p, c_void_p] + [c_void_p]),
    'simq_gemm_f32_batched': (c_int, [c_void_p, c_void_p, c_void_p, c_int, c_int, c_int, c_int, c_void_p, c_void_p]),
    'simq_conv2d_dgrad': (c_int, [c_void_p, c_void_p, c_void_p, c_void_p] + [c_int] * 8 + [c_void_p] + [c_void_p]),
    'simq_conv2d_wgrad': (c_int, [c_void_p, c_void_p, c_void_p] + [c_int] * 9 + [c_void_p] + [c_void_p]),
    'simq_conv2d_fwd_bf16': (c_int, [c_void_p, c_void_p, c_void_p, c_void_p] + [c_int] * 10 + [c_void_p, c_void_p, c_void_p] + [c_void_p]),
    'simq_conv2d_wgrad_bf16': (c_int, [c_void_p, c_void_p, c_void_p] + [c_int] * 10 + [c_void_p, c_void_p] + [c_void_p]),
    'simq_conv2d_wgrad_bf16_slab_bytes': (c_int64, []),
    'simq_conv2d_wgrad_bf16_slab': (c_int, [c_void_p, c_void_p, c_void_p] + [c_int] * 10 + [c_void_p, c_void_p, c_void_p] + [c_void_p]),
    'simq_upsample2x_fwd': (c_int, [c_void_p, c_void_p, c_int, c_int, c_int, c_int, c_void_p]),
    'simq_upsample2x_bwd': (c_int, [c_void_p, c_void_p, c_int, c_int, c_int, c_int, c_void_p]),
    'simq_profile_start': (c_int, []),
    'simq_profile_stop': (c_int, [c_void_p, c_int]),
    'simq_launch_counts_reset': (c_int, []),
    'simq_launch_count': (c_int64, [c_char_p]),
    'simq_launch_counts': (c_int, [c_char_p, c_int]),
    'simq_conv2d_wgrad_winograd': (c_int, [c_void_p, c_void_p, c_void_p] + [c_int] * 5 + [c_void_p, c_void_p] + [c_void_p]),
    'simq_conv2d_fwd_winograd': (c_int, [c_void_p, c_void_p, c_void_p, c_void_p] + [c_int] * 5 + [c_void_p, c_void_p, c_void_p] + [c_void_p]),
    'simq_conv2d_fwd_winograd4': (c_int, [c_void_p, c_void_p, c_void_p, c_void_p] + [c_int] * 5 + [c_void_p, c_void_p, c_void_p] + [c_void_p]),
    'simq_bn_relu_apply': (c_int, [c_void_p] * 5 + [c_int, c_void_p, c_int64, c_int, c_int, c_void_p, c_void_p, c_void_p]),
    'simq_bn_relu_backward': (c_int, [c_void_p, c_void_p, c_int] + [c_void_p] * 8 + [c_int64, c_int, c_int, c_void_p]),
    'simq_conv2d_fwd_bnrelu_in': (c_int, [c_void_p] * 6 + [c_int] * 10 + [c_void_p, c_void_p] + [c_void_p]),
    'simq_conv2d_wgrad_bnrelu_in': (c_int, [c_void_p] * 5 + [c_int] * 10 + [c_void_p, c_void_p] + [c_void_p]),
    'simq_conv2d_fwd_stem_f32': (c_int, [c_void_p, c_void_p, c_void_p] + [c_int] * 4 + [c_void_p, c_void_p]),
    'simq_conv2d_fwd_stem_bf16': (c_int, [c_void_p, c_void_p, c_void_p] + [c_int] * 4 + [c_void_p, c_void_p, c_void_p]),
    'simq_conv2d_wgrad_stem_bf16': (c_int, [c_void_p, c_void_p, c_void_p] + [c_int] * 4 + [c_void_p, c_void_p]),
    'simq_forward_sync': (c_int, [c_void_p, c_int, c_int, c_void_p, c_void_p, c_void_p, c_void_p, c_void_p, c_void_p, c_void_p, c_void_p]),
    'simq_backward_sync': (c_int, [c_void_p, c_int, c_void_p, c_void_p, c_void_p, c_void_p, c_void_p, c_void_p, c_float, c_void_p, c_void_p,
                                   c_int, c_void_p, c_void_p]),
    'simq_comm_reduce_f64': (c_int, [c_void_p, c_void_p, c_int64, c_void_p]),
    'simq_forward_sync_null': (c_int, [c_void_p, c_int, c_void_p, c_void_p, c_void_p, c_void_p]),
    'simq_comm_unique_id': (c_int, [c_void_p]),
    'simq_comm_init': (c_int, [c_void_p, c_int, c_int, POINTER(c_void_p)]),
    'simq_comm_adopt_stream': (c_int, [c_void_p, c_void_p]),
    'simq_comm_world_size': (c_int, [c_void_p]),
    'simq_comm_rank': (c_int, [c_void_p]),
    'simq_comm_allreduce': (c_int, [c_void_p, c_void_p, c_int64, c_int, c_void_p]),
    'simq_comm_broadcast': (c_int, [c_void_p, c_void_p, c_int64, c_int, c_void_p]),
    'simq_comm_wait': (c_int, [c_void_p, c_void_p]),
    'simq_comm_progress': (c_int, [c_void_p, c_void_p]),
    'simq_comm_time_waits': (c_int, [c_void_p, c_int]),
    'simq_comm_last_wait_ms': (c_int, [c_void_p, POINTER(c_float)]),
    'simq_comm_destroy': (c_int, [c_void_p]),
    'simq_grid_distance_images': (c_int, [c_void_p, c_int64, c_void_p, c_int, c_void_p, c_void_p, c_int64, c_float, c_int, c_float,
                                          c_void_p, c_void_p]),
    'simq_grid_paths': (c_int, [c_void_p, c_int64, c_void_p, c_int64, c_void_p, c_int, c_void_p, c_void_p, c_int64, c_void_p, c_void_p, c_void_p,
                                c_int64, c_void_p, c_int64, c_void_p, c_void_p]),
    'simq_grid_distance_queries': (c_int, [c_void_p, c_int64, c_void_p, c_int64, c_void_p, c_int, c_void_p, c_int64, c_void_p, c_void_p, c_int64,
                                           c_int, c_void_p, c_int64, c_void_p, c_void_p]),
    'simq_local_state_desc_bytes': (c_int64, [c_int, c_int, c_int, c_int]),
    'simq_local_state_images': (c_int, [c_void_p, c_int, c_void_p, c_int, c_void_p, c_int, c_void_p, c_int, c_void_p, c_int, c_void_p, c_int64,
                                        c_void_p, c_int64, c_void_p]),
    'simq_intention_desc_bytes': (c_int64, [c_int, c_int]),
    'simq_intention_maps': (c_int, [c_void_p, c_int, c_void_p, c_int, c_int, c_int, c_int, c_void_p, c_int64, c_void_p, c_int64, c_void_p]),
    'simq_occupancy_maps': (c_int, [c_void_p, c_int64, c_void_p, c_int, c_void_p, c_void_p, c_void_p, c_int64, c_void_p, c_int64, c_void_p,
                                    c_void_p]),
    'simq_observation_update': (c_int, [c_void_p, c_int64, c_void_p, c_int, c_void_p, c_void_p, c_int64, c_void_p, c_int64, c_void_p, c_void_p]),
    'simq_state_output_visualizations': (c_int, [c_void_p, c_int, c_void_p, c_void_p, c_double, c_int, c_void_p, c_int64, c_void_p]),
}

EXPORTS = tuple(_SIGS)
OPTS_FUNCS = frozenset(('simq_gemm_f32_batched', 'simq_conv2d_fwd', 'simq_conv2d_dgrad', 'simq_conv2d_wgrad', 'simq_conv2d_fwd_bf16', 'simq_conv2d_wgrad_bf16',
                        'simq_conv2d_wgrad_bf16_slab', 'simq_conv2d_wgrad_winograd', 'simq_conv2d_fwd_winograd', 'simq_conv2d_fwd_winograd4',
                        'simq_conv2d_fwd_bnrelu_in', 'simq_conv2d_wgrad_bnrelu_in'))


def launch_counts():
    buf = ctypes.create_string_buffer(4096)
    check(_c.simq_launch_counts(buf, 4096), 'simq_launch_counts')
    return {kv.split('=')[0]: int(kv.split('=')[1]) for kv in buf.value.decode().split(';') if kv}


def launch_opts(tile=None, **fields):
    o = LaunchOpts()
    _c.simq_launch_opts_default(ctypes.byref(o))
    if tile is not None and tile[0] > 0:
        o.force_bm, o.force_bn = int(tile[0]), int(tile[1])
    for k, v in fields.items():
        if k == 'struct_bytes' or not hasattr(o, k):
            raise SimqError('unknown launch option %r (fields of simq_launch_opts: %s)' % (k, ', '.join(n for n, _ in LaunchOpts._fields_[1:])))
        setattr(o, k, int(v))
    return o

for _name, (_res, _args) in _SIGS.items():
    _fn = getattr(_c, _name)
    _fn.restype = _res
    _fn.argtypes = _args


def last_error():
    return (_c.simq_last_error() or b'').decode()


def check(rc, what):
    if rc != 0:
        raise SimqError('%s failed (%d): %s' % (what, rc, last_error()))


def ptr(t):
    return None if t is None else c_void_p(t.data_ptr())


def stream_ptr(device=None):
    return c_void_p(torch.cuda.current_stream(device).cuda_stream)


class Lib:
    c = _c
    version = _c.simq_version()
    build_flags = _c.simq_build_flags()
    path = LIB_PATH


    @staticmethod
    def call(name, *args, opts=None):
        if name in OPTS_FUNCS:
            args = args + (ctypes.byref(opts) if opts is not None else None,)
        elif opts is not None:
            raise SimqError('%s takes no simq_launch_opts' % name)
        check(getattr(_c, name)(*args), name)


lib = Lib()

if Lib.build_flags != 0:
    import warnings
    warnings.warn('simq: SIMQ_LIBRARY selected the ablation build %s (simq_build_flags = %d): kernel selection follows SIMQ_* environment '
                  'variables; bench.py and the parity tests refuse it -- unset SIMQ_LIBRARY for anything but tools/' % (LIB_PATH, Lib.build_flags),
                  RuntimeWarning, stacklevel=2)


DEFAULT_PLAN_OPTIONS = {}


class Plan:

    def __init__(self, num_input_channels, num_output_channels, precision='fp32', options=None):
        self.cin, self.cout = int(num_input_channels), int(num_output_channels)
        if precision not in PRECISIONS:
            raise SimqError('unknown precision %r (choose from %s)' % (precision, sorted(PRECISIONS)))
        self.precision = precision
        o = PlanOptions()
        _c.simq_plan_options_default(ctypes.byref(o))
        for k, v in dict(DEFAULT_PLAN_OPTIONS, **(options or {})).items():
            if k == 'struct_bytes' or not hasattr(o, k):
                raise SimqError('unknown plan option %r (fields of simq_plan_options: %s)' % (k, ', '.join(n for n, _ in PlanOptions._fields_[1:])))
            setattr(o, k, int(v))
        h = c_void_p()
        check(_c.simq_plan_create_opts(self.cin, self.cout, PRECISIONS[precision], ctypes.byref(o), ctypes.byref(h)), 'simq_plan_create_opts')
        self.handle = h
        got = PlanOptions()
        check(_c.simq_plan_get_options(h, ctypes.byref(got)), 'simq_plan_get_options')
        self.options = {n: getattr(got, n) for n, _ in PlanOptions._fields_[1:]}
        self.param_count = _c.simq_param_count(h)
        self.bnbuf_count = _c.simq_bnbuf_count(h)
        self.tensors = []
        buf = ctypes.create_string_buffer(128)
        for i in range(_c.simq_param_num_tensors(h)):
            off, shape, kind = c_int64(), (c_int64 * 4)(), c_int()
            check(_c.simq_param_tensor_info(h, i, buf, 128, ctypes.byref(off), ctypes.byref(shape), ctypes.byref(kind)),
                  'simq_param_tensor_info')
            shp = list(shape) if kind.value == KIND_CONV_W else [shape[0]]
            self.tensors.append((buf.value.decode(), off.value, shp, kind.value))
        self.bn_layers = []
        for i in range(_c.simq_bn_num_layers(h)):
            off, ch = c_int64(), c_int()
            check(_c.simq_bn_layer_info(h, i, buf, 128, ctypes.byref(off), ctypes.byref(ch)), 'simq_bn_layer_info')
            self.bn_layers.append((buf.value.decode(), off.value, ch.value))

    def workspace_bytes(self, batch, forward_only=False):
        n = (_c.simq_workspace_bytes_forward if forward_only else _c.simq_workspace_bytes)(self.handle, int(batch))
        if n < 0:
            raise SimqError('simq_workspace_bytes(%d) failed' % batch)
        return n

    def __del__(self):
        try:
            if getattr(self, 'handle', None):
                _c.simq_plan_destroy(self.handle)
                self.handle = None
        except Exception:
            pass
```

Measured before the change: 4597.

## Make deterministic mode parallel: per-sample head partials, own stem slab, late join

In deterministic mode, the one-hot head backward no longer runs as a single serial block. It now launches one block per sample, writes per-sample partials, and folds them in a fixed order with a small fold kernel. The stem weight-gradient gets its own slab so it can overlap with the side-stream wgrad, and the late-join overlap is allowed in deterministic mode too. The slab-sum kernel is restructured to batch loads across splits. This only affects the deterministic path and adds workspace memory plus an extra launch.

```diff
diff --git a/include/simq.h b/include/simq.h
--- a/include/simq.h
+++ b/include/simq.h
@@ -231,6 +231,7 @@
 int64_t simq_conv2d_wgrad_bf16_slab_bytes(void);
 int simq_conv2d_wgrad_bf16_slab(const float* d_x, const float* d_dy, float* d_dw_ohwi, int batch, int hin, int win, int cin, int cout,
                                 int r, int s, int stride, int pad, int nplanes, void* d_scratch, void* d_slab, void* stream, const simq_launch_opts* opts);
+int simq_wgrad_slab_sum(const float* d_slab, float* d_dw, int64_t n, int splits, void* stream);
 int simq_upsample2x_fwd(const float* d_in, float* d_out, int batch, int h, int w, int c, void* stream);
 int simq_upsample2x_bwd(const float* d_dout, float* d_din, int batch, int h, int w, int c, void* stream);
 
diff --git a/spatial-intention-maps_amd/csrc/backward.hip b/spatial-intention-maps_amd/csrc/backward.hip
--- a/spatial-intention-maps_amd/csrc/backward.hip
+++ b/spatial-intention-maps_amd/csrc/backward.hip
@@ -25,7 +25,7 @@
                                mask_from_y ? c.aux(bn, 0) : nullptr, mask_from_y ? c.aux(bn, 1) : nullptr);
 }
 
-int conv_wgrad(const Ctx& c, const ConvL& cv, const Act& x, const Act& dy, int hin, const InBn& in = InBn()) {
+int conv_wgrad(const Ctx& c, const ConvL& cv, const Act& x, const Act& dy, int hin, const InBn& in = InBn(), bool own_slab = false) {
     ConvGeom g = geom(c.p, cv, c.B, hin);
     if (c.mc() && cv.wp_off >= 0) {
         SIMQ_REQUIRE(!in.on(), "conv_wgrad: BatchNorm-on-load exists for fp32 plans only");
@@ -36,6 +36,7 @@
     if (cv.wu_off >= 0 && c.L.wino >= 0 && winograd_wgrad_eligible(g) && c.p->opt.winograd_wgrad &&
         winograd_wgrad_pays(g, c.p->opt.winograd_wgrad_f4 != 0))
         return launch_conv_wgrad_winograd(x.f, dy.f, c.grads + cv.w_off, g, c.f(c.L.wino), c.stream, c.p->opt.winograd_wgrad_f4 != 0, in);
+    if (own_slab && c.dslab_stem()) return launch_conv_wgrad(x.f, dy.f, c.grads + cv.w_off, g, c.stream, in, c.dslab_stem(), stem_det_slab_floats(c.p->cin));
     return launch_conv_wgrad(x.f, dy.f, c.grads + cv.w_off, g, c.stream, in, c.dslab());
 }
 
@@ -108,7 +109,7 @@
     if (oh) {
         RC(launch_head_onehot_bwd(c.f(L.ah2), c.params + p->h3.w_off, oh->action, oh->q_sa, oh->y, oh->grad_scale, S[1],
                                   c.grads + p->h3.w_off, c.grads + p->h3.b_off, B, p->cout, c.stream,
-                                  c.f(L.yh2), 0, c.aux(p->hb2, 2), c.aux(p->hb2, 3), no_fuse_head ? nullptr : c.red(p->hb2), p->opt.deterministic));
+                                  c.f(L.yh2), 0, c.aux(p->hb2, 2), c.aux(p->hb2, 3), no_fuse_head ? nullptr : c.red(p->hb2), L.hpart >= 0 ? c.f(L.hpart) : nullptr));
     } else {
         RC(launch_upsample2x_fwd(c.f(L.ah2), c.f(L.up2), B, 48, 48, 32, c.stream));
         RC(launch_head_conv3_bwd(c.f(L.up2), c.params + p->h3.w_off, d_dq, S[0], c.grads + p->h3.w_off, c.grads + p->h3.b_off, B, 9216, 32, p->cout, c.stream,
@@ -247,7 +248,7 @@
         if (piped) SIMQ_CHECK_HIP(hipEventRecord(c.ev_wdone[set], c.wstream));
         else RC(join());
     }
-    const bool late_join = piped && phase != 1 && i_hi > i_lo && ((i_hi - i_lo) & 1) == 1 && !p->opt.deterministic;
+    const bool late_join = piped && phase != 1 && i_hi > i_lo && ((i_hi - i_lo) & 1) == 1;
     if (piped) {
         if (late_join) SIMQ_CHECK_HIP(hipStreamWaitEvent(c.stream, c.ev_wdone[0], 0));
         else RC(join());
@@ -271,7 +272,7 @@
     if (stem16)
         RC(launch_stem_wgrad_bf16(x0.f, T1.pl.hi, c.grads + p->stem.w_off, T0, B, 96, 96, p->cin, c.stream));
     else
-        RC(conv_wgrad(c, p->stem, x0, T1, 96));
+        RC(conv_wgrad(c, p->stem, x0, T1, 96, InBn(), true));
     if (late_join) RC(join());
     return 0;
 }
diff --git a/spatial-intention-maps_amd/csrc/common.h b/spatial-intention-maps_amd/csrc/common.h
--- a/spatial-intention-maps_amd/csrc/common.h
+++ b/spatial-intention-maps_amd/csrc/common.h
@@ -114,7 +114,13 @@
 int launch_conv_winograd4(const float* x, const float* U4, float* y, const ConvGeom& g, const ConvEpilogue& e, float* scratch,
                           hipStream_t stream, const InBn& in = InBn());
 constexpr int64_t kWgradDetSlabFloats = 16 << 20;
-int launch_conv_wgrad(const float* x, const float* dy, float* dw, const ConvGeom& g, hipStream_t stream, const InBn& in = InBn(), float* det_slab = nullptr);
+constexpr int kWgradMaxSplits = 96;
+inline int64_t stem_det_slab_floats(int cin) {
+    const int64_t want = (int64_t)kWgradMaxSplits * 64 * 49 * cin;
+    return want < kWgradDetSlabFloats ? want : kWgradDetSlabFloats;
+}
+int launch_conv_wgrad(const float* x, const float* dy, float* dw, const ConvGeom& g, hipStream_t stream, const InBn& in = InBn(), float* det_slab = nullptr,
+                      int64_t det_slab_floats = kWgradDetSlabFloats);
 int launch_wgrad_slab_sum(const float* slab, float* dw, int64_t n, int splits, hipStream_t stream);
 int launch_wgrad_batched(const float* x, const float* dy, float* dw, int M, int N, int K, int batch, hipStream_t stream, const LaunchTune& tune = LaunchTune());
 bool winograd_wgrad_eligible(const ConvGeom& g);
@@ -191,7 +197,8 @@
                            float grad_scale, float* ds1, float* dw3, float* db3, int B, int Cout, hipStream_t stream,
                            const float* ypre = nullptr, int ypre_bf16 = 0, const float* mean = nullptr, const float* invstd = nullptr,
                            double* red = nullptr,
-                           int serial = 0);
+                           float* det_part = nullptr);
+int64_t head_onehot_det_part_bytes(int B);
 int launch_head_conv3_bwd(const float* x, const float* w, const float* dq, float* dx, float* dw, float* dbias,
                           int B, int HW, int Cin, int Cout, hipStream_t stream, float* det_slab = nullptr);
 
diff --git a/spatial-intention-maps_amd/csrc/conv_wgrad.hip b/spatial-intention-maps_amd/csrc/conv_wgrad.hip
--- a/spatial-intention-maps_amd/csrc/conv_wgrad.hip
+++ b/spatial-intention-maps_amd/csrc/conv_wgrad.hip
@@ -20,6 +20,7 @@
     unsigned x_bytes, dy_bytes;
     long gx, gdy, gdw;
     float* slab;
+    int64_t slab_floats;
     const float* xscale; const float* xshift;
 };
 
@@ -249,7 +250,7 @@
     const int ltiles = tiles * batch;
     const int rsteps = (p.M + BR - 1) / BR;
     int max_splits = rsteps / 8;
-    if (max_splits > 96) max_splits = 96;
+    if (max_splits > kWgradMaxSplits) max_splits = kWgradMaxSplits;
     if (max_splits < 1) max_splits = 1;
     int splits = 1;
     double best = 1e300;
@@ -270,6 +271,8 @@
     splits = (p.M + rps - 1) / rps;
     p.rows_per_split = rps;
     p.splits = splits;
+    SIMQ_REQUIRE(!p.slab || (int64_t)splits * p.Cout * p.K <= p.slab_floats, "wgrad: %d splits of %ld floats do not fit the slab of %ld floats",
+                 splits, (long)p.Cout * p.K, (long)p.slab_floats);
     p.xcd_group = (tune.wgrad_xcd_group == 2 && batch == 1 && splits >= 8 && tiles > 1) ? 1 : 0;
     const int launch_splits = p.xcd_group ? ((splits + 7) / 8) * 8 : splits;
     note_launch(batch > 1 ? "wgrad_f32_batched" : "wgrad_f32");
@@ -288,10 +291,27 @@
     return 0;
 }
 
-__global__ void __launch_bounds__(256) wgrad_slab_sum_kernel(const float* __restrict__ slab, float* __restrict__ dw, size_t n, int splits) {
-    for (size_t e = blockIdx.x * (size_t)256 + threadIdx.x; e < n; e += (size_t)gridDim.x * 256) {
-        float a = slab[e];
-        for (int s2 = 1; s2 < splits; ++s2) a += slab[(size_t)s2 * n + e];
+constexpr int kSumBatch = 32, kSumThreads = 64;
+
+__global__ void __launch_bounds__(kSumThreads) wgrad_slab_sum_kernel(const float* __restrict__ slab, float* __restrict__ dw, size_t n, int splits) {
+    for (size_t e = blockIdx.x * (size_t)kSumThreads + threadIdx.x; e < n; e += (size_t)gridDim.x * kSumThreads) {
+        const float* src = slab + e;
+        float a = src[0];
+        int s2 = 1;
+        for (; s2 + kSumBatch <= splits; s2 += kSumBatch) {
+            float v[kSumBatch];
+#pragma unroll
+            for (int k = 0; k < kSumBatch; ++k) v[k] = src[(size_t)(s2 + k) * n];
+#pragma unroll
+            for (int k = 0; k < kSumBatch; ++k) a += v[k];
+        }
+        if (s2 < splits) {
+            float v[kSumBatch];
+#pragma unroll
+            for (int k = 0; k < kSumBatch; ++k) v[k] = s2 + k < splits ? src[(size_t)(s2 + k) * n] : 0.f;
+#pragma unroll
+            for (int k = 0; k < kSumBatch; ++k) if (s2 + k < splits) a += v[k];
+        }
         dw[e] = a;
     }
 }
@@ -299,16 +319,18 @@
 }
 
 int launch_wgrad_slab_sum(const float* slab, float* dw, int64_t n, int splits, hipStream_t stream) {
-    int blocks = (int)((n + 255) / 256);
-    if (blocks > 2048) blocks = 2048;
-    hipLaunchKernelGGL(wgrad_slab_sum_kernel, dim3(blocks), dim3(256), 0, stream, slab, dw, (size_t)n, splits);
+    SIMQ_REQUIRE(slab && dw && n >= 1 && splits >= 1, "wgrad_slab_sum: bad argument (n=%ld, splits=%d)", (long)n, splits);
+    int64_t blocks = (n + kSumThreads - 1) / kSumThreads;
+    if (blocks > 8192) blocks = 8192;
+    hipLaunchKernelGGL(wgrad_slab_sum_kernel, dim3((unsigned)blocks), dim3(kSumThreads), 0, stream, slab, dw, (size_t)n, splits);
     SIMQ_CHECK_LAUNCH();
     return 0;
 }
 
-int launch_conv_wgrad(const float* x, const float* dy, float* dw, const ConvGeom& g, hipStream_t stream, const InBn& in, float* det_slab) {
+int launch_conv_wgrad(const float* x, const float* dy, float* dw, const ConvGeom& g, hipStream_t stream, const InBn& in, float* det_slab,
+                      int64_t det_slab_floats) {
     WgradArgs a;
-    a.x = x; a.dy = dy; a.dw = dw; a.slab = det_slab;
+    a.x = x; a.dy = dy; a.dw = dw; a.slab = det_slab; a.slab_floats = det_slab_floats;
     a.xscale = in.scale; a.xshift = in.shift;
     SIMQ_REQUIRE(!in.live, "conv_wgrad: BatchNorm-on-load takes the scale / shift the forward pass saved (not a live layer)");
     SIMQ_REQUIRE(!in.scale || g.Cin % 64 == 0, "conv_wgrad: BatchNorm-on-load needs Cin %% 64 == 0 (Cin=%d)", g.Cin);
@@ -345,7 +367,7 @@
     a.M = M; a.K = K;
     a.tilesI = a.tilesJ = a.rows_per_split = 0;
     a.gx = (long)M * K; a.gdy = (long)M * N; a.gdw = (long)N * K;
-    a.xscale = a.xshift = nullptr; a.slab = nullptr;
+    a.xscale = a.xshift = nullptr; a.slab = nullptr; a.slab_floats = 0;
     const double xb = 4.0 * M * K, yb = 4.0 * M * N;
     SIMQ_REQUIRE(xb < 4294967000.0 && yb < 4294967000.0, "wgrad_batched: operand exceeds the 4 GiB buffer-addressing limit");
     a.x_bytes = (unsigned)xb; a.dy_bytes = (unsigned)yb;
diff --git a/spatial-intention-maps_amd/csrc/head.hip b/spatial-intention-maps_amd/csrc/head.hip
--- a/spatial-intention-maps_amd/csrc/head.hip
+++ b/spatial-intention-maps_amd/csrc/head.hip
@@ -126,17 +126,24 @@
     }
 }
 
+constexpr int kHeadPartFloats = 128;
+
 __global__ void __launch_bounds__(32) head_onehot_bwd_kernel(const float* __restrict__ ah2, const float* __restrict__ w3,
                                                              const int64_t* __restrict__ action, const float* __restrict__ q_sa,
                                                              const float* __restrict__ y, float grad_scale, float* ds1, float* dw3,
                                                              float* db3, int Cout, const float* __restrict__ ypre, int ypre_bf16,
-                                                             const float* __restrict__ mean, const float* __restrict__ invstd, double* red, int B) {
+                                                             const float* __restrict__ mean, const float* __restrict__ invstd, double* red, int B,
+                                                             float* part) {
     constexpr int W2 = 96, W1 = 48, CIN = 32;
     for (int b = blockIdx.x; b < B; b += gridDim.x) {
     const int ci = threadIdx.x;
     const int64_t a = action[b];
     const int co = (int)(a / (W2 * W2)), p = (int)(a - (int64_t)co * W2 * W2);
-    if (co >= Cout) continue;
+    float* pt = part ? part + (size_t)b * kHeadPartFloats : nullptr;
+    if (co >= Cout) {
+        if (pt && ci == 0) reinterpret_cast<int*>(pt)[0] = -1;
+        continue;
+    }
     const int oy = p / W2, ox = p - oy * W2;
     const float d = q_sa[b] - y[b];
     const float g = fminf(fmaxf(d, -1.f), 1.f) * grad_scale;
@@ -148,8 +155,13 @@
     const float* src = ah2 + (size_t)b * W1 * W1 * CIN + ci;
     const float up = ly0 * (lx0 * src[(y0 * W1 + x0) * CIN] + lx1 * src[(y0 * W1 + x1) * CIN]) +
                      ly1 * (lx0 * src[(y1 * W1 + x0) * CIN] + lx1 * src[(y1 * W1 + x1) * CIN]);
-    unsafeAtomicAdd(dw3 + co * CIN + ci, g * up);
-    if (ci == 0) unsafeAtomicAdd(db3 + co, g);
+    if (pt) {
+        pt[32 + ci] = g * up;
+        if (ci == 0) { reinterpret_cast<int*>(pt)[0] = co; pt[1] = g; }
+    } else {
+        unsafeAtomicAdd(dw3 + co * CIN + ci, g * up);
+        if (ci == 0) unsafeAtomicAdd(db3 + co, g);
+    }
     const float dx = g * w3[co * CIN + ci];
     float* base = ds1 + (size_t)b * W1 * W1 * CIN + ci;
     base[(y0 * W1 + x0) * CIN] += ly0 * lx0 * dx;
@@ -172,8 +184,66 @@
             s1 += dz * ((yv - mu) * is);
         }
     }
-    unsafeAtomicAdd(red + ci, (double)s0);
-    unsafeAtomicAdd(red + CIN + ci, (double)s1);
+    if (pt) {
+        pt[64 + ci] = s0;
+        pt[96 + ci] = s1;
+    } else {
+        unsafeAtomicAdd(red + ci, (double)s0);
+        unsafeAtomicAdd(red + CIN + ci, (double)s1);
+    }
+    }
+}
+
+constexpr int kHeadFoldBatch = 16;
+
+__global__ void __launch_bounds__(128) head_onehot_fold_kernel(const float* __restrict__ part, float* dw3, float* db3, double* red, int Cout, int B) {
+    constexpr int CIN = 32;
+    const int ci = threadIdx.x & 31, role = threadIdx.x >> 5;
+    if ((role == 1 || role == 2) && !red) return;
+    if (role == 3 && ci != 0) return;
+    float acc[MAX_COUT];
+    double dacc = 0.0;
+#pragma unroll
+    for (int c = 0; c < MAX_COUT; ++c) acc[c] = 0.f;
+    if (role == 0) {
+#pragma unroll
+        for (int c = 0; c < MAX_COUT; ++c) if (c < Cout) acc[c] = dw3[c * CIN + ci];
+    } else if (role == 3) {
+#pragma unroll
+        for (int c = 0; c < MAX_COUT; ++c) if (c < Cout) acc[c] = db3[c];
+    } else {
+        dacc = red[(role - 1) * CIN + ci];
+    }
+    const int voff = role == 3 ? 1 : 32 * (role + 1) + ci;
+    for (int b0 = 0; b0 < B; b0 += kHeadFoldBatch) {
+        int co[kHeadFoldBatch];
+        float v[kHeadFoldBatch];
+#pragma unroll
+        for (int k = 0; k < kHeadFoldBatch; ++k) {
+            const bool in = b0 + k < B;
+            const float* pt = part + (size_t)(in ? b0 + k : b0) * kHeadPartFloats;
+            co[k] = in ? reinterpret_cast<const int*>(pt)[0] : -1;
+            v[k] = pt[voff];
+        }
+#pragma unroll
+        for (int k = 0; k < kHeadFoldBatch; ++k) {
+            if (co[k] < 0) continue;
+            if (role == 1 || role == 2) {
+                dacc += (double)v[k];
+            } else {
+#pragma unroll
+                for (int c = 0; c < MAX_COUT; ++c) if (co[k] == c) acc[c] += v[k];
+            }
+        }
+    }
+    if (role == 0) {
+#pragma unroll
+        for (int c = 0; c < MAX_COUT; ++c) if (c < Cout) dw3[c * CIN + ci] = acc[c];
+    } else if (role == 3) {
+#pragma unroll
+        for (int c = 0; c < MAX_COUT; ++c) if (c < Cout) db3[c] = acc[c];
+    } else {
+        red[(role - 1) * CIN + ci] = dacc;
     }
 }
 
@@ -219,14 +289,21 @@
 
 int launch_head_onehot_bwd(const float* ah2, const float* w3, const int64_t* action, const float* q_sa, const float* y,
                            float grad_scale, float* ds1, float* dw3, float* db3, int B, int Cout, hipStream_t stream,
-                           const float* ypre, int ypre_bf16, const float* mean, const float* invstd, double* red, int serial) {
+                           const float* ypre, int ypre_bf16, const float* mean, const float* invstd, double* red, float* det_part) {
     SIMQ_REQUIRE(Cout >= 1 && Cout <= MAX_COUT, "head_onehot_bwd: Cout=%d unsupported", Cout);
+    SIMQ_REQUIRE(B >= 1, "head_onehot_bwd: batch=%d", B);
     SIMQ_CHECK_HIP(hipMemsetAsync(ds1, 0, sizeof(float) * (size_t)B * 48 * 48 * 32, stream));
-    hipLaunchKernelGGL(head_onehot_bwd_kernel, dim3(serial ? 1 : B), dim3(32), 0, stream, ah2, w3, action, q_sa, y, grad_scale, ds1, dw3, db3, Cout,
-                       ypre, ypre_bf16, mean, invstd, red, B);
-    SIMQ_CHECK_LAUNCH();
-    return 0;
-}
+    hipLaunchKernelGGL(head_onehot_bwd_kernel, dim3(B), dim3(32), 0, stream, ah2, w3, action, q_sa, y, grad_scale, ds1, dw3, db3, Cout,
+                       ypre, ypre_bf16, mean, invstd, red, B, det_part);
+    SIMQ_CHECK_LAUNCH();
+    if (det_part) {
+        hipLaunchKernelGGL(head_onehot_fold_kernel, dim3(1), dim3(128), 0, stream, det_part, dw3, db3, red, Cout, B);
+        SIMQ_CHECK_LAUNCH();
+    }
+    return 0;
+}
+
+int64_t head_onehot_det_part_bytes(int B) { return (int64_t)B * kHeadPartFloats * (int64_t)sizeof(float); }
 
 int launch_head_up_relu_conv3(const float* z2, const float* w, float* z, int B, int Cout, hipStream_t stream) {
     SIMQ_REQUIRE(Cout >= 1 && Cout <= MAX_COUT, "head_up_relu_conv3: Cout=%d unsupported", Cout);
diff --git a/spatial-intention-maps_amd/csrc/layout.hip b/spatial-intention-maps_amd/csrc/layout.hip
--- a/spatial-intention-maps_amd/csrc/layout.hip
+++ b/spatial-intention-maps_amd/csrc/layout.hip
@@ -75,6 +75,8 @@
     }
     L.wslab = p->precision == SIMQ_PREC_BF16 ? take(conv_wgrad_bf16_slab_bytes()) : -1;
     L.dslab = p->opt.deterministic ? take(kWgradDetSlabFloats * f) : -1;
+    L.dslab_stem = p->opt.deterministic ? take(stem_det_slab_floats(p->cin) * f) : -1;
+    L.hpart = p->opt.deterministic ? take(head_onehot_det_part_bytes(B)) : -1;
     L.total = off;
     return L;
 }
diff --git a/spatial-intention-maps_amd/csrc/ops_abi.hip b/spatial-intention-maps_amd/csrc/ops_abi.hip
--- a/spatial-intention-maps_amd/csrc/ops_abi.hip
+++ b/spatial-intention-maps_amd/csrc/ops_abi.hip
@@ -305,6 +305,11 @@
     return launch_conv_wgrad_bf16(xp, yp, nplanes, d_dw, g, st, static_cast<float*>(d_slab));
 }
 
+int simq_wgrad_slab_sum(const float* d_slab, float* d_dw, int64_t n, int splits, void* stream) {
+    SIMQ_REQUIRE(d_slab && d_dw && n >= 1 && splits >= 1, "wgrad_slab_sum: bad argument");
+    return launch_wgrad_slab_sum(d_slab, d_dw, n, splits, static_cast<hipStream_t>(stream));
+}
+
 int simq_upsample2x_fwd(const float* d_in, float* d_out, int batch, int h, int w, int c, void* stream) {
     return launch_upsample2x_fwd(d_in, d_out, batch, h, w, c, static_cast<hipStream_t>(stream));
 }
diff --git a/spatial-intention-maps_amd/csrc/plan.h b/spatial-intention-maps_amd/csrc/plan.h
--- a/spatial-intention-maps_amd/csrc/plan.h
+++ b/spatial-intention-maps_amd/csrc/plan.h
@@ -98,6 +98,8 @@
     int64_t S2[3];
     int64_t wslab;
     int64_t dslab;
+    int64_t dslab_stem;
+    int64_t hpart;
     int64_t fwd_total;
     int64_t total;
 };
@@ -157,6 +159,7 @@
         return lazy1() || (p->precision == SIMQ_PREC_BF16 && p->opt.bn1_mask_from_preact && planes_only());
     }
     float* dslab() const { return L.dslab >= 0 ? f(L.dslab) : nullptr; }
+    float* dslab_stem() const { return L.dslab_stem >= 0 ? f(L.dslab_stem) : nullptr; }
     InBn inbn_saved(const BnL& b) const { InBn in; in.scale = aux(b, 0); in.shift = aux(b, 1); return in; }
     void wplanes(const ConvL& cv, bool transposed, const uint16_t* out[2]) const {
         uint16_t* base = reinterpret_cast<uint16_t*>(wc + (transposed ? W.wtpl : W.wpl));
diff --git a/spatial-intention-maps_amd/simq/_lib.py b/spatial-intention-maps_amd/simq/_lib.py
--- a/spatial-intention-maps_amd/simq/_lib.py
+++ b/spatial-intention-maps_amd/simq/_lib.py
@@ -111,6 +111,7 @@
     'simq_conv2d_wgrad_bf16': (c_int, [c_void_p, c_void_p, c_void_p] + [c_int] * 10 + [c_void_p, c_void_p] + [c_void_p]),
     'simq_conv2d_wgrad_bf16_slab_bytes': (c_int64, []),
     'simq_conv2d_wgrad_bf16_slab': (c_int, [c_void_p, c_void_p, c_void_p] + [c_int] * 10 + [c_void_p, c_void_p, c_void_p] + [c_void_p]),
+    'simq_wgrad_slab_sum': (c_int, [c_void_p, c_void_p, c_int64, c_int, c_void_p]),
     'simq_upsample2x_fwd': (c_int, [c_void_p, c_void_p, c_int, c_int, c_int, c_int, c_void_p]),
     'simq_upsample2x_bwd': (c_int, [c_void_p, c_void_p, c_int, c_int, c_int, c_int, c_void_p]),
     'simq_profile_start': (c_int, []),
```

Measured after the change: 4731, median of 6. 1.03x the previous value.
